# kharchenkolab/dropEst

Hardware: AMD Instinct MI355X
Metric: Mreads/s processed to final count matrix (higher is better)
Workload: dtype u64

## Files before the change

dropest_amd/csrc/context.h:

```cpp
#pragma once

#include <algorithm>
#include <chrono>
#include <condition_variable>
#include <functional>
#include <mutex>
#include <cstring>
#include <map>
#include <memory>
#include <string>
#include <thread>
#include <unordered_map>
#include <unordered_set>
#include <vector>

#include "../../include/dropest_amd.h"
#include "k_cbhash.h"
#include "k_collisions.h"
#include "k_merge.h"
#include "k_umi_directional.h"
#include "whitelist.h"
#include "k_misc.h"
#include "k_radix.h"
#include "k_ssort.h"
#include "k_segreduce.h"
#include "k_mergepath.h"
#include "matrix_decode.h"
#include "util.h"

namespace dropest {

typedef unsigned long long u64;
typedef uint32_t u32;

struct ReadChunk {
	DevBuf<u64> cb, umi;
	DevBuf<u32> gene, aux;
	const u64 *p_cb = nullptr, *p_umi = nullptr;
	const u32 *p_gene = nullptr, *p_aux = nullptr;
	uint64_t n = 0;
};

struct KernelStat { u32 launches = 0; double ms = 0, bytes = 0; };

__global__ __launch_bounds__(256) void store_append_kernel(const u64 *__restrict__ s_cb, const u64 *__restrict__ s_umi, const u32 *__restrict__ s_gene, const u32 *__restrict__ s_aux,
                                                           u64 *__restrict__ d_cb, u64 *__restrict__ d_umi, u32 *__restrict__ d_gene, u32 *__restrict__ d_aux, size_t count) {
	for (size_t i = size_t(blockIdx.x) * 256u + threadIdx.x; i < count; i += size_t(gridDim.x) * 256u) { d_cb[i] = s_cb[i]; d_umi[i] = s_umi[i]; d_gene[i] = s_gene[i]; d_aux[i] = s_aux[i]; }
}

struct ReadStore {
	DevBuf<u64> cb, umi;
	DevBuf<u32> gene, aux;
	size_t n = 0;
	hipStream_t copy = nullptr;
	PinnedBuf<unsigned char> stage[2];
	hipEvent_t done[2] = {nullptr, nullptr};
	int cur = 0;
	~ReadStore() { for (auto e : done) if (e) (void)hipEventDestroy(e); if (copy) (void)hipStreamDestroy(copy); }
	size_t capacity() const { return cb.n; }
	void reserve(size_t want) {
		if (want <= capacity() && cb.p) return;
		size_t cap = std::max<size_t>(want, std::max<size_t>(capacity() * 2, size_t(1) << 20));
		if (n && !copy) HIP_CHECK(hipStreamCreateWithFlags(&copy, hipStreamNonBlocking));
		if (copy) HIP_CHECK(stream_wait(copy));
		DevBuf<u64> ncb, numi; DevBuf<u32> ngene, naux;
		ncb.alloc(cap); numi.alloc(cap); ngene.alloc(cap); naux.alloc(cap);
		ncb.mark_persistent(); numi.mark_persistent(); ngene.mark_persistent(); naux.mark_persistent();
		if (n) {
			HIP_CHECK(hipMemcpyAsync(ncb.p, cb.p, n * 8, hipMemcpyDeviceToDevice, copy));
			HIP_CHECK(hipMemcpyAsync(numi.p, umi.p, n * 8, hipMemcpyDeviceToDevice, copy));
			HIP_CHECK(hipMemcpyAsync(ngene.p, gene.p, n * 4, hipMemcpyDeviceToDevice, copy));
			HIP_CHECK(hipMemcpyAsync(naux.p, aux.p, n * 4, hipMemcpyDeviceToDevice, copy));
			HIP_CHECK(stream_wait(copy));
		}
		cb = std::move(ncb); umi = std::move(numi); gene = std::move(ngene); aux = std::move(naux);
	}
	static bool is_pinned(const void *p) {
		hipPointerAttribute_t a{};
		if (hipPointerGetAttributes(&a, p) != hipSuccess) { (void)hipGetLastError(); return false; }
		return a.type == hipMemoryTypeHost;
	}
	void push(const uint64_t *h_cb, const uint64_t *h_umi, const uint32_t *h_gene, const uint32_t *h_aux, size_t count) {
		if (!count) return;
		reserve(n + count);
		if (!copy) HIP_CHECK(hipStreamCreateWithFlags(&copy, hipStreamNonBlocking));
		if (is_pinned(h_cb) && is_pinned(h_umi) && is_pinned(h_gene) && is_pinned(h_aux)) {
			HIP_CHECK(hipMemcpyAsync(cb.p + n, h_cb, count * 8, hipMemcpyHostToDevice, copy));
			HIP_CHECK(hipMemcpyAsync(umi.p + n, h_umi, count * 8, hipMemcpyHostToDevice, copy));
			HIP_CHECK(hipMemcpyAsync(gene.p + n, h_gene, count * 4, hipMemcpyHostToDevice, copy));
			HIP_CHECK(hipMemcpyAsync(aux.p + n, h_aux, count * 4, hipMemcpyHostToDevice, copy));
			HIP_CHECK(stream_wait(copy));
			n += count;
			return;
		}
		const size_t piece_max = size_t(4) << 20;
		for (size_t at = 0; at < count; at += piece_max) {
			const size_t m = std::min(piece_max, count - at);
			PinnedBuf<unsigned char> &st = stage[cur];
			if (!done[cur]) HIP_CHECK(hipEventCreateWithFlags(&done[cur], hipEventDisableTiming));
			else HIP_CHECK(event_wait(done[cur]));
			st.ensure(m * 24);
			unsigned char *b = st.p;
			std::memcpy(b, h_cb + at, m * 8); std::memcpy(b + m * 8, h_umi + at, m * 8);
			std::memcpy(b + m * 16, h_gene + at, m * 4); std::memcpy(b + m * 20, h_aux + at, m * 4);
			HIP_CHECK(hipMemcpyAsync(cb.p + n, b, m * 8, hipMemcpyHostToDevice, copy));
			HIP_CHECK(hipMemcpyAsync(umi.p + n, b + m * 8, m * 8, hipMemcpyHostToDevice, copy));
			HIP_CHECK(hipMemcpyAsync(gene.p + n, b + m * 16, m * 4, hipMemcpyHostToDevice, copy));
			HIP_CHECK(hipMemcpyAsync(aux.p + n, b + m * 20, m * 4, hipMemcpyHostToDevice, copy));
			HIP_CHECK(hipEventRecord(done[cur], copy));
			cur ^= 1;
			n += m;
		}
	}
	void push_segments(size_t n_seg, const uint64_t *const *h_cb, const uint64_t *const *h_umi, const uint32_t *const *h_gene, const uint32_t *const *h_aux,
	                   const uint64_t *counts) {
		size_t total = 0;
		for (size_t k = 0; k < n_seg; ++k) total += size_t(counts[k]);
		if (!total) return;
		if (total > (size_t(4) << 20)) { for (size_t k = 0; k < n_seg; ++k) push(h_cb[k], h_umi[k], h_gene[k], h_aux[k], size_t(counts[k])); return; }
		reserve(n + total);
		if (!copy) HIP_CHECK(hipStreamCreateWithFlags(&copy, hipStreamNonBlocking));
		PinnedBuf<unsigned char> &st = stage[cur];
		if (!done[cur]) HIP_CHECK(hipEventCreateWithFlags(&done[cur], hipEventDisableTiming));
		else HIP_CHECK(event_wait(done[cur]));
		st.ensure(total * 24);
		unsigned char *b = st.p;
		size_t at = 0;
		for (size_t k = 0; k < n_seg; ++k) {
			const size_t m = size_t(counts[k]);
			if (!m) continue;
			std::memcpy(b + at * 8, h_cb[k], m * 8); std::memcpy(b + total * 8 + at * 8, h_umi[k], m * 8);
			std::memcpy(b + total * 16 + at * 4, h_gene[k], m * 4); std::memcpy(b + total * 20 + at * 4, h_aux[k], m * 4);
			at += m;
		}
		HIP_CHECK(hipMemcpyAsync(cb.p + n, b, total * 8, hipMemcpyHostToDevice, copy));
		HIP_CHECK(hipMemcpyAsync(umi.p + n, b + total * 8, total * 8, hipMemcpyHostToDevice, copy));
		HIP_CHECK(hipMemcpyAsync(gene.p + n, b + total * 16, total * 4, hipMemcpyHostToDevice, copy));
		HIP_CHECK(hipMemcpyAsync(aux.p + n, b + total * 20, total * 4, hipMemcpyHostToDevice, copy));
		HIP_CHECK(hipEventRecord(done[cur], copy));
		cur ^= 1;
		n += total;
	}
	void push_device(const uint64_t *d_cb, const uint64_t *d_umi, const uint32_t *d_gene, const uint32_t *d_aux, size_t count, hipStream_t on) {
		if (!count) return;
		reserve(n + count);
		hipLaunchKernelGGL(store_append_kernel, dim3(unsigned(std::min<size_t>((count + 255) / 256, 4096))), dim3(256), 0, on, reinterpret_cast<const u64 *>(d_cb),
		                   reinterpret_cast<const u64 *>(d_umi), d_gene, d_aux, cb.p + n, umi.p + n, gene.p + n, aux.p + n, count);
		HIP_CHECK(hipGetLastError());
		HIP_CHECK(stream_wait(on));
		n += count;
	}
	void push_peer(const uint64_t *d_cb, const uint64_t *d_umi, const uint32_t *d_gene, const uint32_t *d_aux, size_t count, int dst_device, int src_device, hipStream_t on) {
		if (!count) return;
		reserve(n + count);
		HIP_CHECK(hipMemcpyPeerAsync(cb.p + n, dst_device, d_cb, src_device, count * 8, on));
		HIP_CHECK(hipMemcpyPeerAsync(umi.p + n, dst_device, d_umi, src_device, count * 8, on));
		HIP_CHECK(hipMemcpyPeerAsync(gene.p + n, dst_device, d_gene, src_device, count * 4, on));
		HIP_CHECK(hipMemcpyPeerAsync(aux.p + n, dst_device, d_aux, src_device, count * 4, on));
		HIP_CHECK(stream_wait(on));
		n += count;
	}
	void wait() { if (copy) HIP_CHECK(stream_wait(copy)); }
	void clear() { wait(); n = 0; }
};

inline std::string decode_code(u64 code, const std::vector<std::string> &side) {
	if (code & ESCAPE_BIT) {
		u64 k = code & ~ESCAPE_BIT;
		if (k >= side.size()) throw RangeError("escaped code refers to an unregistered side string");
		return side[k];
	}
	if (code == 0) return std::string();
	int len = (bit_length(code) - 1) / 2;
	std::string s(size_t(len), 'A');
	for (int i = 0; i < len; ++i) s[size_t(i)] = "ACGT"[(code >> (2 * (len - 1 - i))) & 3];
	return s;
}
inline bool encode_code(const std::string &s, u64 &code) {
	if (s.empty() || s.size() > 31) return false;
	u64 c = 1;
// ... 73 lines not shown
		std::unique_lock<std::mutex> one(job_m, std::try_to_lock);
		if (!one.owns_lock()) return false;
		{
			std::lock_guard<std::mutex> lk(m);
			job = fn; active = workers; pending = workers; ++generation; error.clear();
		}
		cv_go.notify_all();
		std::unique_lock<std::mutex> lk(m);
		cv_done.wait(lk, [&] { return pending == 0; });
		if (!error.empty()) throw std::runtime_error(error);
		return true;
	}
};
template <class F>
inline unsigned parallel_ranges(size_t n, F &&fn, size_t min_per_worker = 100000, unsigned max_workers = 8) {
	HostPool &pool = HostPool::get();
	unsigned workers = unsigned(std::min<size_t>(std::min<size_t>(max_workers, pool.size()), std::max<size_t>(1, n / std::max<size_t>(1, min_per_worker))));
	if (workers <= 1) { fn(size_t(0), n, 0u); return 1; }
	if (pool.run(workers, [&](unsigned w) { fn(n * w / workers, n * (w + 1) / workers, w); })) return workers;
	for (unsigned w = 0; w < workers; ++w) fn(n * w / workers, n * (w + 1) / workers, w);
	return workers;
}

struct GlibcRand {
	uint32_t ring[34];
	int pos = 0;
	uint64_t drawn = 0;
	explicit GlibcRand(unsigned seed = 1) { this->seed(seed); }
	void seed(unsigned s) {
		int32_t r[34];
		r[0] = int32_t(s ? s : 1u);
		for (int i = 1; i < 31; ++i) {
			const int64_t hi = r[i - 1] / 127773, lo = r[i - 1] % 127773;
			int64_t w = 16807 * lo - 2836 * hi;
			if (w < 0) w += 2147483647;
			r[i] = int32_t(w);
		}
		for (int i = 0; i < 31; ++i) ring[i] = uint32_t(r[i]);
		for (int i = 31; i < 34; ++i) ring[i] = ring[i - 31];
		pos = 0; drawn = 0;
		for (int i = 0; i < 310; ++i) step();
	}
	uint32_t step() {
		const uint32_t v = ring[(pos + 3) % 34] + ring[(pos + 31) % 34];
		ring[pos] = v;
		pos = (pos + 1) % 34;
		return v;
	}
	int next() { ++drawn; return int(step() >> 1); }
	void skip_to(uint64_t n_drawn) { while (drawn < n_drawn) next(); }
};

struct HostCell {
	u32 id;
	CellRowPod row;
	bool merged = false, excluded = false;
};

}

struct SimplePairs { std::vector<uint64_t> key; std::vector<uint32_t> cnt, ed; std::vector<double> prob;  };

struct dropest_ctx {
	using u64 = dropest::u64;
	using u32 = dropest::u32;

	dropest_cfg cfg;
	std::string barcodes_file, match_levels;
	u32 query_mask = 0;
	u32 min_before = 0, min_after = 0;
	hipStream_t stream = nullptr;

	std::vector<dropest::ReadChunk> chunks;
	dropest::ReadStore store;
	long store_chunk = -1;
	uint64_t n_reads = 0;
	dropest::DevBuf<u64> cat_cb, cat_umi;
	dropest::DevBuf<u32> cat_gene, cat_aux;
	const u64 *d_cb = nullptr, *d_umi = nullptr;
	const u32 *d_gene = nullptr, *d_aux = nullptr;
	std::vector<std::string> side;
	dropest::ReadPack rpack{};
	std::function<void()> unpack_reads;
	void need_columns() {
		if (!rpack.on()) return;
		if (!unpack_reads) throw dropest::InvalidError("internal: packed reads without an unpacker");
		unpack_reads();
		rpack = dropest::ReadPack{};
	}

	bool initialized = false, merged = false;
	dropest::GlibcRand rng;
	void reseed_rng() { rng.seed(cfg.umi_merge_kind == DROPEST_UMI_MERGE_SIMPLE ? 42u : 1u); }

	dropest::DevBuf<dropest::CbSlot> t_slots;
	dropest::DevBuf<u32> slot;
	dropest::DevBuf<u64> hot_key;
	dropest::DevBuf<u32> hot_slot;
	u32 n_hot = 0;
	dropest::CbTable table{};
	uint64_t forced_table_capacity = 0;
	u32 n_cells = 0;
	dropest::DevBuf<u64> cell_cb;
	dropest::DevBuf<u32> cell_first;
	dropest::KeyLayout layout{};
	int umi_clean_bits = 0;
	u32 wanted_bits[3] = {0, 0, 0};
	bool umi_sentinel_stripped = false;
	int umi_dict_mode = 0;
	bool umi_dict_on = false;
	u32 umi_dict_n = 0;
	dropest::DevBuf<u64> umi_dict, umi_ranked;
	std::vector<u64> umi_dict_host;
	const u64 *umi_key_column() const { return umi_dict_on ? umi_ranked.p : d_umi; }
	void build_umi_dict(const std::function<void(dropest::DevBuf<u64> &, u32 &)> *across = nullptr);
	bool umi_dict_wanted(int gene_bits, int cell_bits) const;
	void sort_unique_u64(dropest::DevBuf<u64> &d, u32 &n);
	bool map_umi(u64 api_code, u64 &field) const;
	bool map_umi_or_add(u64 api_code, u64 &field);
	dropest::IngestStats ingest{};
	dropest::GlobalCounters counters{};

	dropest::DevBuf<u64> keys_a, keys_b;
	dropest::DevBuf<u32> vals_a, vals_b;
	bool chr_from_gene = false;
	bool lazy_stats = false;
	dropest::DevBuf<u32> gene_chr;
	dropest::DevBuf<u32> mol_exon, mol_intron, mol_exon2, mol_intron2, cg_exon, cg_intron;

	u32 n_mol = 0;
	dropest::DevBuf<u64> mol_key;
	dropest::DevBuf<u32> mol_reads, mol_mark;
	u32 n_cg = 0;
	dropest::DevBuf<u64> cg_key;
	dropest::DevBuf<u32> cg_mol_begin, cg_n_all, cg_n_req, cg_reads_all, cg_reads_req;
	dropest::DevBuf<u32> cell_cg_count;
	dropest::DevBuf<u32> cell_cg_begin, cell_n_genes, cell_req_genes, cell_req_umis, cell_total_umis, cell_total_reads;
	u32 n_chr_rows = 0;
	dropest::DevBuf<u64> chr_row_key;
	dropest::DevBuf<u32> chr_exon, chr_intron, chr_inter;

	dropest::Whitelist wl;
	dropest::DevBuf<dropest::WlEntry> d_wl[dropest::WL_MAX_PARTS];
	dropest::DevBuf<u64> d_wl_code[dropest::WL_MAX_PARTS];
	dropest::DevBuf<dropest::WlTabRow> d_wl_tab[dropest::WL_MAX_PARTS];
	bool wl_tab_ok = false;
	dropest::DevBuf<u64> mol_key2;
	dropest::DevBuf<u32> mol_reads2, mol_mark2, remap;
	std::unordered_map<u32, u32> reassign;
	std::unordered_map<u64, std::vector<dropest::UmiOverride>> umi_overrides;

	dropest::PinnedBuf<unsigned char> h_stage;
	void fetch(void *dst, const void *d_src, size_t bytes);
	dropest::PinnedBuf<unsigned char> h_up;
	void upload(void *d_dst, const void *src, size_t bytes);

	dropest::DevBuf<u32> tile_counts, tile_prefix, scalars, rs_hist, rs_row_total, rs_digit_base;
	dropest::DevBuf<u32> real_list;
	dropest::DevBuf<dropest::CellRowPod> real_rows_dev;
	dropest::DevBuf<u32> sizes_dev;
	bool real_list_current = false;
	bool real_pristine = false;
	dropest::DevBuf<u64> scalars64;
	struct MatrixResult {
		dropest::DevBuf<u32> d_row, d_val;
		dropest::PinnedBuf<u32> h_row, h_val;
		struct List {
			dropest::DevBuf<u32> d;
			dropest::PinnedBuf<u32> h;
			u32 cap = 0, n = 0;
			void ensure(u32 c, bool to_host) { cap = c; d.ensure(1 + 2 * size_t(c)); if (to_host) h.ensure(1 + 2 * size_t(c)); }
			u32 *d_count() const { return d.p; }
			u32 *d_pos() const { return d.p + 1; }
			u32 *d_val() const { return d.p + 1 + cap; }
			u32 *h_count() const { return h.p; }
			u32 *h_pos() const { return h.p ? h.p + 1 : nullptr; }
			u32 *h_val() const { return h.p ? h.p + 1 + cap : nullptr; }
		};
		dropest::DevBuf<uint16_t> d_row16, d_val16;
		dropest::PinnedBuf<uint16_t> h_row16, h_val16;
		List vals;
		dropest::DevBuf<uint8_t> d_drow8, d_val8;
		dropest::PinnedBuf<uint8_t> h_drow8, h_val8;
		List rows;
		int narrow = 0;
		dropest::DevBuf<u32> d_col_cell, d_col_start, d_col_list;
		std::vector<u32> col_list_host;
		bool wire = false;
		std::shared_ptr<dropest::DecodeJob> job, late_job;
		std::chrono::steady_clock::time_point job_t0;
		MatrixResult *dependent = nullptr;
		std::vector<u32> rider_out, rider_cnt, wire_chunk_end;
		dropest::DevBuf<u32> d_rider_out;
		void settle() {
			if (dependent) { MatrixResult *d = dependent; dependent = nullptr; d->settle(); }
			if (job) { (void)job->wait(); job->quiesce(); job.reset(); }
			if (late_job) { late_job->quiesce(); late_job.reset(); }
		}
		dropest::PinnedBuf<u32> h_flags;
		u32 wire_epoch = 0;
		std::vector<u32> colptr;
		uint64_t nnz = 0, ncols = 0;
	} mat[3];
	dropest::DevBuf<dropest::IngestStats> d_ingest;
	dropest::DevBuf<dropest::GlobalCounters> d_counters;

	std::vector<dropest::HostCell> real;
	std::vector<uint64_t> filtered;
	std::vector<u32> filtered_ridx;
	dropest::PinnedBuf<u64> sort_stage;
	dropest::DevBuf<u64> sort_cols;
	std::vector<u32> sort_idx;
	std::vector<int32_t> filtered_umis;
	std::vector<uint64_t> sort_ids;
	bool filtered_valid = false;
	u32 filtered_threshold = 0;
	int filtered_max_cells = -1;
	struct CbMirror {
		std::vector<u64> key; std::vector<u32> id; u64 mask = 0; int level = 0;
		void clear() { key.clear(); id.clear(); mask = 0; level = 0; }
		void build(size_t n, const std::function<void(size_t, u64 &, u32 &)> &item) {
			size_t cap = 16; while (cap < n * 2 + 2) cap <<= 1;
			key.assign(cap, 0ull); id.assign(cap, 0u); mask = cap - 1;
			for (size_t i = 0; i < n; ++i) {
				u64 k; u32 v; item(i, k, v);
				u64 h = dropest::mix64(k) & mask;
				while (key[h] != 0ull && key[h] != k) h = (h + 1) & mask;
				key[h] = k; id[h] = v;
			}
		}
		long find(u64 k) const {
			if (key.empty()) return -1;
			for (u64 h = dropest::mix64(k) & mask;; h = (h + 1) & mask) { if (key[h] == k) return long(id[h]); if (key[h] == 0ull) return -1; }
		}
	} cb_mirror;
	long real_find(u32 cell_id) const {
		size_t lo = 0, hi = real.size();
		while (lo < hi) { size_t mid = (lo + hi) / 2; if (real[mid].id < cell_id) lo = mid + 1; else hi = mid; }
		return (lo < real.size() && real[lo].id == cell_id) ? long(lo) : -1;
	}
	u32 real_at(u32 cell_id) const {
		long i = real_find(cell_id);
		if (i < 0) throw dropest::RangeError("cell is not a real-candidate cell");
		return u32(i);
	}
	std::string barcode_of(const dropest::HostCell &h) const { return dropest::decode_code(h.row.barcode, side); }
	const std::vector<uint64_t> &filtered_cells();
	std::vector<std::pair<uint64_t, uint64_t>> merge_pairs;
	uint64_t n_real_now = 0;

	bool profiling = false;
	std::string profile_only;
	std::map<std::string, dropest::KernelStat> stats;
	struct Pending { std::string name; hipEvent_t a, b; double bytes; };
	std::vector<Pending> pending;
	std::vector<hipEvent_t> event_pool;

	bool stage_sync = getenv("DROPEST_STAGE_SYNC") != nullptr;
	struct HostStage {
		dropest_ctx *c; const char *name; std::chrono::steady_clock::time_point t0;
		HostStage(dropest_ctx *ctx, const char *n) : c(ctx), name(n) {
			if (c->stage_sync && c->profiling) (void)dropest::stream_wait(c->stream);
			t0 = std::chrono::steady_clock::now();
		}
		~HostStage() {
			if (!c->profiling || !c->profile_only.empty()) return;
			if (c->stage_sync) (void)dropest::stream_wait(c->stream);
			auto &s = c->stats[std::string("host:") + name];
			s.launches++;
			s.ms += std::chrono::duration<double, std::milli>(std::chrono::steady_clock::now() - t0).count();
		}
	};

	~dropest_ctx();
	void init_from_cfg(const dropest_cfg &c);

	template <class F> void timed(const char *name, double bytes, F &&launch);
	void collect_timings();

	void concat_chunks();
	void free_results();
	void release_tables() {
		t_slots.release(); slot.release(); keys_a.release(); keys_b.release(); vals_a.release(); vals_b.release();
		mol_key.release(); mol_reads.release(); mol_mark.release(); mol_key2.release(); mol_reads2.release(); mol_mark2.release();
		mol_exon.release(); mol_intron.release(); mol_exon2.release(); mol_intron2.release();
	}
	void run_set_initialized();
	void run_merge_and_filter();

	void build_cb_table();
	void assign_cell_ids();
	void plan_key_layout();
	void build_keys(bool with_stats = false, bool allow_fused = true);
	bool build_keys_fused(bool with_stats);
	void ss_splitters_from_sample(u32 n_sample, u32 os, u32 Ff, u32 F2, u64 varying_of_sample);
	bool keys_in_l1 = false;
	dropest::DevBuf<u32> ks_flag;
	u32 main_sort_passes = 0, main_sort_kind = 0;
	void scan_counts(const u32 *in, u32 *out, u32 n, u32 *total_out);
	dropest::DevBuf<u32> scan_chunk;
	void radix_sort(u64 *&keys, u32 *&vals, u64 *&keys_alt, u32 *&vals_alt, u32 n, u64 varying_mask, int val_bytes = 4,
	                const char *stat_prefix = nullptr);
	dropest::DevBuf<u64> ss_sample_a, ss_sample_b, ss_fine, ss_coarse;
	dropest::DevBuf<u32> ss_base1, ss_cnt2, ss_bucket_base, ss_bucket_cnt, ss_tmp, ss_n_loc, ss_prefix, ss_chunk, ss_big_list;
	struct RecvChunk { hipEvent_t ev; dropest::CbRanges rg; };
	std::vector<RecvChunk> recv_chunks;
	double hot_coverage = 0;
	dropest::DevBuf<u32> ss_cg_loc, ss_cg_cnt, ss_cg_prefix;
	bool cg_from_sort = false;
	dropest::DevBuf<u32> ss_cursors;
	bool ss_no_reserve = false;
	bool splitter_sort_reduce();
	void reduce_all();
	void reduce_molecules_to_cell_gene();
	void reduce_cell_gene_to_cells();
	void refresh_real_rows();
	void upload_whitelist();
	void search_merge_candidates(const std::vector<u32> &cells, const dropest::MergeUniverse &U, dropest::MergeSearch &S);
	void search_merge_candidates_host(const std::vector<u32> &cells, const dropest::MergeUniverse &U, dropest::MergeSearch &S);
	void build_merge_pairs(const std::vector<u32> &cells, dropest::MergeSearch &S);
	void decide_merge_targets(const dropest::MergeUniverse &U, dropest::MergeSearch &S, const std::vector<u32> &inter,
	                          std::vector<long> &targets, std::vector<u32> &target_ridx);
	std::vector<std::vector<u32>> replay_candidate_orders(const dropest::MergeUniverse &U, dropest::MergeSearch &S,
	                                                      const std::vector<u32> &need_order);
	std::vector<u32> pair_intersections(const std::vector<u32> &pair_base_cell, const std::vector<u32> &pair_cand_cell);
	void pair_intersections(const std::vector<u32> &pair_base_cell, const std::vector<u32> &pair_cand_cell, std::vector<u32> &inter);
	std::vector<double> poisson_expected_intersections(const std::vector<u32> &pair_base_cell, const std::vector<u32> &pair_cand_cell);
	struct PoissonTables { dropest::DevBuf<double> p, mult, np; dropest::DevBuf<u64> adj; u32 n_classes = 0, max_size = 0; bool ready = false; } ptab;
	void poisson_local_umis(u32 &kept, u32 &max_size);
	struct PoissonSource { const u32 *cell_cg_begin, *cell_cg_count; const u64 *cg_key; const u32 *cg_mol_begin; u64 gene_mask; };
	void poisson_tables_from_state();
	void poisson_tables_from_umi_codes(u32 kept, u64 code_mask, u32 max_size);
	void poisson_expected_pairs(const PoissonSource &src, const u32 *d_pb, const u32 *d_pc, u32 NP, const u32 *count_host, double *expected);
	struct ValidationView {
		dropest::DevBuf<u64> mol_key, cg_key;
		dropest::DevBuf<u32> cg_mol_begin, cell_cg_begin, cell_cg_count;
		dropest::DevBuf<uint4> barcodes;
		std::vector<uint64_t> cells;
		std::vector<u32> umis;
		u32 n_mol = 0, n_cg = 0, F = 0;
		int umi_bits = 0, gene_bits = 0;
		u64 gene_none = 0;
		double ms = 0;
	};
	bool is_shard_ctx = false, was_split = false;
	void validation_build_view(ValidationView &V);
	void validation_set_barcodes(ValidationView &V, const std::vector<std::string> &text);
	void validation_finish_view(ValidationView &V);
	struct ValidationPairs {
		dropest::DevBuf<u32> d_pb, d_pc, d_cnt, d_inter; dropest::DevBuf<dropest::PairRange> d_pr;
		std::vector<u32> cnt;
	};
	bool validation_common_genes(const ValidationView &V, const std::vector<u32> &a, const std::vector<u32> &b, ValidationPairs &P);
	u32 validation_evaluate_range(const ValidationView &V, const dropest_validation_opts &opts, ValidationPairs &P, u32 q0, u32 q1, u32 *inter, double *expected);
	static void validation_tail(size_t n, const u32 *inter, double *expected, double *prob);
	void validation_sample(const ValidationView &V, const dropest_validation_opts &opts, dropest_validation_sample &S, std::vector<u32> &a, std::vector<u32> &b);
	void validation_evaluate(const ValidationView &V, const dropest_validation_opts &opts, dropest_validation_sample &S, const std::vector<u32> &a,
	                         const std::vector<u32> &b);
	void run_merge_validation(const dropest_validation_opts *opts, dropest_validation_sample *samples, u32 n_samples);
	void poisson_build_tables(const u32 *d_counts, u32 n_counts, double total, u32 max_size);
	void poisson_expected_from_keys(const u32 *d_off, u32 NP, const u64 *d_keys, u32 NK, double *expected_host);
	void shard_merge_umi_histogram(dropest::DevBuf<u32> &hist, uint64_t &kept, u32 &max_size);
	void shard_merge_set_umi_distribution(const u32 *d_counts, uint64_t n_counts, uint64_t kept_total, u32 max_size);
	void shard_merge_expected(uint64_t n_pairs, const uint32_t *cand_local, const uint64_t *base_begin, const uint64_t *base_end,
	                          const uint64_t *d_base_low, double *expected);
	void shard_merge_decide_poisson(const uint32_t *inter, const double *expected, int64_t *target_g);
	void decide_poisson_targets(const dropest::MergeUniverse &U, dropest::MergeSearch &S, const std::vector<u32> &inter,
	                            const std::vector<double> &expected, std::vector<long> &targets, std::vector<u32> &target_ridx);
	std::vector<long> compute_merge_targets(const std::vector<u32> &cells, const std::vector<u32> &ridx,
	                                        std::vector<u32> *target_ridx = nullptr);
	void compute_merge_targets(const std::vector<u32> &cells, const std::vector<u32> &ridx, std::vector<long> &targets,
	                           std::vector<u32> *target_ridx);
	dropest::DevBuf<u32> cell_real_index;
	struct MergeScratch {
		dropest::MergeSearch S;
		std::vector<u32> pb, inter, tr, cells, ridx, target_ridx, cur, rank, src, tgt32, lists, ids_dense;
		std::vector<long> targets;
		std::vector<int64_t> tgt;
		std::vector<int32_t> reads, umis;
		std::vector<uint8_t> excl;
		dropest::DevBuf<u32> d_pb, d_pc, d_inter, d_src, d_tgt;
		dropest::DevBuf<dropest::PairRange> d_pr;
	} ms;
	void run_cb_merge_real();
	void run_cb_merge_simple();
	void simple_merge_targets(std::vector<u32> &cells, std::vector<u32> &tgt_id, SimplePairs &P);
	struct StrategyTargets { bool valid = false; std::vector<u32> cells, target; SimplePairs P; } strategy_targets;
	const StrategyTargets &need_strategy_targets();
	struct SimpleReplayInput { std::vector<u64> query; std::vector<std::vector<u32>> in_order; };
	void simple_pair_table(const u64 *sorted, u32 n_valid, int cell_bits, const u32 *d_cell_size, const u64 *d_cell_code, SimplePairs &P,
	                       dropest::DevBuf<u64> *d_run_key, dropest::DevBuf<u32> *d_run_cnt, u32 *n_runs = nullptr);
	void simple_pairs_to_host(const u64 *d_run_key, const u32 *d_run_cnt, u32 runs, const u64 *d_cell_code, SimplePairs &P);
	void simple_replay_local(const std::vector<u32> &bases, SimpleReplayInput &R, bool globalize);
	void run_cb_merge_all();
	void merge_all_filtered_targets(std::vector<u32> &target_pos);
	void merge_all_targets(std::vector<u64> code, const std::vector<int32_t> &umis, const std::function<std::string(u32)> &text,
	                       const std::vector<u32> *bases, std::vector<u32> &target_pos);
	std::unordered_set<u32> extra_excluded;
	std::unordered_set<u32> explicit_sources;
	void clear_strategy_pairs() {
		if (explicit_sources.empty()) { merge_pairs.clear(); return; }
		std::vector<std::pair<uint64_t, uint64_t>> keep;
		for (auto const &pr : merge_pairs) if (explicit_sources.count(u32(pr.first))) keep.push_back(pr);
		merge_pairs.swap(keep);
	}
	void mutate_exclude_cell(u32 cell);
	void mutate_merge_cells(u32 src, u32 tgt);
	void mutate_merge_umis(u32 cell, u32 gene, uint64_t n, const uint64_t *src, const uint64_t *tgt);
	void mutate_add_umi_to_cell(u32 cell, u32 gene, uint64_t umi_code, u32 mark, const uint8_t *quality, u32 quality_length);
	u32 n_qsum_rows = 0;
	void emit_matrix_levels(u32 query_mask, bool reads_output);
	struct ShardMerge;
	std::shared_ptr<ShardMerge> shard;
	bool ingested = false, external_merge_done = false;
	void run_ingest();
	void shard_export_rows(const std::vector<u32> &local_cells);
	void shard_merge_begin_free();
	void shard_merge_search(uint64_t n_global, const uint64_t *g_barcode, const uint32_t *g_n_genes, const int32_t *g_total_umis,
	                        uint64_t n_bases, const uint32_t *base_g, const uint32_t *base_local, uint64_t *n_pairs);
	void shard_merge_intersect(uint64_t n_pairs, const uint32_t *cand_local, const uint64_t *base_begin, const uint64_t *base_end,
	                           const uint64_t *d_base_low, uint32_t *inter);
	void shard_merge_decide(const uint32_t *inter, int64_t *target_g);
	void shard_merge_quality_import(uint64_t n_local, const uint32_t *local_rank, const uint32_t *d_import_rank, const uint32_t *d_import_q);
	const u32 *reagg_import_prio = nullptr;
	u32 reagg_import_from = 0, reagg_import_n = 0;
	void shard_merge_finish(uint64_t n_local, const uint32_t *local_id, const uint8_t *excluded, const uint8_t *merged_away,
	                        const int32_t *total_reads, const int32_t *total_umis, uint64_t n_moves, const uint32_t *move_src,
	                        const uint32_t *move_tgt, uint64_t n_import, const uint32_t *d_cell, const uint64_t *d_low,
	                        const uint32_t *const d_cols[4]);
	void reaggregate_after_merge();
	void run_umi_merge_simple();
	std::vector<u32> umi_first_positions(const std::vector<u64> &sorted_codes);
	struct ShardHooks {
		std::function<std::vector<u64>(const std::vector<u64> &)> first_seen_global;
		std::function<std::vector<u64>(const std::vector<u32> &, const std::vector<u32> &, const std::vector<u32> &)> rng_offsets;
		std::function<void(u32 *, size_t)> globalize_umi_first;
	};
	std::shared_ptr<ShardHooks> hooks;
	void emit_columns_device(bool filtered_m, bool reads_output, const std::vector<u32> &col_cell, const std::vector<u32> &col_start, uint64_t nnz, bool wait = true);
	struct GatheredGroups { std::vector<u32> size, off, begin, hr, hm, hfirst; std::vector<u64> hk; };
	void umi_gather_groups(const std::vector<u32> &groups, GatheredGroups &G, const u32 *d_first_table);
	void umi_patch_groups(const std::vector<u32> &p_idx, const std::vector<u32> &p_all, const std::vector<u32> &p_req,
	                      const std::vector<u32> &p_rreq, const std::unordered_map<u32, int> &umis_removed);
// ... 59 lines not shown
```

dropest_amd/csrc/dropest_amd.hip:

```cpp

#include "context.h"
extern "C" void dropest_bgzf_warm_up(void *stream);
#include "k_keyscatter.h"
#include "k_umidict.h"

#include <atomic>
#include <functional>
#include <map>
#include <mutex>

using namespace dropest;

static thread_local std::string g_last_error;

template <class F>
static dropest_status guarded(F &&f) {
	try {
		f();
		return DROPEST_OK;
	} catch (const InvalidError &e) { g_last_error = e.what(); return DROPEST_ERR_INVALID;
	} catch (const RangeError &e) { g_last_error = e.what(); return DROPEST_ERR_RANGE;
	} catch (const UnsupportedError &e) { g_last_error = e.what(); return DROPEST_ERR_UNSUPPORTED;
	} catch (const IoError &e) { g_last_error = e.what(); return DROPEST_ERR_IO;
	} catch (const DeviceError &e) { g_last_error = e.what(); return DROPEST_ERR_DEVICE;
	} catch (const std::bad_alloc &) { g_last_error = "host allocation failed"; return DROPEST_ERR_DEVICE;
	} catch (const std::exception &e) { g_last_error = e.what(); return DROPEST_ERR_INVALID; }
}

static void need_init(dropest_ctx *ctx) {
	if (!ctx) throw InvalidError("null context");
	if (!ctx->initialized) throw InvalidError("You must initialize container");
	HIP_CHECK(hipSetDevice(ctx->cfg.device));
}

static inline u32 div_up(uint64_t a, uint64_t b) { return u32((a + b - 1) / b); }

static void partition_by_owner_on(int device, hipStream_t st, const u64 *d_cb, const u64 *d_umi, const u32 *d_gene, const u32 *d_aux, uint64_t n64,
                                  u32 n_parts, u64 *d_out_cb, u64 *d_out_umi, u32 *d_out_gene, u32 *d_out_aux, u32 *d_out_idx, uint64_t *counts,
                                  void *d_scratch, uint64_t scratch_bytes);

template <class K>
static u32 resident_grid(K kernel, int threads, u32 wanted) {
	int dev = 0, cus = 0, per_cu = 0;
	HIP_CHECK(hipGetDevice(&dev));
	HIP_CHECK(hipDeviceGetAttribute(&cus, hipDeviceAttributeMultiprocessorCount, dev));
	HIP_CHECK(hipOccupancyMaxActiveBlocksPerMultiprocessor(&per_cu, kernel, threads, 0));
	return std::max<u32>(1u, std::min<u32>(wanted, u32(std::max(1, cus) * std::max(1, per_cu))));
}

static u32 query_mask_from_code(const std::string &code) {
	u32 m = 0;
	for (char c : code) {
		switch (c) {
			case 'e': m |= 1u << 2; break;
			case 'i': m |= 1u << 4; break;
			case 'E': m |= 1u << 3; break;
			case 'I': m |= 1u << 5; break;
			case 'B': m |= 1u << 6; break;
			case 'A': m |= 1u << 7; break;
			default: throw InvalidError(std::string("Unexpected gene match levels: ") + c);
		}
	}
	return m;
}

void dropest_ctx::init_from_cfg(const dropest_cfg &c) {
	cfg = c;
	barcodes_file = c.barcodes_file ? c.barcodes_file : "";
	match_levels = c.gene_match_levels ? c.gene_match_levels : "eEBA";
	cfg.barcodes_file = barcodes_file.c_str();
	cfg.gene_match_levels = match_levels.c_str();
	query_mask = query_mask_from_code(match_levels);
	if (c.min_genes_before_merge < 0 || c.min_genes_after_merge < 0) throw InvalidError("negative gene threshold");
	min_before = u32(c.min_genes_before_merge);
	min_after = std::max(u32(c.min_genes_after_merge), min_before);
	if (c.merge_kind != DROPEST_MERGE_NONE && c.merge_kind != DROPEST_MERGE_REAL_BARCODES && c.merge_kind != DROPEST_MERGE_SIMPLE &&
	    c.merge_kind != DROPEST_MERGE_POISSON_REAL && c.merge_kind != DROPEST_MERGE_POISSON_SIMPLE && c.merge_kind != DROPEST_MERGE_ALL)
		throw InvalidError("unknown merge_kind");
	if (c.umi_merge_kind != DROPEST_UMI_MERGE_SIMPLE && c.umi_merge_kind != DROPEST_UMI_MERGE_DIRECTIONAL)
		throw InvalidError("unknown umi_merge_kind");
	if (c.max_umi_merge_edit_distance < 0) throw InvalidError("negative max_umi_merge_edit_distance");
	int ndev = 0;
	if (hipGetDeviceCount(&ndev) != hipSuccess || ndev == 0)
		throw DeviceError("no HIP device visible: the dropEst hot path has no CPU implementation");
	if (c.device < 0 || c.device >= ndev) throw InvalidError("device ordinal out of range");
	HIP_CHECK(hipSetDevice(c.device));
	HIP_CHECK(hipStreamCreateWithFlags(&stream, hipStreamNonBlocking));
	{
		void *scratch = nullptr;
		HIP_CHECK(hipMalloc(&scratch, 256));
		(void)hipMemsetAsync(scratch, 0, 256, stream);
		(void)hipMemsetAsync(scratch, 0, 256, nullptr);
		{
			void *pin = nullptr, *big = nullptr;
			const size_t mb = size_t(1) << 20;
			if (hipHostMalloc(&pin, mb, hipHostMallocDefault) == hipSuccess && hipMalloc(&big, mb) == hipSuccess) {
				(void)hipMemcpyAsync(big, pin, mb, hipMemcpyHostToDevice, nullptr);
				(void)hipMemcpyAsync(pin, big, mb, hipMemcpyDeviceToHost, nullptr);
				(void)hipStreamSynchronize(nullptr);
				for (size_t bytes : {size_t(8) << 10, size_t(48) << 10, size_t(256) << 10, mb}) {
					(void)hipMemcpyAsync(big, pin, bytes, hipMemcpyHostToDevice, stream);
					(void)hipMemcpyAsync(pin, big, bytes, hipMemcpyDeviceToHost, stream);
				}
				(void)hipStreamSynchronize(stream);
			}
			if (big) (void)hipFree(big);
			if (pin) (void)hipHostFree(pin);
		}
		hipLaunchKernelGGL(store_append_kernel, dim3(1), dim3(256), 0, stream, (const u64 *)nullptr, (const u64 *)nullptr, (const u32 *)nullptr, (const u32 *)nullptr,
		                   (u64 *)nullptr, (u64 *)nullptr, (u32 *)nullptr, (u32 *)nullptr, size_t(0));
		(void)hipGetLastError();
		dropest_bgzf_warm_up(stream);
		(void)hipStreamSynchronize(stream);
		(void)hipStreamSynchronize(nullptr);
		(void)hipFree(scratch);
	}
	reseed_rng();
}

dropest_ctx::~dropest_ctx() {
	for (auto &p : pending) { (void)hipEventDestroy(p.a); (void)hipEventDestroy(p.b); }
	for (auto e : event_pool) (void)hipEventDestroy(e);
	for (auto &M : mat) M.settle();
	if (stream2) { (void)stream_wait(stream2); (void)hipStreamDestroy(stream2); }
	if (ev_fork) (void)hipEventDestroy(ev_fork);
	if (ev_raw) (void)hipEventDestroy(ev_raw);
	if (ev_ship) (void)hipEventDestroy(ev_ship);
	if (stream) (void)hipStreamDestroy(stream);
}

template <class F>
void dropest_ctx::timed(const char *name, double bytes, F &&launch) {
	auto selected = [&]() {
		if (profile_only.empty()) return true;
		size_t at = 0;
		while (at <= profile_only.size()) {
			size_t end = profile_only.find('|', at);
			if (end == std::string::npos) end = profile_only.size();
			if (end > at && std::strncmp(name, profile_only.c_str() + at, end - at) == 0) return true;
			at = end + 1;
		}
		return false;
	};
	static const bool sync_trace = getenv("DROPEST_SYNC_TRACE") != nullptr;
	if (sync_trace) {
		fprintf(stderr, "[launch %p] %s\n", static_cast<void *>(this), name);
		launch();
		HIP_CHECK(hipGetLastError());
		HIP_CHECK(hipStreamSynchronize(stream));
		if (stream2) HIP_CHECK(hipStreamSynchronize(stream2));
		fprintf(stderr, "[done   %p] %s\n", static_cast<void *>(this), name);
		return;
	}
	if (!profiling || !selected()) {
		launch(); HIP_CHECK(hipGetLastError()); return;
	}
	auto get = [&]() {
		if (!event_pool.empty()) { hipEvent_t e = event_pool.back(); event_pool.pop_back(); return e; }
		hipEvent_t e; HIP_CHECK(hipEventCreate(&e)); return e;
	};
	hipEvent_t a = get(), b = get();
	HIP_CHECK(hipEventRecord(a, stream));
	launch();
	HIP_CHECK(hipGetLastError());
	HIP_CHECK(hipEventRecord(b, stream));
	pending.push_back(Pending{name, a, b, bytes});
}

void dropest_ctx::fetch(void *dst, const void *d_src, size_t bytes) {
	if (!bytes) return;
	h_stage.ensure(std::max<size_t>(bytes, 4096));
	HIP_CHECK(hipMemcpyAsync(h_stage.p, d_src, bytes, hipMemcpyDeviceToHost, stream));
	HIP_CHECK(stream_wait(stream));
	if (bytes < (size_t(4) << 20)) std::memcpy(dst, h_stage.p, bytes);
	else
		dropest::parallel_ranges(bytes, [&](size_t b, size_t e, unsigned) { std::memcpy(static_cast<char *>(dst) + b, h_stage.p + b, e - b); }, size_t(2) << 20, dropest::HostPool::MAX);
}

void dropest_ctx::upload(void *d_dst, const void *src, size_t bytes) {
	if (!bytes) return;
	if (bytes < (size_t(1) << 20)) { HIP_CHECK(hipMemcpyAsync(d_dst, src, bytes, hipMemcpyHostToDevice, stream)); HIP_CHECK(stream_wait(stream)); return; }
	h_up.ensure(bytes);
	dropest::parallel_ranges(bytes, [&](size_t b, size_t e, unsigned) { std::memcpy(h_up.p + b, static_cast<const char *>(src) + b, e - b); }, size_t(2) << 20, dropest::HostPool::MAX);
	HIP_CHECK(hipMemcpyAsync(d_dst, h_up.p, bytes, hipMemcpyHostToDevice, stream));
	HIP_CHECK(stream_wait(stream));
}

static void tail_mark(const char *what, bool restart = false) {
	static const bool on = getenv("DROPEST_TAIL_TRACE") != nullptr;
	if (!on) return;
	static thread_local std::chrono::steady_clock::time_point t0;
	const auto now = std::chrono::steady_clock::now();
	if (restart) t0 = now;
	fprintf(stderr, "[tail] %9.1f us  %s\n", std::chrono::duration<double, std::micro>(now - t0).count(), what);
}

void dropest_ctx::collect_timings() {
	if (pending.empty()) return;
	HIP_CHECK(stream_wait(stream));
	for (auto &p : pending) {
		float ms = 0;
		HIP_CHECK(hipEventElapsedTime(&ms, p.a, p.b));
		auto &s = stats[p.name];
		s.launches++; s.ms += ms; s.bytes += p.bytes;
		event_pool.push_back(p.a); event_pool.push_back(p.b);
	}
	pending.clear();
}

void dropest_ctx::concat_chunks() {
	if (d_cb) return;
	if (n_reads == 0) return;
	store.wait();
	if (store_chunk >= 0) {
		dropest::ReadChunk &c = chunks[size_t(store_chunk)];
		c.p_cb = store.cb.p; c.p_umi = store.umi.p; c.p_gene = store.gene.p; c.p_aux = store.aux.p; c.n = store.n;
	}
	if (n_reads >= 0xFFFFFFFEull) throw UnsupportedError("more than 2^32-2 reads in one context (shard across GPUs)");
	if (chunks.size() == 1) {
		d_cb = chunks[0].p_cb; d_umi = chunks[0].p_umi; d_gene = chunks[0].p_gene; d_aux = chunks[0].p_aux;
		return;
	}
	cat_cb.alloc(n_reads); cat_umi.alloc(n_reads); cat_gene.alloc(n_reads); cat_aux.alloc(n_reads);
	cat_cb.mark_persistent(); cat_umi.mark_persistent(); cat_gene.mark_persistent(); cat_aux.mark_persistent();
	uint64_t off = 0;
	for (auto &c : chunks) {
		HIP_CHECK(hipMemcpyAsync(cat_cb.p + off, c.p_cb, c.n * 8, hipMemcpyDeviceToDevice, stream));
		HIP_CHECK(hipMemcpyAsync(cat_umi.p + off, c.p_umi, c.n * 8, hipMemcpyDeviceToDevice, stream));
		HIP_CHECK(hipMemcpyAsync(cat_gene.p + off, c.p_gene, c.n * 4, hipMemcpyDeviceToDevice, stream));
		HIP_CHECK(hipMemcpyAsync(cat_aux.p + off, c.p_aux, c.n * 4, hipMemcpyDeviceToDevice, stream));
		off += c.n;
	}
	HIP_CHECK(stream_wait(stream));
	chunks.clear();
	chunks.emplace_back();
	chunks[0].p_cb = cat_cb.p; chunks[0].p_umi = cat_umi.p; chunks[0].p_gene = cat_gene.p; chunks[0].p_aux = cat_aux.p;
	chunks[0].n = n_reads;
	d_cb = cat_cb.p; d_umi = cat_umi.p; d_gene = cat_gene.p; d_aux = cat_aux.p;
}

void dropest_ctx::free_results() {
	HostStage hs(this, "reset");
	invalidate_prefetch();
	initialized = merged = ingested = external_merge_done = false;
	ss_no_reserve = false;
	reseed_rng();
	shard.reset();
	n_cells = n_mol = n_cg = n_chr_rows = 0;
	cb_mirror.clear(); real_pristine = false;
	real.clear(); filtered.clear(); filtered_valid = false; strategy_targets = StrategyTargets(); merge_pairs.clear(); reassign.clear(); umi_overrides.clear(); n_real_now = 0;
	merge_rank.clear(); reagg_prio = nullptr; extra_excluded.clear(); explicit_sources.clear(); mol_sorted_rows = 0xFFFFFFFFu;
	layout = dropest::KeyLayout{}; umi_clean_bits = 0; umi_sentinel_stripped = false; chr_from_gene = false;
	umi_dict_on = false; umi_dict_n = 0; umi_dict_host.clear();
}

static constexpr u32 GENE_CHR_CAP = 1u << 20;

void dropest_ctx::build_cb_table() {
	const u32 n = u32(n_reads);
	uint64_t cap = forced_table_capacity ? forced_table_capacity : cfg.cb_table_capacity;
	const bool chunked = !recv_chunks.empty() && !forced_table_capacity;
	const u32 n_chunks_in = chunked ? u32(recv_chunks.size()) : 1u;
	if (chunked) HIP_CHECK(hipStreamWaitEvent(stream, recv_chunks[0].ev, 0));
	uint64_t n_first = n;
	if (chunked) n_first = recv_chunks[0].rg.total();
	auto over_sample_ranges = [&](auto &&f) {
		if (!chunked) { f(u32(0), n); return; }
		const CbRanges &rg = recv_chunks[0].rg;
		for (u32 q = 0; q < rg.n; ++q) if (rg.cnt[q]) f(rg.off[q], rg.cnt[q]);
	};
	uint64_t sample_min = uint64_t(1) << 22;
	if (const char *e = getenv("DROPEST_CB_SAMPLE_MIN")) sample_min = uint64_t(std::max(1ll, atoll(e)));
	if (cap == 0 && n_reads >= sample_min && !getenv("DROPEST_CB_NO_SAMPLE")) {
		const u32 stride = 64, n_s = u32(div_up(u32(std::min<uint64_t>(n_first, n)), stride)) + (chunked ? 64u : 0u);
		uint64_t cap_s = 1024; while (cap_s < uint64_t(n_s) * 2) cap_s <<= 1;
		t_slots.ensure(cap_s); scalars.ensure(4 + CB_HOT_LEVELS + 4);
		CbTable ts{t_slots.p, cap_s - 1};
		HIP_CHECK(hipMemsetAsync(t_slots.p, 0, cap_s * sizeof(CbSlot), stream));
		HIP_CHECK(hipMemsetAsync(scalars.p, 0, 4, stream));
		timed("cb_sample", double(n_s) * 8, [&] {
			static const u32 count_every = [] { const char *e = getenv("DROPEST_CB_SAMPLE_COUNT_EVERY"); return e && atoi(e) >= 1 ? u32(atoi(e)) : 4u; }();
			over_sample_ranges([&](u32 off, u32 cnt) {
				hipLaunchKernelGGL(cb_sample_distinct_kernel, dim3(std::min<u32>(div_up(div_up(cnt, stride), 256), 2048u)), dim3(256), 0, stream, d_cb + off, cnt, stride, ts, scalars.p, rpack, count_every);
			});
		});
		HIP_CHECK(hipMemsetAsync(scalars.p + 4, 0, 4 * CB_HOT_LEVELS, stream));
		const bool want_hot = !getenv("DROPEST_CB_NO_HOT");
		if (want_hot) timed("cb_hot_count", double(cap_s) * sizeof(CbSlot), [&] { hipLaunchKernelGGL(cb_hot_count_kernel, dim3(1024), dim3(256), 0, stream, ts, scalars.p + 4); });
		u32 head[4 + CB_HOT_LEVELS] = {0};
		fetch(head, scalars.p, sizeof(head));
		const u32 distinct = head[0];
		if (getenv("DROPEST_CB_TRACE")) {
			fprintf(stderr, "[cb] sample of %u reads: %u distinct; barcodes with >= t sample hits:", n_s, distinct);
			for (int l = 0; l < CB_HOT_LEVELS; ++l) fprintf(stderr, " %u:%u", cb_hot_threshold(l), head[4 + l]);
			fprintf(stderr, "\n");
		}
		const uint64_t est = std::min<uint64_t>(n_reads, uint64_t(double(distinct) * stride * (double(n) / double(std::max<uint64_t>(1, n_first)))));
		cap = 1024; while (cap < est + est / 2) cap <<= 1;
		n_hot = 0; hot_coverage = 0;
		if (want_hot && cap < (1ull << 31)) {
			int level = -1;
			for (int l = 0; l < CB_HOT_LEVELS; ++l) if (head[4 + l] <= CB_HOT_MAX) { level = l; break; }
			if (level >= 0 && head[4 + level] >= 16) {
				hot_key.ensure(CB_HOT_MAX); hot_slot.ensure(CB_HOT_MAX);
				HIP_CHECK(hipMemsetAsync(scalars.p + 1, 0, 4, stream));
				timed("cb_hot_collect", double(cap_s) * sizeof(CbSlot), [&] {
					hipLaunchKernelGGL(cb_hot_collect_kernel, dim3(1024), dim3(256), 0, stream, ts, cb_hot_threshold(level), hot_key.p, scalars.p + 1);
				});
				n_hot = head[4 + level];
				double covered = 0;
				for (int l = level; l < CB_HOT_LEVELS; ++l) covered += double(head[4 + l] - (l + 1 < CB_HOT_LEVELS ? head[4 + l + 1] : 0u)) * cb_hot_threshold(l);
				hot_coverage = covered / double(std::max<u32>(1u, n_s));
			}
		}
		if (profiling) stats["count:hot_barcodes"].launches = n_hot;
	} else n_hot = 0;
	if (cap == 0) { cap = 1024; while (cap < n_reads / 2) cap <<= 1; }
	if (cap & (cap - 1)) throw InvalidError("cb_table_capacity must be a power of two");
	slot.ensure(n);
	d_ingest.ensure(1);
	for (int attempt = 0;; ++attempt) {
		if (cap > (1ull << 32)) throw UnsupportedError("barcode table would exceed 2^32 slots");
		t_slots.ensure(cap);
		table.slots = t_slots.p; table.mask = cap - 1;
		HIP_CHECK(hipMemsetAsync(t_slots.p, 0, cap * sizeof(CbSlot), stream));
		IngestStats init{};
		init.umi_clean_min = ~0ull;
		HIP_CHECK(hipMemcpyAsync(d_ingest.p, &init, sizeof(init), hipMemcpyHostToDevice, stream));
		gene_chr.ensure(GENE_CHR_CAP);
		HIP_CHECK(hipMemsetAsync(gene_chr.p, 0xFF, size_t(GENE_CHR_CAP) * 4, stream));
		if (n >= (1u << 20) || lazy_stats) {
			const u32 stride = 2048, n_s = div_up(n, stride);
			timed("gene_chr_seed", double(n_s) * 8, [&] {
				over_sample_ranges([&](u32 off, u32 cnt) {
					hipLaunchKernelGGL(gene_chr_seed_kernel, dim3(std::min<u32>(div_up(div_up(cnt, stride), 256), 64u)), dim3(256), 0, stream, d_gene + off, d_aux + off, cnt, stride, gene_chr.p, GENE_CHR_CAP, d_ingest.p, rpack);
				});
			});
		}
		const bool vec = ((uintptr_t(d_cb) | uintptr_t(d_umi) | uintptr_t(d_gene) | uintptr_t(d_aux)) & 15u) == 0;
		static const u32 grid_v = resident_grid(cb_insert_kernel<256, true>, 256, ~0u), grid_s = resident_grid(cb_insert_kernel<256, false>, 256, ~0u);
		const u32 blocks = std::min<u32>(div_up(n, 256 * 4), vec ? grid_v : grid_s);
		if (lazy_stats)
			timed("ingest_sample_stats", double(div_up(n, 256u)) * 16, [&] {
				const u32 every = std::max<u32>(1u, 256u / n_chunks_in);
				over_sample_ranges([&](u32 off, u32 cnt) {
					hipLaunchKernelGGL(ingest_sample_stats_kernel, dim3(std::min<u32>(div_up(div_up(cnt, every), 256), 1024u)), dim3(256), 0, stream, d_umi + off, d_gene + off, d_aux + off, cnt, every, d_ingest.p, rpack);
				});
			});
		if (n_hot && attempt == 0 && cap < (1ull << 31)) {
			const int want = int(size_t(CB_HOT_LDS) * 16);
			bool granted = true;
			for (const void *k : {reinterpret_cast<const void *>(cb_insert_hot_kernel<true, false>), reinterpret_cast<const void *>(cb_insert_hot_kernel<false, false>),
			                      reinterpret_cast<const void *>(cb_insert_hot_kernel<true>), reinterpret_cast<const void *>(cb_insert_hot_kernel<false>)})
				if (hipFuncSetAttribute(k, hipFuncAttributeMaxDynamicSharedMemorySize, want) != hipSuccess) { (void)hipGetLastError(); granted = false; }
			if (!granted) n_hot = 0;
		}
		if (n_hot && attempt == 0 && cap < (1ull << 31)) {
			hipLaunchKernelGGL(cb_hot_preinsert_kernel, dim3(div_up(n_hot, 256)), dim3(256), 0, stream, hot_key.p, n_hot, table, hot_slot.p, &d_ingest.p->overflow);
			HIP_CHECK(hipGetLastError());
			const size_t lds = size_t(CB_HOT_LDS) * 16;
			int cus = 0;
			HIP_CHECK(hipDeviceGetAttribute(&cus, hipDeviceAttributeMultiprocessorCount, cfg.device));
			const u32 hb = std::min<u32>(div_up(n, 1024 * 4), u32(std::max(1, cus)));
			const CbHot hot{hot_key.p, hot_slot.p, n_hot};
			timed("cb_insert", double(n) * (lazy_stats ? 8 + 4 : 8 + 8 + 4 + 4 + 4), [&] {
				auto go = [&](auto kernel) {
					HIP_CHECK(hipFuncSetAttribute(reinterpret_cast<const void *>(kernel), hipFuncAttributeMaxDynamicSharedMemorySize, int(lds)));
					for (u32 k = 0; k < n_chunks_in; ++k) {
						if (chunked && k) HIP_CHECK(hipStreamWaitEvent(stream, recv_chunks[k].ev, 0));
						hipLaunchKernelGGL(kernel, dim3(hb), dim3(1024), lds, stream, d_cb, d_umi, d_gene, d_aux, chunked ? recv_chunks[k].rg : CbRanges::whole(n), table, hot, slot.p, gene_chr.p, GENE_CHR_CAP, d_ingest.p, rpack);
					}
				};
				if (lazy_stats) { if (vec) go(cb_insert_hot_kernel<true, false>); else go(cb_insert_hot_kernel<false, false>); }
				else if (vec) go(cb_insert_hot_kernel<true>); else go(cb_insert_hot_kernel<false>);
			});
#ifdef DROPEST_CBI_PROBE
			if (lazy_stats && vec && getenv("DROPEST_CBI_PROBE")) {
				keys_a.ensure(n);
				auto again = [&](const char *name, auto kernel) {
					HIP_CHECK(hipFuncSetAttribute(reinterpret_cast<const void *>(kernel), hipFuncAttributeMaxDynamicSharedMemorySize, int(lds)));
					timed(name, double(n) * 12, [&] { hipLaunchKernelGGL(kernel, dim3(hb), dim3(1024), lds, stream, d_cb, d_umi, d_gene, d_aux, CbRanges::whole(n), table, hot, reinterpret_cast<u32 *>(keys_a.p), gene_chr.p, GENE_CHR_CAP, d_ingest.p); });
				};
				again("cbi:again", cb_insert_hot_kernel<true, false, 0>);
				again("cbi:no_probe", cb_insert_hot_kernel<true, false, 1>);
				again("cbi:no_lds", cb_insert_hot_kernel<true, false, 2>);
				again("cbi:no_atomics", cb_insert_hot_kernel<true, false, 4>);
				again("cbi:no_probe_no_lds", cb_insert_hot_kernel<true, false, 3>);
				again("cbi:no_probe_no_atomics", cb_insert_hot_kernel<true, false, 5>);
			}
#endif
		} else {
		n_hot = 0;
		timed("cb_insert", double(n) * (lazy_stats ? 8 + 4 : 8 + 8 + 4 + 4 + 4), [&] {
			auto go = [&](auto kernel) {
				const bool by_chunk = chunked && attempt == 0;
				for (u32 k = 0; k < (by_chunk ? n_chunks_in : 1u); ++k) {
					if (by_chunk && k) HIP_CHECK(hipStreamWaitEvent(stream, recv_chunks[k].ev, 0));
					hipLaunchKernelGGL(kernel, dim3(blocks), dim3(256), 0, stream, d_cb, d_umi, d_gene, d_aux, by_chunk ? recv_chunks[k].rg : CbRanges::whole(n), table, slot.p, gene_chr.p, GENE_CHR_CAP, d_ingest.p, rpack);
				}
			};
			if (lazy_stats) { if (vec) go(cb_insert_kernel<256, true, false>); else go(cb_insert_kernel<256, false, false>); }
			else if (vec) go(cb_insert_kernel<256, true>); else go(cb_insert_kernel<256, false>);
		});
		}
		fetch(&ingest, d_ingest.p, sizeof(ingest));
		if (!ingest.overflow) break;
		if (attempt >= 6) throw DeviceError("barcode table overflow after repeated growth");
		cap <<= 2;
	}
}

void dropest_ctx::assign_cell_ids() {
	const u32 n = u32(n_reads);
	const uint64_t cap = table.mask + 1;
	keys_a.ensure(n); keys_b.ensure(n);
	vals_a.ensure(1); vals_b.ensure(1);
	scalars.ensure(16);
	HIP_CHECK(hipMemsetAsync(scalars.p, 0, 4, stream));
	timed("cb_compact_slots", double(cap) * 16, [&] {
		hipLaunchKernelGGL(cb_compact_slots_kernel, dim3(u32(std::min<uint64_t>((cap + 4095) / 4096, 4096))), dim3(256), 0, stream, table,
		                   keys_a.p, scalars.p);
	});
	u32 total = 0;
	fetch(&total, scalars.p, 4);
	n_cells = total;
	if (uint64_t(n_cells) * 10 > cap * 7)
	{
		forced_table_capacity = cap << 2;
		build_cb_table();
		return assign_cell_ids();
	}
	u64 *k = keys_a.p, *k_alt = keys_b.p;
	u32 *v = vals_a.p, *v_alt = vals_b.p;
	const int ord_bits = std::max(1, bit_length(uint64_t(n ? n - 1 : 0)));
	radix_sort(k, v, k_alt, v_alt, n_cells, ((1ull << ord_bits) - 1ull) << 32, 0, "cell_ids:");
	cell_cb.ensure(n_cells); cell_first.ensure(n_cells);
	timed("cb_assign_ids", double(n_cells) * 40, [&] {
		hipLaunchKernelGGL(cb_assign_sorted_kernel, dim3(div_up(n_cells, 256)), dim3(256), 0, stream, k, n_cells, table, cell_cb.p, cell_first.p);
	});
}

void dropest_ctx::plan_key_layout() {
	KeyLayout L{};
	const bool any_clean = ingest.umi_clean_max != 0;
	int clean_bits = 0;
	umi_sentinel_stripped = false;
	if (any_clean) {
		const int bl_min = bit_length(ingest.umi_clean_min), bl_max = bit_length(ingest.umi_clean_max);
		if (bl_min == bl_max) {
			umi_sentinel_stripped = true;
			clean_bits = bl_max - 1;
			L.umi_strip_mask = clean_bits ? ((1ull << clean_bits) - 1ull) : 0ull;
		} else {
			clean_bits = bl_max;
			L.umi_strip_mask = ~0ull;
		}
	}
	L.gene_bits = bit_length(uint64_t(ingest.gene_max_plus1));
	if ((1ull << L.gene_bits) - 1 < ingest.gene_max_plus1) L.gene_bits++;
	if (L.gene_bits == 0) L.gene_bits = 1;
	L.gene_none = (1ull << L.gene_bits) - 1ull;
	L.cell_bits = std::max(1, bit_length(uint64_t(n_cells ? n_cells - 1 : 0)));
	if (!umi_dict_on && n_reads && !hooks && !rpack.on() && umi_dict_wanted(L.gene_bits, L.cell_bits)) build_umi_dict();
	if (umi_dict_on) {
		umi_sentinel_stripped = false;
		clean_bits = std::max(1, bit_length(uint64_t(umi_dict_n) + 255u));
		L.umi_strip_mask = ~0ull;
	}
	umi_clean_bits = clean_bits;
	L.umi_escape_base = 1ull << clean_bits;
	L.umi_bits = clean_bits;
	if (ingest.umi_escape_max_plus1) L.umi_bits = bit_length(L.umi_escape_base + ingest.umi_escape_max_plus1 - 1);
	wanted_bits[0] = u32(L.cell_bits); wanted_bits[1] = u32(L.gene_bits); wanted_bits[2] = u32(L.umi_bits);
	if (L.gene_bits + L.umi_bits >= 64)
		throw UnsupportedError("gene + UMI fields of the sort key need " + std::to_string(L.gene_bits + L.umi_bits) + " bits and leave no room for the cells; "
		                       "the pass should have keyed the UMIs by their rank in a dictionary (k_umidict.h; sharded runs: shard_run.h global_umi_dictionary)");
	if (L.umi_bits + L.gene_bits + L.cell_bits > 64)
		throw UnsupportedError("sort key needs " + std::to_string(L.umi_bits + L.gene_bits + L.cell_bits) +
		                       " bits (cell " + std::to_string(L.cell_bits) + " + gene " + std::to_string(L.gene_bits) +
		                       " + UMI " + std::to_string(L.umi_bits) + "); one context sorts 64-bit keys -- the cell field shrinks when the stream is split by barcode: dropest_ctx_split");
	chr_from_gene = !ingest.gene_chr_conflict && (L.umi_bits >= 16 || (u64(ingest.chr_max_plus1) <= (1ull << L.umi_bits)));
	if (getenv("DROPEST_FORCE_GENERAL_LAYOUT")) chr_from_gene = false;
	if (chr_from_gene) {
		const bool fits = L.umi_bits + L.gene_bits + L.cell_bits + 3 <= 64 && !getenv("DROPEST_FORCE_BYTE_VALUES");
		L.mark_shift = fits ? 3 : 0;
		L.val_bytes = fits ? 0 : 1;
	} else {
		L.mark_shift = 0; L.val_bytes = 4;
	}
	layout = L;
}

bool dropest_ctx::umi_dict_wanted(int gene_bits, int cell_bits) const {
	int clean_bits = 0;
	if (ingest.umi_clean_max != 0) {
		const int bl_min = bit_length(ingest.umi_clean_min), bl_max = bit_length(ingest.umi_clean_max);
		clean_bits = bl_min == bl_max ? bl_max - 1 : bl_max;
	}
	int plain_bits = clean_bits;
	if (ingest.umi_escape_max_plus1) plain_bits = bit_length((1ull << clean_bits) + ingest.umi_escape_max_plus1 - 1);
	const int mode = getenv("DROPEST_UMI_DICT") ? atoi(getenv("DROPEST_UMI_DICT")) : umi_dict_mode;
	return mode >= 2 || gene_bits + plain_bits >= 64 || (mode == 1 && plain_bits + gene_bits + cell_bits > 64);
}

void dropest_ctx::build_umi_dict(const std::function<void(dropest::DevBuf<u64> &, u32 &)> *across) {
	HostStage hs(this, "umi_dict");
	need_columns();
	const u32 n = u32(n_reads);
	u32 total = 0;
	umi_dict.ensure(1);
	if (n) {
		keys_a.ensure(n); keys_b.ensure(n); vals_a.ensure(1); vals_b.ensure(1);
		u64 *k = keys_a.p, *k_alt = keys_b.p;
		u32 *v = vals_a.p, *v_alt = vals_b.p;
		timed("umi_dict:fill", double(n) * 20, [&] {
			hipLaunchKernelGGL(umi_dict_fill_kernel, dim3(std::min<u32>(div_up(n, 256), 8192u)), dim3(256), 0, stream, d_umi, d_gene, n, k);
		});
		radix_sort(k, v, k_alt, v_alt, n, ~0ull, 0, "umi_dict:");
		const u32 nb = div_up(n, u32(UD_T * UD_PER));
		DevBuf<u32> cnt, base;
		cnt.alloc(nb); base.alloc(nb);
		scalars.ensure(16);
		timed("umi_dict:unique", double(n) * 16, [&] {
			hipLaunchKernelGGL(umi_dict_count_kernel, dim3(nb), dim3(UD_T), 0, stream, k, n, cnt.p);
			scan_counts(cnt.p, base.p, nb, scalars.p);
		});
		fetch(&total, scalars.p, 4);
		umi_dict.ensure(std::max<u32>(total, 1u));
		if (total) hipLaunchKernelGGL(umi_dict_write_kernel, dim3(nb), dim3(UD_T), 0, stream, k, n, base.p, umi_dict.p);
		HIP_CHECK(hipGetLastError());
	}
	if (across) { HIP_CHECK(stream_wait(stream)); (*across)(umi_dict, total); }
	umi_dict_n = total;
	umi_ranked.ensure(std::max<u32>(n, 1u));
	timed("umi_dict:rank", double(n) * 20, [&] {
		if (n) hipLaunchKernelGGL(umi_dict_rank_kernel, dim3(std::min<u32>(div_up(n, 256), 8192u)), dim3(256), 0, stream, d_umi, d_gene, n, umi_dict.p, total, umi_ranked.p);
	});
	HIP_CHECK(hipGetLastError());
	umi_dict_host.resize(total);
	if (total) fetch(umi_dict_host.data(), umi_dict.p, size_t(total) * 8);
	else HIP_CHECK(stream_wait(stream));
	umi_dict_on = true;
	if (profiling) stats["count:umi_dictionary"].launches += 1;
}

void dropest_ctx::sort_unique_u64(dropest::DevBuf<u64> &d, u32 &n) {
	if (n == 0) return;
	keys_a.ensure(n); keys_b.ensure(n); vals_a.ensure(1); vals_b.ensure(1);
	HIP_CHECK(hipMemcpyAsync(keys_a.p, d.p, size_t(n) * 8, hipMemcpyDeviceToDevice, stream));
	u64 *k = keys_a.p, *k_alt = keys_b.p;
	u32 *v = vals_a.p, *v_alt = vals_b.p;
	radix_sort(k, v, k_alt, v_alt, n, ~0ull, 0, "umi_dict:all:");
	const u32 nb = div_up(n, u32(UD_T * UD_PER));
	DevBuf<u32> cnt, base;
	cnt.alloc(nb); base.alloc(nb);
	scalars.ensure(16);
	hipLaunchKernelGGL(umi_dict_count_kernel, dim3(nb), dim3(UD_T), 0, stream, k, n, cnt.p);
	scan_counts(cnt.p, base.p, nb, scalars.p);
	u32 total = 0;
	fetch(&total, scalars.p, 4);
	d.ensure(std::max<u32>(total, 1u));
	if (total) hipLaunchKernelGGL(umi_dict_write_kernel, dim3(nb), dim3(UD_T), 0, stream, k, n, base.p, d.p);
	HIP_CHECK(hipGetLastError());
	HIP_CHECK(stream_wait(stream));
	n = total;
}

dropest_ctx::u64 dropest_ctx::unmap_umi(u64 ucode) const {
	if (ucode >= layout.umi_escape_base && ingest.umi_escape_max_plus1) return ESCAPE_BIT | (ucode - layout.umi_escape_base);
	if (umi_dict_on) {
		if (ucode >= umi_dict_host.size()) throw InvalidError("internal: UMI rank beyond the dictionary");
		return umi_dict_host[size_t(ucode)];
	}
	if (umi_sentinel_stripped) return (1ull << umi_clean_bits) | ucode;
	return ucode;
}

bool dropest_ctx::map_umi(u64 api_code, u64 &field) const {
	const u64 umask = layout.umi_bits ? ((1ull << layout.umi_bits) - 1ull) : 0ull;
	if (api_code & ESCAPE_BIT) {
		const u64 id = api_code & ~ESCAPE_BIT;
		if (id >= ingest.umi_escape_max_plus1) return false;
		field = layout.umi_escape_base + id;
		return true;
	}
	if (umi_dict_on) {
		const auto sorted_end = umi_dict_host.begin() + umi_dict_n;
		auto it = std::lower_bound(umi_dict_host.begin(), sorted_end, api_code);
		if (it == sorted_end || *it != api_code) it = std::find(sorted_end, umi_dict_host.end(), api_code);
		if (it == umi_dict_host.end()) return false;
		field = u64(it - umi_dict_host.begin());
		return true;
	}
	if (umi_sentinel_stripped && bit_length(api_code) - 1 != umi_clean_bits) return false;
	field = api_code & layout.umi_strip_mask;
	return !(field > umask || (ingest.umi_escape_max_plus1 && field >= layout.umi_escape_base));
}

bool dropest_ctx::map_umi_or_add(u64 api_code, u64 &field) {
	if (map_umi(api_code, field)) return true;
	if (!umi_dict_on || (api_code & ESCAPE_BIT) || u64(umi_dict_host.size()) >= layout.umi_escape_base) return false;
	field = u64(umi_dict_host.size());
	umi_dict_host.push_back(api_code);
	return true;
}

static int sort_mode_override() {
	const char *e = getenv("DROPEST_SORT");
	if (!e) return 0;
	return !strcmp(e, "lsd") ? 1 : (!strcmp(e, "splitter") ? 2 : 0);
}

struct SsPlan { bool applicable = false, reserve = false; int tb = 0, fb1 = 0, fb2 = 0; uint64_t cap1 = 0, cap2 = 0, span = 0, os = 64; };
static SsPlan ss_plan(uint64_t n_reads, bool chr_from_gene, int val_bytes) {
	SsPlan P;
	const int mode = sort_mode_override();
	const char *e_min = getenv("DROPEST_SSORT_MIN");
	const uint64_t min_reads = e_min ? uint64_t(atoll(e_min)) : (uint64_t(1) << 22);
	if (mode == 1 || !chr_from_gene || val_bytes > 1) return P;
	if (mode != 2 && n_reads < min_reads) return P;
	if (n_reads < 512 || n_reads >= 0xFFFFFFFEull) return P;
	int tb = 8;
	while (tb < 20 && (n_reads >> tb) > 1600) ++tb;
	if (const char *e = getenv("DROPEST_SSORT_TB")) tb = std::min(20, std::max(8, atoi(e)));
	if ((n_reads >> tb) > 4096) return P;
	P.applicable = true; P.tb = tb; P.fb1 = tb / 2; P.fb2 = tb - P.fb1;
	const uint64_t F1 = 1ull << P.fb1, F2 = 1ull << tb, mean1 = (n_reads + F1 - 1) / F1, mean2 = (n_reads + F2 - 1) / F2;
	P.cap1 = (mean1 + mean1 / 16 + 2 * SS_TILE + 15) & ~15ull;
	P.cap2 = (mean2 + mean2 * 3 / 4 + 64 + 15) & ~15ull;
	if (mean2 <= 1024 && n_reads >= (1ull << 28) && !getenv("DROPEST_SSORT_OS")) {
		P.os = 32;
		P.cap2 = (mean2 * 5 / 2 + 64 + 15) & ~15ull;
	}
	if (const char *e = getenv("DROPEST_SS_CAP2_PERCENT")) P.cap2 = (mean2 * uint64_t(std::max(100, atoi(e))) / 100 + 15) & ~15ull;
	P.span = std::max(F1 * P.cap1, F2 * P.cap2);
	P.reserve = !getenv("DROPEST_SS_NO_RESERVE") && P.span < 0xFFFFFFF0ull;
	if (!P.reserve) P.span = n_reads;
	return P;
}

void dropest_ctx::ss_splitters_from_sample(u32 n_sample, u32 os, u32 Ff, u32 F2, u64 varying_of_sample) {
	u64 *k = ss_sample_a.p, *k_alt = ss_sample_b.p;
	u32 *v = nullptr, *v_alt = nullptr;
	radix_sort(k, v, k_alt, v_alt, n_sample, varying_of_sample, 0, "ss_sample:");
	hipLaunchKernelGGL(ss_pick_splitters_kernel, dim3(div_up(F2, 256)), dim3(256), 0, stream, k, os, Ff, F2, ss_fine.p, ss_coarse.p);
	HIP_CHECK(hipGetLastError());
}

bool dropest_ctx::build_keys_fused(bool with_stats) {
	const bool off = getenv("DROPEST_NO_FUSED_KEYS") != nullptr;
	if (off || ss_no_reserve || !chr_from_gene || layout.val_bytes > 1) return false;
	const char *e_cov = getenv("DROPEST_FUSED_KEYS_MIN_COVERAGE");
	const double min_cov = e_cov ? atof(e_cov) : 0.4;
	if (hot_coverage < min_cov) return false;
	const SsPlan plan = ss_plan(n_reads, chr_from_gene, layout.val_bytes);
	if (!plan.applicable || !plan.reserve) return false;
	const u32 n = u32(n_reads);
	const bool vec = ((uintptr_t(umi_key_column()) | uintptr_t(d_gene) | uintptr_t(d_aux)) & 15u) == 0;
	if (!vec) return false;
	const int fb1 = plan.fb1, fb2 = plan.fb2, ms = layout.mark_shift, VB = layout.val_bytes;
	const u32 F1 = 1u << fb1, Ff = 1u << fb2, F2 = F1 * Ff;
	if (F1 > KS_MAXF) return false;
	uint64_t os_max = plan.os;
	if (const char *e = getenv("DROPEST_SSORT_OS")) os_max = uint64_t(std::max(1, atoi(e)));
	const u32 os = u32(std::max<uint64_t>(1, std::min<uint64_t>(os_max, uint64_t(n) / (uint64_t(F2) * 2))));
	const u32 n_sample = F2 * os;
	const u32 lds_genes = with_stats && !getenv("DROPEST_NO_LDS_GENE_TABLE") ? std::min<u32>((ingest.gene_max_plus1 + 3u) & ~3u, BK_LDS_GENES_MAX) : 0u;
	const size_t lds = ks_dynamic_lds(lds_genes);
	const size_t span = size_t(plan.span);
	const size_t val_words = (span * size_t(VB) + 3) / 4 + 1;
	keys_a.ensure(span); keys_b.ensure(span); vals_a.ensure(val_words); vals_b.ensure(val_words);
	const CbHot hot{hot_key.p, hot_slot.p, n_hot};
	ss_sample_a.ensure(n_sample); ss_sample_b.ensure(n_sample); ss_fine.ensure(F2); ss_coarse.ensure(F1);
	timed("ss_sample", double(n_sample) * (20.0 / 16 * 8 + 8), [&] {
		if (rpack.on()) hipLaunchKernelGGL(ss_sample_reads_kernel<true>, dim3(div_up(n_sample, 256)), dim3(256), 0, stream, umi_key_column(), d_gene, d_aux, slot.p, n, table, layout, hot, rpack, n_sample, ss_sample_a.p);
		else hipLaunchKernelGGL(ss_sample_reads_kernel<false>, dim3(div_up(n_sample, 256)), dim3(256), 0, stream, umi_key_column(), d_gene, d_aux, slot.p, n, table, layout, hot, rpack, n_sample, ss_sample_a.p);
	});
	const int key_bits = layout.cell_bits + layout.gene_bits + layout.umi_bits;
	ss_splitters_from_sample(n_sample, os, Ff, F2, key_bits >= 64 ? ~0ull : ((1ull << key_bits) - 1ull));
	const u32 cap1 = u32(plan.cap1), CS1 = 32;
	ss_cursors.ensure(size_t(F1) * CS1 + F2); ks_flag.ensure(1);
	HIP_CHECK(hipMemsetAsync(ss_cursors.p, 0, (size_t(F1) * CS1 + F2) * 4, stream));
	HIP_CHECK(hipMemsetAsync(ks_flag.p, 0, 4, stream));
	d_counters.ensure(1);
	GlobalCounters init{};
	init.key_and = ~0ull;
	HIP_CHECK(hipMemcpyAsync(d_counters.p, &init, sizeof(init), hipMemcpyHostToDevice, stream));
	if (with_stats) {
		IngestStats zero{};
		zero.umi_clean_min = ~0ull;
		zero.gene_chr_conflict = ingest.gene_chr_conflict;
		HIP_CHECK(hipMemcpyAsync(d_ingest.p, &zero, sizeof(zero), hipMemcpyHostToDevice, stream));
	}
	int cus = 0, dev = 0;
	HIP_CHECK(hipGetDevice(&dev));
	HIP_CHECK(hipDeviceGetAttribute(&cus, hipDeviceAttributeMultiprocessorCount, dev));
	const SsReserve r1{ss_cursors.p, CS1, cap1, 0u, ks_flag.p, 0u};
	bool launched = true;
	timed("build_keys+L1", double(n) * (8 + 4 + 4 + 4 + 4 + 8 + VB), [&] {
		auto go = [&](auto kernel) {
			if (hipFuncSetAttribute(reinterpret_cast<const void *>(kernel), hipFuncAttributeMaxDynamicSharedMemorySize, int(lds)) != hipSuccess) { (void)hipGetLastError(); launched = false; return; }
			const u32 blocks = std::max<u32>(1u, std::min<u32>(div_up(n, u32(KS_TILE)), u32(std::max(1, cus))));
			hipLaunchKernelGGL(kernel, dim3(blocks), dim3(KS_T), lds, stream, umi_key_column(), d_gene, d_aux, slot.p, n, table, layout, d_counters.p, hot, gene_chr.p, GENE_CHR_CAP, d_ingest.p,
			                   lds_genes, rpack, keys_b.p, reinterpret_cast<uint8_t *>(vals_b.p), ms, fb1, ss_coarse.p, r1);
		};
		auto pick = [&](auto vb) {
			constexpr int V = decltype(vb)::value;
			const int mode = with_stats ? (lds_genes ? 2 : 1) : 0;
			if (rpack.on()) { if (mode == 2) go(build_keys_scatter_kernel<V, 2, true>); else if (mode == 1) go(build_keys_scatter_kernel<V, 1, true>); else go(build_keys_scatter_kernel<V, 0, true>); }
			else { if (mode == 2) go(build_keys_scatter_kernel<V, 2, false>); else if (mode == 1) go(build_keys_scatter_kernel<V, 1, false>); else go(build_keys_scatter_kernel<V, 0, false>); }
		};
		if (VB == 0) pick(std::integral_constant<int, 0>{}); else pick(std::integral_constant<int, 1>{});
	});
	if (!launched) return false;
	fetch(&counters, d_counters.p, sizeof(counters));
	if (with_stats) {
		IngestStats exact{};
		fetch(&exact, d_ingest.p, sizeof(exact));
		exact.cb_escape_count = ingest.cb_escape_count;
		exact.overflow = 0;
		ingest = exact;
	}
	keys_in_l1 = true;
	return true;
}

void dropest_ctx::build_keys(bool with_stats, bool allow_fused) {
	keys_in_l1 = false;
	if (allow_fused && build_keys_fused(with_stats)) return;
	const u32 n = u32(n_reads);
	const size_t span = std::max<size_t>(n, ss_no_reserve ? 0 : size_t(ss_plan(n_reads, chr_from_gene, layout.val_bytes).span));
	const size_t val_words = (span * size_t(layout.val_bytes) + 3) / 4 + 1;
	keys_a.ensure(span); keys_b.ensure(span); vals_a.ensure(val_words); vals_b.ensure(val_words);
	d_counters.ensure(1);
	GlobalCounters init{};
	init.key_and = ~0ull;
	HIP_CHECK(hipMemcpyAsync(d_counters.p, &init, sizeof(init), hipMemcpyHostToDevice, stream));
	if (with_stats) {
		IngestStats zero{};
		zero.umi_clean_min = ~0ull;
		zero.gene_chr_conflict = ingest.gene_chr_conflict;
		HIP_CHECK(hipMemcpyAsync(d_ingest.p, &zero, sizeof(zero), hipMemcpyHostToDevice, stream));
	}
	const bool vec = ((uintptr_t(umi_key_column()) | uintptr_t(d_gene) | uintptr_t(d_aux)) & 15u) == 0;
	timed("build_keys", double(n) * (8 + 4 + 4 + 4 + 4 + 8 + layout.val_bytes), [&] {
		void *v = vals_a.p;
		const CbHot hot{hot_key.p, hot_slot.p, n_hot};
		int cus = 0, dev = 0;
		HIP_CHECK(hipGetDevice(&dev));
		HIP_CHECK(hipDeviceGetAttribute(&cus, hipDeviceAttributeMultiprocessorCount, dev));
		const u32 lds_genes = with_stats && !getenv("DROPEST_NO_LDS_GENE_TABLE") ? std::min<u32>((ingest.gene_max_plus1 + 3u) & ~3u, BK_LDS_GENES_MAX) : 0u;
		auto go = [&](auto kernel, u32 lds = 0u) {
			int per_cu = 0;
			HIP_CHECK(hipOccupancyMaxActiveBlocksPerMultiprocessor(&per_cu, kernel, 256, lds));
			const u32 blocks = std::max<u32>(1u, std::min<u32>(div_up(n, 256 * 4), u32(std::max(1, cus) * std::max(1, std::min(per_cu, 4)))));
			hipLaunchKernelGGL(kernel, dim3(blocks), dim3(256), lds, stream, umi_key_column(), d_gene, d_aux, slot.p, n, table, layout, keys_a.p, v, d_counters.p, hot,
			                   gene_chr.p, GENE_CHR_CAP, d_ingest.p, lds, rpack);
		};
		if (rpack.on() && !vec) throw InvalidError("internal: packed exchange records that are not 16-byte aligned");
		auto pick = [&](auto vb) {
			constexpr int VB = decltype(vb)::value;
			if (rpack.on()) {
				if (with_stats && lds_genes) { if (n_hot) go(build_keys_kernel<256, VB, true, true, true, true, true>, lds_genes); else go(build_keys_kernel<256, VB, true, false, true, true, true>, lds_genes); }
				else if (with_stats) { if (n_hot) go(build_keys_kernel<256, VB, true, true, true, false, true>); else go(build_keys_kernel<256, VB, true, false, true, false, true>); }
				else { if (n_hot) go(build_keys_kernel<256, VB, true, true, false, false, true>); else go(build_keys_kernel<256, VB, true, false, false, false, true>); }
			} else if (with_stats && lds_genes && vec) {
				if (n_hot) go(build_keys_kernel<256, VB, true, true, true, true>, lds_genes); else go(build_keys_kernel<256, VB, true, false, true, true>, lds_genes);
			} else if (with_stats) {
				if (n_hot) { if (vec) go(build_keys_kernel<256, VB, true, true, true>); else go(build_keys_kernel<256, VB, false, true, true>); }
				else { if (vec) go(build_keys_kernel<256, VB, true, false, true>); else go(build_keys_kernel<256, VB, false, false, true>); }
			} else {
				if (n_hot) { if (vec) go(build_keys_kernel<256, VB, true, true>); else go(build_keys_kernel<256, VB, false, true>); }
				else { if (vec) go(build_keys_kernel<256, VB, true>); else go(build_keys_kernel<256, VB, false>); }
			}
		};
		if (layout.val_bytes == 0) pick(std::integral_constant<int, 0>{});
		else if (layout.val_bytes == 1) pick(std::integral_constant<int, 1>{});
		else pick(std::integral_constant<int, 4>{});
	});
	fetch(&counters, d_counters.p, sizeof(counters));
	if (with_stats) {
		IngestStats exact{};
		fetch(&exact, d_ingest.p, sizeof(exact));
		exact.cb_escape_count = ingest.cb_escape_count;
		exact.overflow = 0;
		ingest = exact;
	}
}

static constexpr int RS_T = 512, RS_I = 16, RS_TILE_REC = RS_T * RS_I;
template <int T, int I, bool PF, int VB, int RB = 8>
static void rs_launch_shape(dim3 grid, hipStream_t st, const u64 *k, const void *v, u64 *ok, void *ov, u32 n, int shift, u32 tpb,
                            const u32 *hist, const u32 *base) {
	static_assert(RS_TILE_REC % (T * I) == 0, "shape must tile the histogram ranges");
	hipLaunchKernelGGL((rs_scatter_kernel_t<T, I, PF, VB, RB>), grid, dim3(T), 0, st, k, v, ok, ov, n, shift, tpb * u32(RS_TILE_REC / (T * I)), hist, base);
}
static int rs_shape_override() {
	static const int shape = [] { const char *e = getenv("DROPEST_RS_SHAPE"); return e ? atoi(e) : -1; }();
	return shape;
}
template <int VB>
static void rs_launch_vb(int shape, dim3 grid, hipStream_t st, const u64 *k, const void *v, u64 *ok, void *ov, u32 n, int shift, u32 tpb,
                         const u32 *hist, const u32 *base) {
	switch (shape) {
		case 1: return rs_launch_shape<512, 8, true, VB>(grid, st, k, v, ok, ov, n, shift, tpb, hist, base);
		case 2: return rs_launch_shape<512, 8, false, VB>(grid, st, k, v, ok, ov, n, shift, tpb, hist, base);
		case 3: return rs_launch_shape<256, 8, false, VB>(grid, st, k, v, ok, ov, n, shift, tpb, hist, base);
		case 4: return rs_launch_shape<512, 4, false, VB>(grid, st, k, v, ok, ov, n, shift, tpb, hist, base);
		case 5: return rs_launch_shape<1024, 4, false, VB>(grid, st, k, v, ok, ov, n, shift, tpb, hist, base);
		case 6: return rs_launch_shape<256, 16, false, VB>(grid, st, k, v, ok, ov, n, shift, tpb, hist, base);
		case 7: return rs_launch_shape<1024, 8, false, VB>(grid, st, k, v, ok, ov, n, shift, tpb, hist, base);
		default: return rs_launch_shape<512, 16, true, VB>(grid, st, k, v, ok, ov, n, shift, tpb, hist, base);
	}
}
static void rs_launch(int val_bytes, int bits, dim3 grid, hipStream_t st, const u64 *k, const void *v, u64 *ok, void *ov, u32 n, int shift, u32 tpb,
                      const u32 *hist, const u32 *base) {
	if (bits == 9) {
		if (val_bytes == 0) return rs_launch_shape<512, 8, false, 0, 9>(grid, st, k, v, ok, ov, n, shift, tpb, hist, base);
		if (val_bytes == 1) return rs_launch_shape<512, 8, false, 1, 9>(grid, st, k, v, ok, ov, n, shift, tpb, hist, base);
		return rs_launch_shape<512, 16, true, 4, 9>(grid, st, k, v, ok, ov, n, shift, tpb, hist, base);
	}
	const int o = rs_shape_override();
	if (val_bytes == 0) rs_launch_vb<0>(o >= 0 ? o : 2, grid, st, k, v, ok, ov, n, shift, tpb, hist, base);
	else if (val_bytes == 1) rs_launch_vb<1>(o >= 0 ? o : 2, grid, st, k, v, ok, ov, n, shift, tpb, hist, base);
	else rs_launch_vb<4>(o >= 0 ? o : 0, grid, st, k, v, ok, ov, n, shift, tpb, hist, base);
}

struct RadixPass { int shift, bits; };
static constexpr u32 RS_RADIX_MAX = 512;
static std::vector<RadixPass> plan_radix_passes(u64 varying_mask) {
	std::vector<RadixPass> plain, wide;
	if (!varying_mask) return plain;
	const int lo = __builtin_ctzll(varying_mask), hi = 64 - __builtin_clzll(varying_mask), width = hi - lo;
	for (int shift = lo; shift < 64; shift += 8)
		if ((varying_mask >> shift) & 0xFFull) plain.push_back({shift, 8});
	static const bool allow_wide = getenv("DROPEST_RS_NO_WIDE") == nullptr;
	const int passes = (width + 8) / 9, n9 = width - 8 * passes;
	static const int max_wide = [] { const char *e = getenv("DROPEST_RS_WIDE_MAX"); return e ? atoi(e) : 64; }();
	if (!allow_wide || n9 < 1 || n9 > max_wide || size_t(passes) >= plain.size()) return plain;
	int shift = lo;
	for (int i = 0; i < passes; ++i) { const int bits = i >= passes - n9 ? 9 : 8; wide.push_back({shift, bits}); shift += bits; }
	return wide;
}

void dropest_ctx::scan_counts(const u32 *in, u32 *out, u32 n, u32 *total_out) {
	if (n <= 16384 || n > 1024u * 1024u) {
		hipLaunchKernelGGL(scan_small_kernel, dim3(1), dim3(1024), 0, stream, in, out, n, total_out);
		return;
	}
	const u32 n_chunks = div_up(n, 1024);
	scan_chunk.ensure(1024);
	hipLaunchKernelGGL(ss_chunk_sums_kernel<1024>, dim3(n_chunks), dim3(1024), 0, stream, in, n, scan_chunk.p);
	hipLaunchKernelGGL(ss_prefix_kernel<1024>, dim3(n_chunks), dim3(1024), 0, stream, in, n, scan_chunk.p, n_chunks, out, total_out);
}

void dropest_ctx::radix_sort(u64 *&keys, u32 *&vals, u64 *&keys_alt, u32 *&vals_alt, u32 n, u64 varying_mask, int val_bytes,
                             const char *stat_prefix) {
	if (n == 0) return;
	const u32 n_tiles = div_up(n, RS_TILE_REC);
	u32 nblocks = std::min<u32>(n_tiles, 1024);
	const u32 tpb = div_up(n_tiles, nblocks);
	nblocks = div_up(n_tiles, tpb);
	rs_hist.ensure(size_t(RS_RADIX_MAX) * nblocks); rs_row_total.ensure(RS_RADIX_MAX); rs_digit_base.ensure(RS_RADIX_MAX);
	const std::string scatter_s = std::string(stat_prefix ? stat_prefix : "") +
	                              (val_bytes == 4 ? "rs_scatter" : (val_bytes == 1 ? "rs_scatter:key+1B" : "rs_scatter:keys"));
	const std::string hist_s = std::string(stat_prefix ? stat_prefix : "") + "rs_hist", scan_s = std::string(stat_prefix ? stat_prefix : "") + "rs_scan";
	const char *scatter_name = scatter_s.c_str();
	for (const RadixPass &ps : plan_radix_passes(varying_mask)) {
		const int shift = ps.shift;
		const u32 radix = 1u << ps.bits;
		timed(hist_s.c_str(), double(n) * 8, [&] {
			if (ps.bits == 9) hipLaunchKernelGGL(rs_hist_kernel<9>, dim3(nblocks), dim3(RS_THREADS), 0, stream, keys, n, shift, tpb, u32(RS_TILE_REC), rs_hist.p);
			else hipLaunchKernelGGL(rs_hist_kernel<8>, dim3(nblocks), dim3(RS_THREADS), 0, stream, keys, n, shift, tpb, u32(RS_TILE_REC), rs_hist.p);
		});
		timed(scan_s.c_str(), double(radix) * nblocks * 8, [&] {
			hipLaunchKernelGGL(rs_scan_rows_kernel, dim3(radix), dim3(256), 0, stream, rs_hist.p, nblocks, rs_row_total.p);
			if (ps.bits == 9) hipLaunchKernelGGL(rs_scan_totals_kernel<512>, dim3(1), dim3(512), 0, stream, rs_row_total.p, rs_digit_base.p);
			else hipLaunchKernelGGL(rs_scan_totals_kernel<256>, dim3(1), dim3(256), 0, stream, rs_row_total.p, rs_digit_base.p);
		});
		timed(scatter_name, double(n) * 2 * (8 + val_bytes), [&] {
			rs_launch(val_bytes, ps.bits, dim3(nblocks), stream, keys, vals, keys_alt, vals_alt, n, shift, tpb, rs_hist.p, rs_digit_base.p);
		});
		std::swap(keys, keys_alt);
		std::swap(vals, vals_alt);
	}
}

static std::mutex g_lds_order_mu;
static std::map<int, bool> g_lds_order_known;
static void lds_atomics_mark_unordered(int device) {
	std::lock_guard<std::mutex> lk(g_lds_order_mu);
	g_lds_order_known[device] = false;
	fprintf(stderr, "[dropest_amd] device %d: a bucket came out of its LDS sort unsorted behind the one-atomic ranking; the finishing sort ranks with ballots from now on (slower, same results)\n", device);
}
static bool lds_atomics_lane_ordered(int device, hipStream_t stream) {
	std::mutex &mu = g_lds_order_mu;
	std::map<int, bool> &known = g_lds_order_known;
	std::lock_guard<std::mutex> lk(mu);
	auto it = known.find(device);
	if (it != known.end()) return it->second;
	if (getenv("DROPEST_SS_BALLOT_RANK")) return known[device] = false;
	const u32 rounds = 256;
	std::vector<u32> h(size_t(rounds) * 64), got(size_t(rounds) * 64);
	u32 x = 2463534242u;
	for (u32 r = 0; r < rounds; ++r) {
		const u32 nd = 1u + r % 64u;
		for (u32 l = 0; l < 64; ++l) { x ^= x << 13; x ^= x >> 17; x ^= x << 5; h[size_t(r) * 64 + l] = (x >> 8) % nd; }
	}
	DevBuf<u32> d_in, d_out;
	d_in.alloc(h.size()); d_out.alloc(h.size());
	HIP_CHECK(hipMemcpyAsync(d_in.p, h.data(), h.size() * 4, hipMemcpyHostToDevice, stream));
	hipLaunchKernelGGL(ss_lds_order_probe_kernel, dim3(1), dim3(64), 0, stream, d_in.p, rounds, d_out.p);
	HIP_CHECK(hipGetLastError());
	HIP_CHECK(hipMemcpyAsync(got.data(), d_out.p, got.size() * 4, hipMemcpyDeviceToHost, stream));
	HIP_CHECK(stream_wait(stream));
	bool ordered = true;
	for (u32 r = 0; r < rounds && ordered; ++r) {
		u32 seen[64] = {0};
		for (u32 l = 0; l < 64; ++l) { const u32 d = h[size_t(r) * 64 + l]; if (got[size_t(r) * 64 + l] != seen[d]) ordered = false; ++seen[d]; }
	}
	if (!ordered) fprintf(stderr, "[dropest_amd] device %d: LDS atomics of one instruction are not applied in lane order here; the finishing sort of the splitter sort ranks with ballots (slower, same results)\n", device);
	return known[device] = ordered;
}

bool dropest_ctx::splitter_sort_reduce() {
	const u32 n = u32(n_reads);
	const SsPlan plan = ss_plan(n_reads, chr_from_gene, layout.val_bytes);
	if (!plan.applicable) return false;
	const int tb = plan.tb, fb1 = plan.fb1, fb2 = plan.fb2;
	const bool wide = fb2 > 9;
	const u32 F1 = 1u << fb1, Ff = 1u << fb2, F2 = F1 * Ff;
	const int ms = layout.mark_shift, VB = layout.val_bytes;
	(void)tb;
	uint64_t os_max = plan.os;
	if (const char *e = getenv("DROPEST_SSORT_OS")) os_max = uint64_t(std::max(1, atoi(e)));
	const u32 os = u32(std::max<uint64_t>(1, std::min<uint64_t>(os_max, uint64_t(n) / (uint64_t(F2) * 2))));
	const u32 n_sample = F2 * os;
	const u64 order_mask = ~((1ull << ms) - 1ull);
	const u64 varying = (counters.key_or ^ counters.key_and) & order_mask;
	const bool reserve = plan.reserve && !ss_no_reserve && keys_a.n >= plan.span && keys_b.n >= plan.span &&
	                     (!VB || (vals_a.bytes() >= plan.span && vals_b.bytes() >= plan.span));
	const size_t span = reserve ? size_t(plan.span) : size_t(n);

	HostStage hs(this, "splitter_sort");
	u64 *keys = keys_a.p, *keys_alt = keys_b.p;
	uint8_t *vals = reinterpret_cast<uint8_t *>(vals_a.p), *vals_alt = reinterpret_cast<uint8_t *>(vals_b.p);

	const bool in_l1 = keys_in_l1 && reserve;
	if (keys_in_l1 && !reserve) throw InvalidError("internal: keys partitioned by the key pass, but the sort does not place by reservation");
	const bool rebase = VB == 1 && ms == 0 && reserve && !in_l1 && !getenv("DROPEST_SS_NO_REBASE");
	const int VB2 = rebase ? 0 : VB, ms2 = rebase ? 3 : ms;
	const u64 rebase_mask = rebase ? ~((1ull << layout.umi_bits) - 1ull) : 0ull;
	if (!in_l1) {
		ss_sample_a.ensure(n_sample); ss_sample_b.ensure(n_sample); ss_fine.ensure(F2); ss_coarse.ensure(F1);
		timed("ss_sample", double(n_sample) * 16, [&] {
			hipLaunchKernelGGL(ss_sample_kernel, dim3(div_up(n_sample, 256)), dim3(256), 0, stream, keys, n, ms, n_sample, ss_sample_a.p);
		});
		ss_splitters_from_sample(n_sample, os, Ff, F2, varying >> ms);
	}

	const u32 n_tiles = div_up(n, SS_TILE);
	u32 nblocks = std::min<u32>(n_tiles, 1024);
	const u32 tpb = div_up(n_tiles, nblocks);
	nblocks = div_up(n_tiles, tpb);
	const u32 parts = std::max<u32>(1, std::min<u32>(16, 2048 / F1));
	ss_bucket_base.ensure(F2); ss_bucket_cnt.ensure(F2); scalars.ensure(16);
	HIP_CHECK(hipMemsetAsync(scalars.p, 0, 16, stream));
	u32 max_cnt = 0;
	static const u32 SMALL_MAX = [] { const char *e = getenv("DROPEST_SS_SMALL_MAX"); return e && atoi(e) >= 256 && atoi(e) <= 2048 ? u32(atoi(e)) : 2048u; }();
	const bool atomic_rank = lds_atomics_lane_ordered(cfg.device, stream);
	ss_tmp.ensure(span * 2 + 2); ss_n_loc.ensure(F2); ss_prefix.ensure(F2); ss_chunk.ensure(1024);
	SsLocalArgs a{};
	a.keys = keys; a.vals = vals; a.bucket_base = ss_bucket_base.p; a.bucket_cnt = ss_bucket_cnt.p; a.n_buckets = F2; a.ms = ms2;
	if (rebase) { a.rebase_coarse = ss_coarse.p; a.rebase_mask = rebase_mask; a.rebase_div = Ff; }
	a.t_key = keys_alt; a.t_reads = ss_tmp.p; a.t_agg = ss_tmp.p + span; a.n_loc = ss_n_loc.p;
	if (const char *e = getenv("DROPEST_SS_DEBUG")) a.debug = u32(atoi(e));
	a.order_flag = scalars.p + 2;
	a.atomic_below = u32(ms2 + layout.umi_bits);
	if (const char *e = getenv("DROPEST_SS_ATOMIC_BELOW")) a.atomic_below = u32(atoi(e));
	a.cap = SMALL_MAX; a.skip_above = SMALL_MAX;
	const bool fused_cg_off = getenv("DROPEST_SS_NO_FUSED_CG") != nullptr;
	const bool fuse_cg = !fused_cg_off;
	cg_from_sort = false;
	if (fuse_cg) {
		ss_cg_loc.ensure(F2); ss_cg_cnt.ensure(F2); ss_cg_prefix.ensure(F2);
		HIP_CHECK(hipMemsetAsync(ss_cg_loc.p, 0, size_t(F2) * 4, stream));
		a.cg_loc = ss_cg_loc.p; a.cg_shift = ms2 + layout.umi_bits;
	}
	auto launch_small = [&] {
		static const int wave_mode = [] { const char *e = getenv("DROPEST_SS_LOCAL_WAVE"); return e ? atoi(e) : 0; }();
		if ((wave_mode == 64 || wave_mode == 128) && atomic_rank) {
			const size_t lds1 = ss_local_lds_bytes(a.cap, wave_mode);
			timed(VB2 ? "ss_local:key+1B" : "ss_local:keys", double(n) * (8 + VB2), [&] {
				if (wave_mode == 64) { if (VB2) hipLaunchKernelGGL((ss_local_wave_kernel<64, 1, true>), dim3(F2), dim3(64), lds1, stream, a); else hipLaunchKernelGGL((ss_local_wave_kernel<64, 0, true>), dim3(F2), dim3(64), lds1, stream, a); }
				else { if (VB2) hipLaunchKernelGGL((ss_local_wave_kernel<128, 1, true>), dim3(F2), dim3(128), lds1, stream, a); else hipLaunchKernelGGL((ss_local_wave_kernel<128, 0, true>), dim3(F2), dim3(128), lds1, stream, a); }
			});
			return;
		}
		const size_t lds = ss_local_lds_bytes(a.cap, 256);
		timed(VB2 ? "ss_local:key+1B" : "ss_local:keys", double(n) * (8 + VB2), [&] {
			if (atomic_rank) { if (VB2) hipLaunchKernelGGL((ss_local_kernel<1, true>), dim3(F2), dim3(256), lds, stream, a); else hipLaunchKernelGGL((ss_local_kernel<0, true>), dim3(F2), dim3(256), lds, stream, a); }
			else if (VB2) hipLaunchKernelGGL(ss_local_kernel<1>, dim3(F2), dim3(256), lds, stream, a);
			else hipLaunchKernelGGL(ss_local_kernel<0>, dim3(F2), dim3(256), lds, stream, a);
		});
	};
	if (reserve) {
		const u32 cap1 = u32(plan.cap1), cap2 = u32(plan.cap2), CS1 = 32;
		ss_cursors.ensure(size_t(F1) * CS1 + F2);
		if (!in_l1) HIP_CHECK(hipMemsetAsync(ss_cursors.p, 0, (size_t(F1) * CS1 + F2) * 4, stream));
		else HIP_CHECK(hipMemcpyAsync(scalars.p + 3, ks_flag.p, 4, hipMemcpyDeviceToDevice, stream));
		u32 *cur1 = ss_cursors.p, *cur2 = ss_cursors.p + size_t(F1) * CS1;
		const u32 probe = [] { const char *e = getenv("DROPEST_SS_PROBE"); return e ? u32(atoi(e)) : 0u; }();
		const bool no256 = getenv("DROPEST_SS_NO_F256") != nullptr;
		const u32 rebase_bits = [] { const char *e = getenv("DROPEST_SS_REBASE_BITS"); return e ? u32(std::min(61, std::max(1, atoi(e)))) : 61u; }();
		const SsReserve r1{cur1, CS1, cap1, 0u, scalars.p + 3, probe, rebase_bits}, r2{cur2, 1u, cap2, 0u, scalars.p + 3, probe, 61u};
		if (!in_l1) timed(VB ? "ss_scatter:L1:key+1B" : "ss_scatter:L1:keys", double(n) * (8 + VB + 8 + VB2), [&] {
			auto go = [&](auto kernel) { hipLaunchKernelGGL(kernel, dim3(nblocks), dim3(SS_T), 0, stream, keys, vals, keys_alt, vals_alt, n, ms, fb1, ss_coarse.p, tpb, r1, rebase_mask); };
			if (rebase) { if (wide) go(ss_scatter_res_l1_kernel<1, 1024, true>); else if (fb1 <= 8 && !no256) go(ss_scatter_res_l1_kernel<1, 256, true>); else go(ss_scatter_res_l1_kernel<1, 512, true>); }
			else if (wide) { if (VB) go(ss_scatter_res_l1_kernel<1, 1024>); else go(ss_scatter_res_l1_kernel<0, 1024>); }
			else if (fb1 <= 8 && !no256) { if (VB) go(ss_scatter_res_l1_kernel<1, 256>); else go(ss_scatter_res_l1_kernel<0, 256>); }
			else { if (VB) go(ss_scatter_res_l1_kernel<1, 512>); else go(ss_scatter_res_l1_kernel<0, 512>); }
		});
		timed(VB2 ? "ss_scatter:L2:key+1B" : "ss_scatter:L2:keys", double(n) * 2 * (8 + VB2), [&] {
			auto go = [&](auto kernel) { hipLaunchKernelGGL(kernel, dim3(F1 * parts), dim3(SS_T), 0, stream, keys_alt, vals_alt, keys, vals, ms2, fb2, ss_fine.p, cur1, CS1, cap1, parts, r2,
			                                                 rebase ? ss_coarse.p : static_cast<const u64 *>(nullptr), rebase_mask); };
			if (wide) { if (VB2) go(ss_scatter_res_l2_kernel<1, 1024>); else go(ss_scatter_res_l2_kernel<0, 1024>); }
			else if (fb2 <= 8 && !no256) { if (VB2) go(ss_scatter_res_l2_kernel<1, 256>); else go(ss_scatter_res_l2_kernel<0, 256>); }
			else { if (VB2) go(ss_scatter_res_l2_kernel<1, 512>); else go(ss_scatter_res_l2_kernel<0, 512>); }
		});
		timed("ss_scan", double(F2) * 12, [&] {
			hipLaunchKernelGGL(ss_res_buckets_kernel, dim3(div_up(F2, 256)), dim3(256), 0, stream, cur2, F2, cap2, ss_bucket_base.p, ss_bucket_cnt.p, scalars.p);
		});
		launch_small();
		u32 head[4] = {0, 0, 0, 0};
		fetch(head, scalars.p, 16);
		max_cnt = head[0];
		if (head[3]) {
			stats["count:ss_reserve_overflow"].launches += 1;
			ss_no_reserve = true;
			build_keys(false);
			return splitter_sort_reduce();
		}
		if (max_cnt > SS_LOCAL_MAX) { build_keys(false, false); return false; }
	} else {
	rs_hist.ensure(size_t(F1) * nblocks); rs_row_total.ensure(1024); ss_base1.ensure(F1 + 1);
	timed("ss_hist:L1", double(n) * 8, [&] {
		if (wide) hipLaunchKernelGGL(ss_hist_l1_kernel<1024>, dim3(nblocks), dim3(SS_T), 0, stream, keys, n, ms, fb1, ss_coarse.p, tpb, rs_hist.p);
		else hipLaunchKernelGGL(ss_hist_l1_kernel<512>, dim3(nblocks), dim3(SS_T), 0, stream, keys, n, ms, fb1, ss_coarse.p, tpb, rs_hist.p);
	});
	timed("ss_scan", double(F1) * nblocks * 8, [&] {
		hipLaunchKernelGGL(rs_scan_rows_kernel, dim3(F1), dim3(256), 0, stream, rs_hist.p, nblocks, rs_row_total.p);
		if (wide) hipLaunchKernelGGL(ss_scan_totals_kernel<1024>, dim3(1), dim3(1024), 0, stream, rs_row_total.p, F1, n, ss_base1.p);
		else hipLaunchKernelGGL(ss_scan_totals_kernel<512>, dim3(1), dim3(512), 0, stream, rs_row_total.p, F1, n, ss_base1.p);
	});
	timed(VB ? "ss_scatter:L1:key+1B" : "ss_scatter:L1:keys", double(n) * 2 * (8 + VB), [&] {
		auto go = [&](auto kernel) { hipLaunchKernelGGL(kernel, dim3(nblocks), dim3(SS_T), 0, stream, keys, vals, keys_alt, vals_alt, n, ms, fb1, ss_coarse.p, tpb, rs_hist.p, ss_base1.p); };
		if (wide) { if (VB) go(ss_scatter_l1_kernel<1, 1024>); else go(ss_scatter_l1_kernel<0, 1024>); }
		else { if (VB) go(ss_scatter_l1_kernel<1, 512>); else go(ss_scatter_l1_kernel<0, 512>); }
	});

	ss_cnt2.ensure(size_t(F2) * parts);
	timed("ss_hist:L2", double(n) * 8, [&] {
		if (wide) hipLaunchKernelGGL(ss_hist_l2_kernel<1024>, dim3(F1 * parts), dim3(SS_T), 0, stream, keys_alt, ms, fb2, ss_fine.p, ss_base1.p, parts, ss_cnt2.p);
		else hipLaunchKernelGGL(ss_hist_l2_kernel<512>, dim3(F1 * parts), dim3(SS_T), 0, stream, keys_alt, ms, fb2, ss_fine.p, ss_base1.p, parts, ss_cnt2.p);
	});
	timed("ss_scan", double(F2) * parts * 8, [&] {
		if (wide) hipLaunchKernelGGL(ss_scan_seg_kernel<1024>, dim3(F1), dim3(1024), 0, stream, ss_cnt2.p, Ff, parts, ss_base1.p, ss_bucket_base.p, ss_bucket_cnt.p, scalars.p);
		else hipLaunchKernelGGL(ss_scan_seg_kernel<512>, dim3(F1), dim3(512), 0, stream, ss_cnt2.p, Ff, parts, ss_base1.p, ss_bucket_base.p, ss_bucket_cnt.p, scalars.p);
	});
	fetch(&max_cnt, scalars.p, 4);
	if (max_cnt > SS_LOCAL_MAX) return false;
	timed(VB ? "ss_scatter:L2:key+1B" : "ss_scatter:L2:keys", double(n) * 2 * (8 + VB), [&] {
		auto go = [&](auto kernel) { hipLaunchKernelGGL(kernel, dim3(F1 * parts), dim3(SS_T), 0, stream, keys_alt, vals_alt, keys, vals, ms, fb2, ss_fine.p, ss_base1.p, parts, ss_cnt2.p); };
		if (wide) { if (VB) go(ss_scatter_l2_kernel<1, 1024>); else go(ss_scatter_l2_kernel<0, 1024>); }
		else { if (VB) go(ss_scatter_l2_kernel<1, 512>); else go(ss_scatter_l2_kernel<0, 512>); }
	});
	}

	if (!reserve) launch_small();
	if (max_cnt > SMALL_MAX) {
		std::vector<u32> cnts(F2), medium, big;
		fetch(cnts.data(), ss_bucket_cnt.p, size_t(F2) * 4);
		for (u32 b = 0; b < F2; ++b) if (cnts[b] > SMALL_MAX) (cnts[b] <= 4096 ? medium : big).push_back(b);
		ss_big_list.ensure(medium.size() + big.size());
		if (!medium.empty()) HIP_CHECK(hipMemcpyAsync(ss_big_list.p, medium.data(), medium.size() * 4, hipMemcpyHostToDevice, stream));
		if (!big.empty()) HIP_CHECK(hipMemcpyAsync(ss_big_list.p + medium.size(), big.data(), big.size() * 4, hipMemcpyHostToDevice, stream));
		auto launch = [&](auto kernel, u32 threads, u32 cap, const u32 *list, size_t count) {
			SsLocalArgs g = a;
			g.big_list = list; g.cap = cap; g.skip_above = cap;
			const size_t lds = ss_local_lds_bytes(cap, int(threads));
			HIP_CHECK(hipFuncSetAttribute(reinterpret_cast<const void *>(kernel), hipFuncAttributeMaxDynamicSharedMemorySize, int(lds)));
			hipLaunchKernelGGL(kernel, dim3(u32(count)), dim3(threads), lds, stream, g);
		};
		timed("ss_local:big", 0, [&] {
			if (atomic_rank) {
				if (!medium.empty()) { if (VB2) launch(ss_local_big_kernel<256, 1, true>, 256, 4096, ss_big_list.p, medium.size()); else launch(ss_local_big_kernel<256, 0, true>, 256, 4096, ss_big_list.p, medium.size()); }
				if (!big.empty()) { if (VB2) launch(ss_local_big_kernel<512, 1, true>, 512, SS_LOCAL_MAX, ss_big_list.p + medium.size(), big.size()); else launch(ss_local_big_kernel<512, 0, true>, 512, SS_LOCAL_MAX, ss_big_list.p + medium.size(), big.size()); }
			} else {
				if (!medium.empty()) { if (VB2) launch(ss_local_big_kernel<256, 1>, 256, 4096, ss_big_list.p, medium.size()); else launch(ss_local_big_kernel<256, 0>, 256, 4096, ss_big_list.p, medium.size()); }
				if (!big.empty()) { if (VB2) launch(ss_local_big_kernel<512, 1>, 512, SS_LOCAL_MAX, ss_big_list.p + medium.size(), big.size()); else launch(ss_local_big_kernel<512, 0>, 512, SS_LOCAL_MAX, ss_big_list.p + medium.size(), big.size()); }
			}
		});
		HIP_CHECK(stream_wait(stream));
	}
	const u32 n_chunks = div_up(F2, 1024);
	timed("ss_scan", double(F2) * 12, [&] {
		hipLaunchKernelGGL(ss_chunk_sums_kernel<1024>, dim3(n_chunks), dim3(1024), 0, stream, ss_n_loc.p, F2, ss_chunk.p);
		hipLaunchKernelGGL(ss_prefix_kernel<1024>, dim3(n_chunks), dim3(1024), 0, stream, ss_n_loc.p, F2, ss_chunk.p, n_chunks, ss_prefix.p, scalars.p + 1);
		if (fuse_cg) {
			hipLaunchKernelGGL(ss_cg_counts_kernel, dim3(div_up(F2, 256)), dim3(256), 0, stream, ss_bucket_base.p, ss_n_loc.p, keys_alt, layout.umi_bits, F2, ss_cg_loc.p, ss_cg_cnt.p);
			hipLaunchKernelGGL(ss_chunk_sums_kernel<1024>, dim3(n_chunks), dim3(1024), 0, stream, ss_cg_cnt.p, F2, ss_chunk.p);
			hipLaunchKernelGGL(ss_prefix_kernel<1024>, dim3(n_chunks), dim3(1024), 0, stream, ss_cg_cnt.p, F2, ss_chunk.p, n_chunks, ss_cg_prefix.p, scalars.p + 4);
		}
	});
	u32 total_flag[4] = {0, 0, 0, 0};
	fetch(total_flag, scalars.p + 1, 16);
	if (total_flag[1]) {
		if (atomic_rank) lds_atomics_mark_unordered(cfg.device);
		stats["count:ss_order_violation"].launches += 1;
		build_keys(false, false);
		return false;
	}
	const u32 total = total_flag[0];
	n_mol = total;
	for (auto it = pending.rbegin(); it != pending.rend(); ++it)
		if (it->name.compare(0, 10, "ss_local:k") == 0) { it->bytes += double(n_mol) * 16; break; }
	mol_key.ensure(size_t(n_mol) + 1);
	for (DevBuf<u32> *b : {&mol_reads, &mol_mark, &mol_exon, &mol_intron}) b->ensure(size_t(n_mol) + 1);
	SsCompactArgs c{};
	c.bucket_base = ss_bucket_base.p; c.n_loc = ss_n_loc.p; c.prefix = ss_prefix.p; c.n_buckets = F2;
	c.t_key = keys_alt; c.t_reads = ss_tmp.p; c.t_agg = ss_tmp.p + span;
	c.mol_key = mol_key.p; c.mol_reads = mol_reads.p; c.mol_mark = mol_mark.p; c.mol_exon = mol_exon.p; c.mol_intron = mol_intron.p;
	if (fuse_cg) {
		n_cg = total_flag[3];
		cg_key.ensure(size_t(n_cg) + 1); cg_mol_begin.ensure(size_t(n_cg) + 1);
		for (DevBuf<u32> *b : {&cg_n_all, &cg_n_req, &cg_reads_all, &cg_reads_req, &cg_exon, &cg_intron}) b->ensure(size_t(n_cg) + 1);
		SsCompactCgArgs g{};
		g.bucket_base = ss_bucket_base.p; g.n_loc = ss_n_loc.p; g.prefix = ss_prefix.p; g.cg_loc = ss_cg_loc.p; g.cg_cnt = ss_cg_cnt.p; g.cg_prefix = ss_cg_prefix.p;
		g.n_buckets = F2; g.t_key = keys_alt; g.t_reads = ss_tmp.p; g.t_agg = ss_tmp.p + span;
		g.mol_key = mol_key.p; g.mol_reads = mol_reads.p; g.mol_mark = mol_mark.p; g.mol_exon = mol_exon.p; g.mol_intron = mol_intron.p;
		g.cg_key = cg_key.p; g.cg_mol_begin = cg_mol_begin.p;
		g.out[0] = cg_n_all.p; g.out[1] = cg_n_req.p; g.out[2] = cg_reads_all.p; g.out[3] = cg_reads_req.p; g.out[4] = cg_exon.p; g.out[5] = cg_intron.p;
		g.umi_bits = layout.umi_bits; g.query_mask = query_mask; g.n_cg = n_cg;
		if (const char *e = getenv("DROPEST_CG_DBG")) g.dbg = u32(atoi(e));
		timed("ss_compact:cell_gene", double(n_mol) * (16 + 24) + double(n_cg) * 36, [&] {
			hipLaunchKernelGGL(ss_cg_zero_borders_kernel, dim3(div_up(F2, 256)), dim3(256), 0, stream, g);
			hipLaunchKernelGGL(ss_compact_cg_kernel<false>, dim3(div_up(F2, 4)), dim3(256), 0, stream, g);
		});
		HIP_CHECK(hipMemcpyAsync(cg_mol_begin.p + n_cg, &n_mol, 4, hipMemcpyHostToDevice, stream));
		cg_from_sort = true;
	} else
	timed("ss_compact", double(n_mol) * (16 + 24), [&] {
		hipLaunchKernelGGL(ss_compact_kernel, dim3(div_up(F2, 4)), dim3(256), 0, stream, c);
	});
	for (DevBuf<u32> *b : {&mol_reads, &mol_mark, &mol_exon, &mol_intron}) HIP_CHECK(hipMemsetAsync(b->p + n_mol, 0, 4, stream));
	main_sort_passes = 3; main_sort_kind = 1;
	return true;
}

template <class P>
static u32 seg_reduce_grid(u32 tiles) {
	static const u32 resident = [] {
		int dev = 0, cus = 0, per_cu = 0;
		HIP_CHECK(hipGetDevice(&dev));
		HIP_CHECK(hipDeviceGetAttribute(&cus, hipDeviceAttributeMultiprocessorCount, dev));
		HIP_CHECK(hipOccupancyMaxActiveBlocksPerMultiprocessor(&per_cu, seg_reduce_kernel<P>, SR_THREADS, 0));
		return u32(std::max(1, cus) * std::max(1, per_cu));
	}();
	return std::max<u32>(1u, std::min(tiles, resident));
}

template <class P, class Prep>
static u32 run_segmented_reduce(dropest_ctx &c, const char *tag, P &policy, u32 n, double bytes_per_row, Prep &&prepare,
                                double out_bytes_per_run = 0) {
	if (n == 0) {
		prepare(0);
		if constexpr (!P::DIRECT) for (int ch = 0; ch < P::NV; ++ch) if (policy.out[ch]) HIP_CHECK(hipMemsetAsync(policy.out[ch], 0, 4, c.stream));
		return 0;
	}
	const u32 tiles = div_up(n, SR_THREADS * P::ITEMS);
	c.tile_counts.ensure(tiles); c.tile_prefix.ensure(tiles); c.scalars.ensure(16);
	const std::string n_count = std::string("seg_count:") + tag, n_reduce = std::string("seg_reduce:") + tag;
	c.timed(n_count.c_str(), double(n) * 8, [&] {
		hipLaunchKernelGGL(seg_count_kernel<P>, dim3(tiles), dim3(SR_THREADS), 0, c.stream, policy, n, c.tile_counts.p);
	});
	c.timed("scan_small", double(tiles) * 8, [&] {
		c.scan_counts(c.tile_counts.p, c.tile_prefix.p, tiles, c.scalars.p);
	});
	u32 total = 0;
	c.fetch(&total, c.scalars.p, 4);
	prepare(total);
	if constexpr (!P::DIRECT) {
		hipLaunchKernelGGL(seg_zero_borders_kernel<P>, dim3(div_up(tiles, 256)), dim3(256), 0, c.stream, policy, c.tile_prefix.p, tiles, total);
	}
	c.timed(n_reduce.c_str(), double(n) * bytes_per_row + double(total) * out_bytes_per_run, [&] {
		hipLaunchKernelGGL(seg_reduce_kernel<P>, dim3(seg_reduce_grid<P>(tiles)), dim3(SR_THREADS), 0, c.stream, policy, n, c.tile_prefix.p);
	});
	return total;
}

static void zero_async(dropest_ctx &c, void *p, size_t bytes) { HIP_CHECK(hipMemsetAsync(p, 0, bytes, c.stream)); }
struct ZeroArrays { uint32_t *p[8]; uint32_t n_arrays; };
__global__ __launch_bounds__(256) void zero_arrays_kernel(ZeroArrays a, size_t words) {
	const size_t quads = words / 4;
	for (uint32_t k = 0; k < a.n_arrays; ++k) {
		uint4 *q = reinterpret_cast<uint4 *>(a.p[k]);
		for (size_t i = size_t(blockIdx.x) * 256 + threadIdx.x; i < quads; i += size_t(gridDim.x) * 256) q[i] = make_uint4(0, 0, 0, 0);
		if (blockIdx.x == 0 && threadIdx.x < words - quads * 4) a.p[k][quads * 4 + threadIdx.x] = 0;
	}
}

void dropest_ctx::reduce_all() {
	const u32 n = u32(n_reads);
	u64 *keys = keys_a.p, *keys_alt = keys_b.p;
	u32 *vals = vals_a.p, *vals_alt = vals_b.p;
	const u64 order_mask = ~((1ull << layout.mark_shift) - 1ull);
	const u64 varying = (counters.key_or ^ counters.key_and) & order_mask;
	if (splitter_sort_reduce()) {
		n_chr_rows = 0;
		if (!cg_from_sort) reduce_molecules_to_cell_gene();
		reduce_cell_gene_to_cells();
		HIP_CHECK(stream_wait(stream));
		return;
	}
	main_sort_passes = u32(plan_radix_passes(varying).size()); main_sort_kind = 0;
	radix_sort(keys, vals, keys_alt, vals_alt, n, varying, layout.val_bytes);

	if (chr_from_gene) {
		auto run = [&](auto &p) {
			p.keys = keys;
			n_mol = run_segmented_reduce(*this, "molecules", p, n, 8 + layout.val_bytes, [&](u32 total) {
				mol_key.ensure(total + 1);
				for (DevBuf<u32> *b : {&mol_reads, &mol_mark, &mol_exon, &mol_intron}) b->ensure(total + 1);
				p.mol_key = mol_key.p; p.out[0] = mol_reads.p; p.out[1] = mol_mark.p; p.out[2] = mol_exon.p; p.out[3] = mol_intron.p;
			}, 24);
		};
		if (layout.val_bytes == 0) { ReadsToMoleculesX<0> p{}; run(p); }
		else { ReadsToMoleculesX<1> p{}; p.marks = reinterpret_cast<const uint8_t *>(vals); run(p); }
		n_chr_rows = 0;
	} else {
		{
			ReadsToMolecules p{};
			p.keys = keys; p.vals = vals;
			n_mol = run_segmented_reduce(*this, "molecules", p, n, 12, [&](u32 total) {
				mol_key.ensure(total + 1); mol_reads.ensure(total + 1); mol_mark.ensure(total + 1);
				p.mol_key = mol_key.p; p.out[0] = mol_reads.p; p.out[1] = mol_mark.p;
			}, 16);
		}
		{
			ReadsToChrRows p{};
			p.keys = keys; p.vals = vals;
			p.cell_shift = layout.gene_bits + layout.umi_bits; p.umi_bits = layout.umi_bits; p.gene_mask = layout.gene_none;
			n_chr_rows = run_segmented_reduce(*this, "chr_rows", p, n, 12 + 2, [&](u32 total) {
				chr_row_key.ensure(total + 1); chr_exon.ensure(total + 1); chr_intron.ensure(total + 1); chr_inter.ensure(total + 1);
				p.row_key = chr_row_key.p; p.out[0] = chr_exon.p; p.out[1] = chr_intron.p; p.out[2] = chr_inter.p;
			});
		}
	}
	reduce_molecules_to_cell_gene();
	reduce_cell_gene_to_cells();
	HIP_CHECK(stream_wait(stream));
}

void dropest_ctx::reduce_molecules_to_cell_gene() {
	auto prepare_common = [&](u32 total) {
		cg_key.ensure(total + 1); cg_mol_begin.ensure(total + 1);
		for (DevBuf<u32> *b : {&cg_n_all, &cg_n_req, &cg_reads_all, &cg_reads_req}) b->ensure(total + 1);
	};
	if (chr_from_gene) {
		MoleculesToCellGeneX p{};
		p.mol_key = mol_key.p; p.mol_reads = mol_reads.p; p.mol_mark = mol_mark.p; p.mol_exon = mol_exon.p; p.mol_intron = mol_intron.p;
		p.umi_bits = layout.umi_bits; p.query_mask = query_mask;
		n_cg = run_segmented_reduce(*this, "cell_gene", p, n_mol, 24, [&](u32 total) {
			prepare_common(total);
			for (DevBuf<u32> *b : {&cg_exon, &cg_intron}) b->ensure(total + 1);
			p.cg_key = cg_key.p; p.cg_mol_begin = cg_mol_begin.p;
			p.out[0] = cg_n_all.p; p.out[1] = cg_n_req.p; p.out[2] = cg_reads_all.p; p.out[3] = cg_reads_req.p;
			p.out[4] = cg_exon.p; p.out[5] = cg_intron.p;
		}, 36);
	} else {
		MoleculesToCellGene p{};
		p.mol_key = mol_key.p; p.mol_reads = mol_reads.p; p.mol_mark = mol_mark.p;
		p.umi_bits = layout.umi_bits; p.query_mask = query_mask;
		n_cg = run_segmented_reduce(*this, "cell_gene", p, n_mol, 16, [&](u32 total) {
			prepare_common(total);
			p.cg_key = cg_key.p; p.cg_mol_begin = cg_mol_begin.p;
			p.out[0] = cg_n_all.p; p.out[1] = cg_n_req.p; p.out[2] = cg_reads_all.p; p.out[3] = cg_reads_req.p;
		}, 28);
	}
	HIP_CHECK(hipMemcpyAsync(cg_mol_begin.p + n_cg, &n_mol, 4, hipMemcpyHostToDevice, stream));
}

void dropest_ctx::reduce_cell_gene_to_cells() {
	CellGeneToCells p{};
	p.cg_key = cg_key.p; p.n_all = cg_n_all.p; p.n_req = cg_n_req.p; p.reads_all = cg_reads_all.p;
	p.gene_bits = layout.gene_bits; p.gene_mask = layout.gene_none;
	const size_t nc = size_t(n_cells) + 1;
	cell_cg_begin.ensure(nc); cell_cg_count.ensure(nc); cell_n_genes.ensure(nc); cell_req_genes.ensure(nc);
	cell_req_umis.ensure(nc); cell_total_umis.ensure(nc); cell_total_reads.ensure(nc);
	{
		ZeroArrays z{};
		for (DevBuf<u32> *b : {&cell_cg_begin, &cell_cg_count, &cell_n_genes, &cell_req_genes, &cell_req_umis, &cell_total_umis, &cell_total_reads})
			z.p[z.n_arrays++] = b->p;
		hipLaunchKernelGGL(zero_arrays_kernel, dim3(u32(std::min<size_t>(div_up(u32(std::min<size_t>(nc / 4 + 1, 0xFFFFFFFFull)), 256u), 2048u))), dim3(256), 0, stream, z, nc);
		HIP_CHECK(hipGetLastError());
	}
	p.cell_cg_begin = cell_cg_begin.p;
	p.out[0] = cell_n_genes.p; p.out[1] = cell_req_genes.p; p.out[2] = cell_req_umis.p;
	p.out[3] = cell_total_umis.p; p.out[4] = cell_total_reads.p; p.out[5] = cell_cg_count.p;
	if (n_cg == 0) return;
	const u32 tiles = div_up(n_cg, SR_THREADS * CellGeneToCells::ITEMS);
	timed("seg_reduce:cells", double(n_cg) * (24 + 4), [&] {
		hipLaunchKernelGGL(seg_reduce_kernel<CellGeneToCells>, dim3(seg_reduce_grid<CellGeneToCells>(tiles)), dim3(SR_THREADS), 0, stream, p, n_cg,
		                   static_cast<const u32 *>(nullptr));
	});
}

void dropest_ctx::fetch_real_cells(bool at_init) {
	invalidate_prefetch();
	real.clear(); real_list_current = false;
	if (n_cells == 0) return;
	DevBuf<u32> &list = real_list; list.ensure(n_cells);
	scalars.ensure(16);
	const u32 tiles = div_up(n_cells, RC_TILE);
	tile_counts.ensure(tiles); tile_prefix.ensure(tiles);
	timed("flag_real", double(n_cells) * 8, [&] {
		hipLaunchKernelGGL(count_real_kernel, dim3(tiles), dim3(RC_THREADS), 0, stream, cell_n_genes.p, n_cells, min_before, tile_counts.p);
		scan_counts(tile_counts.p, tile_prefix.p, tiles, scalars.p);
		hipLaunchKernelGGL(write_real_kernel, dim3(tiles), dim3(RC_THREADS), 0, stream, cell_n_genes.p, n_cells, min_before,
		                   tile_prefix.p, list.p);
	});
	tail_mark("fetch_real_cells: flag kernels enqueued", true);
	u32 count = 0;
	fetch(&count, scalars.p, 4);
	tail_mark("count fetched");
	if (count == 0) return;
	DevBuf<CellRowPod> &rows = real_rows_dev; rows.ensure(count);
	CellArrays a{cell_cb.p, cell_first.p, cell_n_genes.p, cell_req_genes.p, cell_req_umis.p, cell_total_umis.p, cell_total_reads.p};
	timed("gather_cell_rows", double(count) * 72, [&] {
		hipLaunchKernelGGL(gather_cell_rows_kernel, dim3(div_up(count, 256)), dim3(256), 0, stream, a, list.p, 0u, count, rows.p);
	});
	const size_t row_bytes = size_t(count) * sizeof(CellRowPod), id_off = (row_bytes + 15) & ~size_t(15);
	h_stage.ensure(id_off + size_t(count) * 4);
	HIP_CHECK(hipMemcpyAsync(h_stage.p, rows.p, row_bytes, hipMemcpyDeviceToHost, stream));
	HIP_CHECK(hipMemcpyAsync(h_stage.p + id_off, list.p, size_t(count) * 4, hipMemcpyDeviceToHost, stream));
	HIP_CHECK(stream_wait(stream));
	tail_mark("rows on the host");
	const CellRowPod *host_rows = reinterpret_cast<const CellRowPod *>(h_stage.p);
	const u32 *ids = reinterpret_cast<const u32 *>(h_stage.p + id_off);
	if (at_init && auto_pf_form >= 0 && n_reads && merge_phase_changes_nothing() && (auto_pf_form != 1 || narrow_possible()))
		prefetch_raw_matrix(auto_pf_reads, auto_pf_form, host_rows, ids, count);
	tail_mark("prefetch enqueued");
	real.resize(count);
	parallel_ranges(count, [&](size_t b, size_t e, unsigned) {
		for (size_t i = b; i < e; ++i) {
			HostCell &h = real[i];
			h.id = ids[i];
			h.row = host_rows[i];
			h.merged = h.excluded = false;
		}
	});
	real_list_current = true;
	real_pristine = true;
	tail_mark("host mirror filled");
}

void dropest_ctx::request_filtered(u32 genes_threshold, int max_cells) {
	filtered_threshold = genes_threshold; filtered_max_cells = max_cells; filtered_valid = false;
	strategy_targets = StrategyTargets();
	n_real_now = 0;
	constexpr unsigned W = dropest::HostPool::MAX;
	uint64_t part[W + 1] = {0};
	const unsigned workers = parallel_ranges(real.size(), [&](size_t b, size_t e, unsigned w) {
		uint64_t c = 0;
		for (size_t i = b; i < e; ++i) { const HostCell &h = real[i]; c += (!h.merged && !h.excluded && h.row.n_genes >= min_before); }
		part[w] = c;
	}, 100000, W);
	for (unsigned w = 0; w < workers; ++w) n_real_now += part[w];
}

const std::vector<uint64_t> &dropest_ctx::filtered_cells() {
	if (!filtered_valid) { HostStage hs(this, "sort_filtered"); sort_filtered(filtered_threshold, filtered_max_cells); }
	return filtered;
}

void dropest_ctx::sort_filtered(u32 genes_threshold, int max_cells) {
	auto passes = [&](const HostCell &h) {
		return !(h.merged || h.excluded || h.row.n_genes < min_before) && h.row.requested_genes >= genes_threshold;
	};
	size_t device_min = 100000;
	if (const char *e = getenv("DROPEST_DEVICE_SORT_MIN")) device_min = size_t(std::max(1, atoi(e)));

	const size_t R = real.size();
	if (R >= device_min && R < 0x50000000ull && real_pristine && real_list_current && genes_threshold == 0 && !getenv("DROPEST_SORTF_HOST")) {
		HostStage st(this, "sort_filtered:device_only");
		const u32 m = u32(R);
		sort_cols.ensure(size_t(m) * 3); scalars64.ensure(8);
		keys_a.ensure(m); keys_b.ensure(m); vals_a.ensure(m); vals_b.ensure(m);
		u64 init[8] = {0, ~0ull, 0, ~0ull, 0, ~0ull, 64, 0};
		HIP_CHECK(hipMemcpyAsync(scalars64.p, init, sizeof(init), hipMemcpyHostToDevice, stream));
		u64 *d_code = sort_cols.p, *d_umis = sort_cols.p + m, *d_sizes = sort_cols.p + 2 * size_t(m);
		hipLaunchKernelGGL(sortf_columns_kernel, dim3(std::min<u32>(div_up(m, 256), 2048u)), dim3(256), 0, stream, real_rows_dev.p, m, d_code, d_umis, d_sizes, scalars64.p);
		HIP_CHECK(hipGetLastError());
		u64 st8[8];
		fetch(st8, scalars64.p, sizeof(st8));
		if (st8[6] == st8[7] && !(st8[0] & ESCAPE_BIT)) {
			u64 *k = keys_a.p, *k_alt = keys_b.p;
			u32 *v = vals_a.p, *v_alt = vals_b.p;
			hipLaunchKernelGGL(iota_kernel, dim3(div_up(m, 256)), dim3(256), 0, stream, v, m);
			HIP_CHECK(hipMemcpyAsync(k, d_code, size_t(m) * 8, hipMemcpyDeviceToDevice, stream));
			radix_sort(k, v, k_alt, v_alt, m, st8[0] ^ st8[1]);
			const std::pair<const u64 *, u64> more[2] = {{d_umis, st8[2] ^ st8[3]}, {d_sizes, st8[4] ^ st8[5]}};
			for (auto const &nx : more) {
				hipLaunchKernelGGL(gather_u64_kernel, dim3(div_up(m, 256)), dim3(256), 0, stream, nx.first, v, m, k);
				HIP_CHECK(hipGetLastError());
				radix_sort(k, v, k_alt, v_alt, m, nx.second);
			}
			sort_stage.ensure((size_t(m) * 3 + 1) / 2 + 1);
			u32 *out = reinterpret_cast<u32 *>(sort_stage.p);
			hipLaunchKernelGGL(sortf_out_kernel, dim3(std::min<u32>(div_up(m, 256), 2048u)), dim3(256), 0, stream, v, real_rows_dev.p, real_list.p, m, out);
			HIP_CHECK(hipGetLastError());
			HIP_CHECK(stream_wait(stream));
			size_t start = 0;
			if (max_cells > 0 && size_t(max_cells) < size_t(m)) start = size_t(m) - size_t(max_cells);
			filtered.resize(m - start); filtered_ridx.resize(m - start); filtered_umis.resize(m - start);
			parallel_ranges(m - start, [&](size_t b, size_t e, unsigned) {
				for (size_t i = b; i < e; ++i) { filtered[i] = out[start + i]; filtered_ridx[i] = out[size_t(m) + start + i]; filtered_umis[i] = int32_t(out[2 * size_t(m) + start + i]); }
			});
			filtered_valid = true;
			return;
		}
	}
	if (R >= device_min) {
		constexpr unsigned W = dropest::HostPool::MAX;
		auto st1 = std::make_unique<HostStage>(this, "sort_filtered:scan");
		size_t count[W] = {0};
		u64 any[W] = {0}; int bl[W]; bool uniform[W];
		for (unsigned w = 0; w < W; ++w) { bl[w] = -1; uniform[w] = true; }
		const unsigned workers = parallel_ranges(R, [&](size_t b, size_t e, unsigned w) {
			size_t c = 0; u64 a = 0; int l0 = -1; bool uni = true;
			for (size_t i = b; i < e; ++i) {
				const HostCell &h = real[i];
				if (!passes(h)) continue;
				++c;
				a |= h.row.barcode;
				const int l = bit_length(h.row.barcode);
				if (l0 < 0) l0 = l; else if (l != l0) uni = false;
			}
			count[w] = c; any[w] = a; bl[w] = l0; uniform[w] = uni;
		}, 100000, W);
		size_t m64 = 0; u64 any_all = 0; int bl_all = -1; bool device_sort = true;
		size_t offset[W + 1];
		for (unsigned w = 0; w < workers; ++w) {
			offset[w] = m64; m64 += count[w]; any_all |= any[w];
			if (count[w]) { if (bl_all < 0) bl_all = bl[w]; device_sort &= uniform[w] && bl[w] == bl_all; }
		}
		if (m64 >= device_min && m64 < 0x50000000ull && device_sort && !(any_all & ESCAPE_BIT)) {
			const u32 m = u32(m64);
			st1.reset();
			auto st2 = std::make_unique<HostStage>(this, "sort_filtered:fill");
			sort_stage.ensure(size_t(m) * 3);
			sort_cols.ensure(size_t(m) * 3);
			sort_idx.resize(m); sort_ids.resize(m);
			keys_a.ensure(m); keys_b.ensure(m); vals_a.ensure(m); vals_b.ensure(m);
			u64 *h_code = sort_stage.p, *h_umis = sort_stage.p + m, *h_sizes = sort_stage.p + 2 * size_t(m);
			u64 o[W][3], a[W][3];
			parallel_ranges(R, [&](size_t b, size_t e, unsigned w) {
				u64 lo[3] = {0, 0, 0}, la[3] = {~0ull, ~0ull, ~0ull};
				size_t at = offset[w];
				for (size_t i = b; i < e; ++i) {
					const HostCell &h = real[i];
					if (!passes(h)) continue;
					const u64 sizes = (u64(h.row.requested_genes) << 32) | h.row.requested_umis;
					const u64 umis = u64(size_t(h.row.total_umis));
					h_code[at] = h.row.barcode; h_umis[at] = umis; h_sizes[at] = sizes; sort_idx[at] = u32(i); sort_ids[at] = h.id;
					lo[0] |= h.row.barcode; la[0] &= h.row.barcode; lo[1] |= umis; la[1] &= umis; lo[2] |= sizes; la[2] &= sizes;
					++at;
				}
				for (int c = 0; c < 3; ++c) { o[w][c] = lo[c]; a[w][c] = la[c]; }
			}, 100000, W);
			u64 vary[3];
			for (int c = 0; c < 3; ++c) {
				u64 oo = 0, aa = ~0ull;
				for (unsigned w = 0; w < workers; ++w) if (count[w]) { oo |= o[w][c]; aa &= a[w][c]; }
				vary[c] = oo ^ aa;
			}
			st2.reset();
			auto st3 = std::make_unique<HostStage>(this, "sort_filtered:device");
			{ HostStage sx(this, "sort_filtered:device:h2d");
			hipLaunchKernelGGL(load_u64_from_host_kernel, dim3(std::min<u32>(div_up(m * 3u, 256), 4096u)), dim3(256), 0, stream, sort_stage.p, m * 3u, sort_cols.p);
			HIP_CHECK(hipGetLastError()); }
			auto sx2 = std::make_unique<HostStage>(this, "sort_filtered:device:sorts");
			const u64 *d_code = sort_cols.p, *d_umis = sort_cols.p + m, *d_sizes = sort_cols.p + 2 * size_t(m);
			u64 *k = keys_a.p, *k_alt = keys_b.p;
			u32 *v = vals_a.p, *v_alt = vals_b.p;
			hipLaunchKernelGGL(iota_kernel, dim3(div_up(m, 256)), dim3(256), 0, stream, v, m);
			HIP_CHECK(hipMemcpyAsync(k, d_code, size_t(m) * 8, hipMemcpyDeviceToDevice, stream));
			radix_sort(k, v, k_alt, v_alt, m, vary[0]);
			const std::pair<const u64 *, u64> more[2] = {{d_umis, vary[1]}, {d_sizes, vary[2]}};
			for (auto const &nx : more) {
				hipLaunchKernelGGL(gather_u64_kernel, dim3(div_up(m, 256)), dim3(256), 0, stream, nx.first, v, m, k);
				HIP_CHECK(hipGetLastError());
				radix_sort(k, v, k_alt, v_alt, m, nx.second);
			}
			sx2.reset();
			u32 *perm = reinterpret_cast<u32 *>(sort_stage.p);
			HostStage sx3(this, "sort_filtered:device:d2h");
			hipLaunchKernelGGL(store_u32_to_host_kernel, dim3(std::min<u32>(div_up(m, 256), 2048u)), dim3(256), 0, stream, v, m, perm);
			HIP_CHECK(hipGetLastError());
			HIP_CHECK(stream_wait(stream));
			st3.reset();
			HostStage st4(this, "sort_filtered:gather");
			size_t start = 0;
			if (max_cells > 0 && size_t(max_cells) < size_t(m)) start = size_t(m) - size_t(max_cells);
			filtered.resize(m - start); filtered_ridx.resize(m - start); filtered_umis.resize(m - start);
			parallel_ranges(m - start, [&](size_t b, size_t e, unsigned) {
				for (size_t i = b; i < e; ++i) { const u32 at = perm[start + i]; filtered[i] = sort_ids[at]; filtered_ridx[i] = sort_idx[at]; filtered_umis[i] = int32_t(h_umis[at]); }
			});
			filtered_valid = true;
			return;
		}
	}

	struct Key { u64 sizes; u64 umis; u64 code; u32 idx; };
	std::vector<Key> keys;
	auto key_of = [&](u32 i) {
		const HostCell &h = real[i];
		return Key{(u64(h.row.requested_genes) << 32) | h.row.requested_umis,
		           u64(size_t(h.row.total_umis)),
		           h.row.barcode, i};
	};
	if (R >= 200000) {
		constexpr unsigned W = dropest::HostPool::MAX;
		size_t count[W] = {0}, offset[W + 1] = {0};
		const unsigned workers = parallel_ranges(R, [&](size_t b, size_t e, unsigned w) {
			size_t c = 0;
			for (size_t i = b; i < e; ++i) c += passes(real[i]) ? 1 : 0;
			count[w] = c;
		}, 100000, W);
		for (unsigned w = 0; w < workers; ++w) offset[w + 1] = offset[w] + count[w];
		keys.resize(offset[workers]);
		parallel_ranges(R, [&](size_t b, size_t e, unsigned w) {
			size_t at = offset[w];
			for (size_t i = b; i < e; ++i) if (passes(real[i])) keys[at++] = key_of(u32(i));
		}, 100000, W);
	} else {
		keys.reserve(8192);
		for (u32 i = 0; i < real.size(); ++i) if (passes(real[i])) keys.push_back(key_of(i));
	}
	auto less = [&](const Key &a, const Key &b) {
		if (a.sizes != b.sizes) return a.sizes < b.sizes;
		if (a.umis != b.umis) return a.umis < b.umis;
		const bool plain = !((a.code | b.code) & ESCAPE_BIT) && bit_length(a.code) == bit_length(b.code);
		if (plain) return a.code < b.code;
		return barcode_of(real[a.idx]) < barcode_of(real[b.idx]);
	};
	if (keys.size() > 64) {
		u64 o = 0, a = ~0ull;
		for (const Key &k : keys) { o |= k.sizes; a &= k.sizes; }
		const u64 vary = o ^ a;
		std::vector<Key> other(keys.size());
		for (int shift = 0; shift < 64; shift += 8) {
			if (!((vary >> shift) & 0xFFull)) continue;
			size_t cnt[257] = {0};
			for (const Key &k : keys) ++cnt[((k.sizes >> shift) & 0xFFull) + 1];
			for (int d = 0; d < 256; ++d) cnt[d + 1] += cnt[d];
			for (const Key &k : keys) other[cnt[(k.sizes >> shift) & 0xFFull]++] = k;
			keys.swap(other);
		}
		for (size_t i = 0; i < keys.size();) {
			size_t j = i + 1;
			while (j < keys.size() && keys[j].sizes == keys[i].sizes) ++j;
			if (j - i > 1) std::sort(keys.begin() + long(i), keys.begin() + long(j), less);
			i = j;
		}
	} else
		std::sort(keys.begin(), keys.end(), less);
	filtered.clear(); filtered_ridx.clear();
	size_t start = 0;
	if (max_cells > 0 && size_t(max_cells) < keys.size()) start = keys.size() - size_t(max_cells);
	filtered_umis.clear();
	for (size_t i = start; i < keys.size(); ++i) { filtered.push_back(real[keys[i].idx].id); filtered_ridx.push_back(keys[i].idx); filtered_umis.push_back(int32_t(keys[i].umis)); }
	filtered_valid = true;
}

#include "quality.h"
#include "merge_host.h"
#include "merge_shard.h"
#include "umi_merge_host.h"
#include "umi_directional_host.h"
#include "poisson_merge.h"
#include "simple_merge.h"
#include "merge_all.h"
#include "mutate_host.h"
#include "matrix_emit.h"
#include "validation.h"

void dropest_ctx::run_ingest() {
	if (initialized) throw InvalidError("Container is already initialized");
	if (ingested) return;
	HostStage hs_all(this, "ingest");
	concat_chunks();
	ingest = IngestStats{};
	ingest.umi_clean_min = ~0ull;
	forced_table_capacity = 0;
	if (n_reads > 0) {
		{ HostStage hs(this, "cb_table"); build_cb_table(); }
		{ HostStage hs(this, "cell_ids"); assign_cell_ids(); }
	}
	ingested = true;
}

void dropest_ctx::run_set_initialized() {
	if (initialized) throw InvalidError("Container is already initialized");
	{
		uint64_t sample_min = uint64_t(1) << 22;
		if (const char *e = getenv("DROPEST_CB_SAMPLE_MIN")) sample_min = uint64_t(std::max(1ll, atoll(e)));
		lazy_stats = !ingested && n_reads >= sample_min && !getenv("DROPEST_EXACT_INGEST_STATS");
	}
	run_ingest();
	HostStage hs_all(this, "set_initialized");
	if (n_reads > 0) {
		{
			HostStage hs(this, "keys");
			plan_key_layout();
			if (lazy_stats) {
				const KeyLayout planned = layout;
				const bool planned_chr = chr_from_gene, planned_strip = umi_sentinel_stripped;
				const int planned_clean = umi_clean_bits;
				build_keys(true);
				lazy_stats = false;
				plan_key_layout();
				const bool same = planned.umi_bits == layout.umi_bits && planned.gene_bits == layout.gene_bits && planned.cell_bits == layout.cell_bits &&
				                  planned.mark_shift == layout.mark_shift && planned.val_bytes == layout.val_bytes &&
				                  planned.umi_strip_mask == layout.umi_strip_mask && planned.umi_escape_base == layout.umi_escape_base &&
				                  planned.gene_none == layout.gene_none;
				if (!same || planned_chr != chr_from_gene || planned_strip != umi_sentinel_stripped || planned_clean != umi_clean_bits) {
					if (profiling) stats["count:key_plan_redone"].launches += 1;
					build_keys(false);
				}
			} else build_keys();
		}
		{ HostStage hs(this, "sort+reduce"); reduce_all(); }
		accumulate_umi_qualities();
		{ HostStage hs(this, "real_cells"); fetch_real_cells(true); }
	} else {
		plan_key_layout();
	}
	request_filtered(0, -1);
	initialized = true;
	was_split = false;
	if (auto_pf_form >= 0 && n_reads && merge_phase_changes_nothing() && (auto_pf_form != 1 || narrow_possible())) prefetch_raw_matrix(auto_pf_reads, auto_pf_form);
	collect_timings();
}

bool dropest_ctx::merge_phase_changes_nothing() const {
	return cfg.merge_kind == DROPEST_MERGE_NONE && cfg.umi_merge_kind != DROPEST_UMI_MERGE_DIRECTIONAL && ingest.umi_escape_max_plus1 == 0 && !hooks &&
	       !external_merge_done;
}

void dropest_ctx::run_merge_and_filter() {
	if (!initialized) throw InvalidError("You must initialize container");
	if (merged) throw InvalidError("merge_and_filter was already run");
	if (!merge_phase_changes_nothing()) invalidate_prefetch();
	HostStage hs(this, "merge_and_filter");
	tail_mark("merge_and_filter entered");
	if (cfg.merge_kind == DROPEST_MERGE_REAL_BARCODES && n_cells && !external_merge_done) run_cb_merge_real();
	if (cfg.merge_kind == DROPEST_MERGE_POISSON_REAL && n_cells && !external_merge_done) run_cb_merge_real();
	if ((cfg.merge_kind == DROPEST_MERGE_SIMPLE || cfg.merge_kind == DROPEST_MERGE_POISSON_SIMPLE) && n_cells && !external_merge_done) run_cb_merge_simple();
	if (cfg.merge_kind == DROPEST_MERGE_ALL && n_cells && !external_merge_done) run_cb_merge_all();
	if (cfg.umi_merge_kind == DROPEST_UMI_MERGE_DIRECTIONAL) run_umi_merge_directional(); else run_umi_merge_simple();
	request_filtered(min_after, cfg.max_cells);
	merged = true;
	if (auto_pf_form >= 0 && n_reads && !raw_pf.valid && (auto_pf_form != 1 || narrow_possible())) prefetch_raw_matrix(auto_pf_reads, auto_pf_form);
	collect_timings();
}

template <class F>
static void for_each_molecule(dropest_ctx *ctx, const std::vector<u64> &k, const std::vector<u32> &r, const std::vector<u32> &m, F &&emit,
                              u32 first_row = 0) {
	const KeyLayout &L = ctx->layout;
	const u64 umask = L.umi_bits ? ((1ull << L.umi_bits) - 1ull) : 0ull;
	u64 done_group = ~0ull;
	for (size_t i = 0; i < k.size(); ++i) {
		const u64 cg = k[i] >> L.umi_bits;
		const u64 g = cg & L.gene_none;
		if (g == L.gene_none) continue;
		const u32 c = u32(cg >> L.gene_bits);
		if (!ctx->umi_overrides.empty()) {
			auto it = ctx->umi_overrides.find(cg);
			if (it != ctx->umi_overrides.end()) {
				if (done_group != cg) { for (const UmiOverride &o : it->second) emit(c, u32(g), o.umi, o.reads, o.mark, o.src_row); done_group = cg; }
				continue;
			}
		}
		emit(c, u32(g), ctx->unmap_umi(k[i] & umask), r[i], uint8_t(m[i]), first_row + u32(i));
	}
}

extern "C" {

const char *dropest_last_error(void) { return g_last_error.c_str(); }

void dropest_cfg_defaults(dropest_cfg *cfg) {
	std::memset(cfg, 0, sizeof(*cfg));
	cfg->device = 0;
	cfg->merge_kind = DROPEST_MERGE_NONE;
	cfg->barcodes_kind = DROPEST_BARCODES_INDROP;
	cfg->barcodes_file = nullptr;
	cfg->min_genes_before_merge = 10;
	cfg->min_genes_after_merge = 10;
	cfg->min_merge_fraction = 0.2;
	cfg->max_cb_merge_edit_distance = 2;
	cfg->umi_merge_kind = DROPEST_UMI_MERGE_SIMPLE;
	cfg->umi_merge_multiplier = 2.0;
	cfg->max_merge_prob = 1e-4;
	cfg->max_real_merge_prob = 1e-7;
	cfg->max_umi_merge_edit_distance = 1;
	cfg->gene_match_levels = "eEBA";
	cfg->max_cells = -1;
	cfg->cb_table_capacity = 0;
}

dropest_status dropest_ctx_create(const dropest_cfg *cfg, dropest_ctx **out) {
	if (!cfg || !out) { g_last_error = "null argument"; return DROPEST_ERR_INVALID; }
	*out = nullptr;
	return guarded([&] {
		std::unique_ptr<dropest_ctx> c(new dropest_ctx());
		c->init_from_cfg(*cfg);
		*out = c.release();
	});
}

void dropest_ctx_destroy(dropest_ctx *ctx) {
	if (!ctx) return;
	(void)hipSetDevice(ctx->cfg.device);
	delete ctx;
}

dropest_status dropest_set_side_strings(dropest_ctx *ctx, const char *const *strings, uint64_t n) {
	return guarded([&] {
		if (!ctx) throw InvalidError("null context");
		if (n < ctx->side.size()) throw InvalidError("the side-string table may only grow");
		for (uint64_t i = ctx->side.size(); i < n; ++i) ctx->side.emplace_back(strings[i]);
	});
}

static void push_common(dropest_ctx *ctx, uint64_t n) {
	if (!ctx) throw InvalidError("null context");
	if (ctx->initialized) throw InvalidError("Container is already initialized");
	if (ctx->d_cb) throw InvalidError("reads were already frozen by a previous set_initialized");
	if (ctx->n_reads + n >= 0xFFFFFFFEull) throw UnsupportedError("more than 2^32-2 reads in one context (shard across GPUs)");
	HIP_CHECK(hipSetDevice(ctx->cfg.device));
}

dropest_status dropest_push_reads(dropest_ctx *ctx, const uint64_t *cb, const uint64_t *umi, const uint32_t *gene,
                                  const uint32_t *aux, uint64_t n) {
	return guarded([&] {
		push_common(ctx, n);
		if (n == 0) return;
		if (!cb || !umi || !gene || !aux) throw InvalidError("null read array");
		if (ctx->store_chunk >= 0 && size_t(ctx->store_chunk) + 1 != ctx->chunks.size()) {
			ReadChunk c;
			c.cb.alloc(n); c.umi.alloc(n); c.gene.alloc(n); c.aux.alloc(n);
			c.cb.mark_persistent(); c.umi.mark_persistent(); c.gene.mark_persistent(); c.aux.mark_persistent();
			HIP_CHECK(hipMemcpyAsync(c.cb.p, cb, n * 8, hipMemcpyHostToDevice, ctx->stream));
			HIP_CHECK(hipMemcpyAsync(c.umi.p, umi, n * 8, hipMemcpyHostToDevice, ctx->stream));
			HIP_CHECK(hipMemcpyAsync(c.gene.p, gene, n * 4, hipMemcpyHostToDevice, ctx->stream));
			HIP_CHECK(hipMemcpyAsync(c.aux.p, aux, n * 4, hipMemcpyHostToDevice, ctx->stream));
			HIP_CHECK(stream_wait(ctx->stream));
			c.p_cb = c.cb.p; c.p_umi = c.umi.p; c.p_gene = c.gene.p; c.p_aux = c.aux.p; c.n = n;
			ctx->chunks.push_back(std::move(c));
			ctx->n_reads += n;
			return;
		}
		if (ctx->store_chunk < 0) { ctx->store_chunk = long(ctx->chunks.size()); ctx->chunks.emplace_back(); }
		ctx->store.push(cb, umi, gene, aux, n);
		ctx->chunks[size_t(ctx->store_chunk)].n = ctx->store.n;
		ctx->n_reads += n;
	});
}

dropest_status dropest_push_reads_gather(dropest_ctx *ctx, uint64_t n_segments, const uint64_t *const *cb, const uint64_t *const *umi,
                                         const uint32_t *const *gene, const uint32_t *const *aux, const uint64_t *counts) {
	return guarded([&] {
		if (n_segments && (!cb || !umi || !gene || !aux || !counts)) throw InvalidError("null segment array");
		uint64_t n = 0;
		for (uint64_t k = 0; k < n_segments; ++k) { n += counts[k]; if (counts[k] && (!cb[k] || !umi[k] || !gene[k] || !aux[k])) throw InvalidError("null read array"); }
		push_common(ctx, n);
		if (n == 0) return;
		if (ctx->store_chunk >= 0 && size_t(ctx->store_chunk) + 1 != ctx->chunks.size()) throw InvalidError("dropest_push_reads_gather after an adopted device chunk: push the segments one by one");
		if (ctx->store_chunk < 0) { ctx->store_chunk = long(ctx->chunks.size()); ctx->chunks.emplace_back(); }
		ctx->store.push_segments(size_t(n_segments), cb, umi, gene, aux, counts);
		ctx->chunks[size_t(ctx->store_chunk)].n = ctx->store.n;
		ctx->n_reads += n;
	});
}

// ... 876 lines not shown
dropest_status dropest_count_matrix_device(dropest_ctx *ctx, int filtered, int reads_output, uint64_t *ncols, uint64_t *nnz,
                                           const uint32_t **colptr, const uint32_t **d_rowidx, const uint32_t **d_values) {
	return guarded([&] {
		need_init(ctx);
		ctx->emit_matrix(filtered != 0, reads_output != 0, false);
		const dropest_ctx::MatrixResult &M = ctx->mat[filtered ? 0 : 1];
		*ncols = M.ncols; *nnz = M.nnz;
		*colptr = M.colptr.data(); *d_rowidx = M.d_row.p; *d_values = M.d_val.p;
	});
}

dropest_status dropest_cell_first_reads_device(dropest_ctx *ctx, uint64_t *n_cells, const uint32_t **d_first) {
	return guarded([&] { need_init(ctx); *n_cells = ctx->n_cells; *d_first = ctx->cell_first.p; });
}

static void assemble_columns_launch(int device, int slot, uint64_t n_cols, const uint64_t *src_start, const uint64_t *dst_start,
                                    const uint64_t *len, const uint32_t *d_src_rows, const uint32_t *d_src_vals,
                                    uint32_t *d_dst_rows, uint32_t *d_dst_vals) {
	HIP_CHECK(hipSetDevice(device));
	if (n_cols == 0) return;
	static DevBuf<u64> desc_cache[64][2];
	static PinnedBuf<u64> desc_host[64][2];
	if (device < 0 || device >= 64) throw InvalidError("device index out of range");
	if (slot < 0 || slot > 1) throw InvalidError("descriptor slot must be 0 or 1");
	DevBuf<u64> &d_desc = desc_cache[device][slot];
	PinnedBuf<u64> &desc = desc_host[device][slot];
	d_desc.ensure(n_cols * 3 + n_cols / 2); desc.ensure(n_cols * 3);
	for (uint64_t c = 0; c < n_cols; ++c) { desc.p[3 * c] = src_start[c]; desc.p[3 * c + 1] = dst_start[c]; desc.p[3 * c + 2] = len[c]; }
	HIP_CHECK(hipMemcpyAsync(d_desc.p, desc.p, n_cols * 3 * 8, hipMemcpyHostToDevice, nullptr));
	hipLaunchKernelGGL(assemble_columns_kernel, dim3(u32(n_cols)), dim3(256), 0, nullptr, d_desc.p, d_src_rows, d_src_vals,
	                   d_dst_rows, d_dst_vals);
	HIP_CHECK(hipGetLastError());
}

dropest_status dropest_assemble_columns(int device, uint64_t n_cols, const uint64_t *src_start, const uint64_t *dst_start,
                                        const uint64_t *len, const uint32_t *d_src_rows, const uint32_t *d_src_vals,
                                        uint32_t *d_dst_rows, uint32_t *d_dst_vals) {
	return guarded([&] {
		assemble_columns_launch(device, 0, n_cols, src_start, dst_start, len, d_src_rows, d_src_vals, d_dst_rows, d_dst_vals);
		HIP_CHECK(hipDeviceSynchronize());
	});
}

dropest_status dropest_assemble_columns_async(int device, int slot, uint64_t n_cols, const uint64_t *src_start, const uint64_t *dst_start,
                                              const uint64_t *len, const uint32_t *d_src_rows, const uint32_t *d_src_vals,
                                              uint32_t *d_dst_rows, uint32_t *d_dst_vals) {
	return guarded([&] {
		assemble_columns_launch(device, slot, n_cols, src_start, dst_start, len, d_src_rows, d_src_vals, d_dst_rows, d_dst_vals);
	});
}

dropest_status dropest_host_register(int device, void *host, uint64_t bytes, void **d_ptr) {
	return guarded([&] {
		if (!host || !d_ptr) throw InvalidError("null argument");
		HIP_CHECK(hipSetDevice(device));
		HIP_CHECK(hipHostRegister(host, bytes, hipHostRegisterMapped | hipHostRegisterPortable));
		HIP_CHECK(hipHostGetDevicePointer(d_ptr, host, 0));
	});
}

dropest_status dropest_host_unregister(int device, void *host) {
	return guarded([&] {
		HIP_CHECK(hipSetDevice(device));
		HIP_CHECK(hipHostUnregister(host));
	});
}

dropest_status dropest_kernel_stats(dropest_ctx *ctx, uint32_t *n, dropest_kernel_stat *out) {
	return guarded([&] {
		if (!ctx) throw InvalidError("null context");
		ctx->collect_timings();
		u32 i = 0;
		for (auto &kv : ctx->stats) {
			if (out) { out[i].name = kv.first.c_str(); out[i].launches = kv.second.launches; out[i].ms = kv.second.ms; out[i].bytes = kv.second.bytes; }
			++i;
		}
		*n = i;
	});
}

dropest_status dropest_set_profiling(dropest_ctx *ctx, int enabled) {
	return guarded([&] {
		if (!ctx) throw InvalidError("null context");
		ctx->collect_timings();
		ctx->profiling = enabled != 0;
		if (enabled) ctx->stats.clear();
	});
}

dropest_status dropest_radix_plan(uint64_t varying_mask, uint32_t *n_passes, int32_t *shifts, int32_t *bits) {
	return guarded([&] {
		if (!n_passes) throw InvalidError("null argument");
		const std::vector<RadixPass> plan = plan_radix_passes(varying_mask);
		*n_passes = u32(plan.size());
		for (size_t i = 0; i < plan.size(); ++i) { if (shifts) shifts[i] = plan[i].shift; if (bits) bits[i] = plan[i].bits; }
	});
}

dropest_status dropest_table_sizes(dropest_ctx *ctx, uint64_t out[4]) {
	return guarded([&] { need_init(ctx); out[0] = ctx->n_reads; out[1] = ctx->n_cells; out[2] = ctx->n_mol; out[3] = ctx->n_cg; });
}

dropest_status dropest_rand_sequence(uint32_t seed, uint64_t n, int32_t *out) {
	return guarded([&] {
		if (n && !out) throw InvalidError("null argument");
		GlibcRand r(seed);
		for (uint64_t i = 0; i < n; ++i) out[i] = r.next();
	});
}

dropest_status dropest_debug_poison_scratch(uint64_t seed, uint64_t *n_blocks) {
	return guarded([&] {
		HIP_CHECK(hipDeviceSynchronize());
		const size_t d = DevRegistry::get().poison_all(seed), h = PinnedRegistry::get().poison_all(seed);
		if (n_blocks) *n_blocks = d + h;
	});
}

dropest_status dropest_debug_alloc_ordinal(uint64_t *next_ordinal) {
	return guarded([&] { auto &r = DevRegistry::get(); std::lock_guard<std::mutex> lk(r.mu); *next_ordinal = r.next; });
}

dropest_status dropest_debug_alloc_site(uint64_t ordinal, char *out, uint64_t out_bytes) {
	return guarded([&] {
		auto &r = DevRegistry::get();
		std::lock_guard<std::mutex> lk(r.mu);
		std::string text = "unknown (set DROPEST_ALLOC_TRACE=1)";
		for (auto const &s : r.sites) if (s.ordinal == ordinal) text = std::string(s.file) + ":" + std::to_string(s.line) + " " + std::to_string(s.bytes) + " B" + (s.recycled ? " recycled" : " fresh");
		if (out && out_bytes) { std::snprintf(out, size_t(out_bytes), "%s", text.c_str()); }
	});
}

dropest_status dropest_debug_refresh(void) {
	return guarded([&] { dropest::DevDebug::refresh(); });
}

dropest_status dropest_debug_trim_pool(void) {
	return guarded([&] { DevRegistry::get().trim_pool(); });
}

dropest_status dropest_set_profiling_filter(dropest_ctx *ctx, const char *name_prefix) {
	return guarded([&] {
		if (!ctx) throw InvalidError("null context");
		ctx->collect_timings();
		ctx->profile_only = name_prefix ? name_prefix : "";
	});
}

void *dropest_stream(dropest_ctx *ctx) { return ctx ? ctx->stream : nullptr; }

}

#include "shard_run.h"
```

dropest_amd/csrc/k_ssort.h:

```cpp
#pragma once

#include "util.h"

namespace dropest {

constexpr int SS_T = 512, SS_I = 8, SS_TILE = SS_T * SS_I;
constexpr int SS_MAX_F = 512;
constexpr uint32_t SS_LOCAL_MAX = 8192;

__global__ __launch_bounds__(256) void ss_sample_kernel(const unsigned long long *__restrict__ keys, uint32_t n, int ms,
                                                        uint32_t n_sample, unsigned long long *__restrict__ out) {
	const uint32_t j = blockIdx.x * 256 + threadIdx.x;
	if (j >= n_sample) return;
	const uint32_t pos = uint32_t((uint64_t(j) * n + n / 2) / n_sample);
	out[j] = keys[pos < n ? pos : n - 1] >> ms;
}

__global__ __launch_bounds__(256) void ss_pick_splitters_kernel(const unsigned long long *__restrict__ sorted_sample, uint32_t os, uint32_t F, uint32_t F2,
                                                                unsigned long long *__restrict__ fine, unsigned long long *__restrict__ coarse) {
	const uint32_t j = blockIdx.x * 256 + threadIdx.x;
	if (j >= F2) return;
	const unsigned long long v = j + 1 < F2 ? sorted_sample[size_t(j + 1) * os] : ~0ull;
	fine[j] = v;
	if ((j + 1) % F == 0) coarse[(j + 1) / F - 1] = v;
// ... 207 lines not shown
	uint32_t *overflow;
	uint32_t dbg;
	uint32_t rebase_bits;
};
template <int VB, int MAXF, bool REBASE = false>
__device__ inline void ss_scatter_res_range(const unsigned long long *__restrict__ keys, const uint8_t *__restrict__ vals,
                                            unsigned long long *__restrict__ okeys, uint8_t *__restrict__ ovals, uint32_t begin, uint32_t end,
                                            int ms, int fb, const unsigned long long *sp, const SsReserve rs, uint32_t *cnt, uint32_t *tstart,
                                            uint32_t *gdelta, uint32_t *scratch, unsigned long long *sk, uint16_t *sd, uint8_t *sv,
                                            unsigned long long rebase_mask = 0) {
	static_assert(!REBASE || VB == 1, "rebased keys carry the mark byte in their low bits");
	constexpr int PER = (MAXF + SS_T - 1) / SS_T;
	const uint32_t F = 1u << fb, tid = threadIdx.x;
	unsigned long long key[SS_I];
	uint8_t val[VB ? SS_I : 1];
	auto load_tile = [&](uint32_t t0) {
		const uint32_t in_tile = end - t0 < uint32_t(SS_TILE) ? end - t0 : uint32_t(SS_TILE);
#pragma unroll
		for (int i = 0; i < SS_I; ++i) {
			const uint32_t p = i * SS_T + tid;
			key[i] = p < in_tile ? keys[t0 + p] : 0ull;
			if (VB) val[i] = p < in_tile ? vals[t0 + p] : uint8_t(0);
		}
	};
	if (begin < end) load_tile(begin);
	for (uint32_t t0 = begin; t0 < end; t0 += SS_TILE) {
		const uint32_t in_tile = end - t0 < uint32_t(SS_TILE) ? end - t0 : uint32_t(SS_TILE);
		for (uint32_t j = tid; j < F; j += SS_T) cnt[j] = 0;
		lds_barrier();
		uint32_t pos[SS_I], rk[SS_I];
#pragma unroll
		for (int i = 0; i < SS_I; ++i) pos[i] = 0;
		for (int b = fb - 1; b >= 0; --b) {
			const uint32_t step = 1u << b;
#pragma unroll
			for (int i = 0; i < SS_I; ++i) if (sp[pos[i] + step - 1] <= (key[i] >> ms)) pos[i] += step;
		}
		if (rs.dbg & 1u) {
			uint32_t pos2[SS_I];
#pragma unroll
			for (int i = 0; i < SS_I; ++i) pos2[i] = 0;
			for (int b = fb - 1; b >= 0; --b) {
				const uint32_t step = 1u << b;
#pragma unroll
				for (int i = 0; i < SS_I; ++i) if (sp[pos2[i] + step - 1] <= ((key[i] ^ (rs.dbg >> 8)) >> ms)) pos2[i] += step;
			}
#pragma unroll
			for (int i = 0; i < SS_I; ++i) pos[i] = (pos[i] + pos2[i]) >> 1;
		}
#pragma unroll
		for (int i = 0; i < SS_I; ++i) rk[i] = (i * SS_T + tid) < in_tile ? atomicAdd(&cnt[pos[i]], 1u) : 0u;
		lds_barrier();
		uint32_t c[PER], got[PER], mine = 0;
#pragma unroll
		for (int k = 0; k < PER; ++k) {
			const uint32_t e = tid * PER + k;
			c[k] = e < F ? cnt[e] : 0u; mine += c[k];
			got[k] = c[k] ? atomicAdd(&rs.cursor[size_t(rs.first + e) * rs.cstride], c[k]) : 0u;
		}
		uint32_t total;
		uint32_t ex = block_excl_scan_u32<SS_T, true>(mine, scratch, total);
#pragma unroll
		for (int k = 0; k < PER; ++k) {
			const uint32_t e = tid * PER + k;
			if (e < F) tstart[e] = ex;
			ex += c[k];
		}
		lds_barrier();
#pragma unroll
		for (int i = 0; i < SS_I; ++i)
			if ((i * SS_T + tid) < in_tile) {
				const uint32_t q = tstart[pos[i]] + rk[i];
				sk[q] = key[i]; sd[q] = uint16_t(pos[i]);
				if (VB) sv[q] = val[i];
			}
		if (!(rs.dbg & 2u) && t0 + SS_TILE < end) load_tile(t0 + SS_TILE);
#pragma unroll
		for (int k = 0; k < PER; ++k) {
			const uint32_t e = tid * PER + k;
			if (e < F) {
				gdelta[e] = (rs.first + e) * rs.cap + got[k] - tstart[e];
				if (got[k] + c[k] > rs.cap) atomicOr(rs.overflow, 1u);
			}
		}
		lds_barrier();
		for (uint32_t q = tid; q < in_tile; q += SS_T) {
			const uint32_t d = sd[q], g = gdelta[d] + q;
			if (g < (rs.first + d + 1u) * rs.cap) {
				if constexpr (REBASE) {
					const unsigned long long diff = sk[q] - (d ? (sp[d - 1u] & rebase_mask) : 0ull);
					if (diff >> rs.rebase_bits) atomicOr(rs.overflow, 1u);
					okeys[g] = (diff << 3) | (unsigned long long)(sv[q] & 7u);
				} else {
					okeys[g] = sk[q];
					if (VB) ovals[g] = sv[q];
				}
			}
		}
		if ((rs.dbg & 2u) && t0 + SS_TILE < end) load_tile(t0 + SS_TILE);
		lds_barrier();
	}
}

#define SS_SCATTER_RES_LDS(VB, MAXF)                                                                        \
	__shared__ unsigned long long sp[MAXF];                                                                 \
	__shared__ uint32_t cnt[MAXF], tstart[MAXF], gdelta[MAXF], scratch[SS_T / 64 + 1];                      \
	__shared__ unsigned long long sk[SS_TILE];                                                              \
	__shared__ uint16_t sd[SS_TILE];                                                                        \
	__shared__ uint8_t sv[VB ? SS_TILE : 1];

template <int VB, int MAXF, bool REBASE = false>
__global__ __launch_bounds__(SS_T) void ss_scatter_res_l1_kernel(const unsigned long long *__restrict__ keys, const uint8_t *__restrict__ vals,
                                                                 unsigned long long *__restrict__ okeys, uint8_t *__restrict__ ovals, uint32_t n,
                                                                 int ms, int fb, const unsigned long long *__restrict__ coarse,
                                                                 uint32_t tiles_per_block, SsReserve rs, unsigned long long rebase_mask) {
	SS_SCATTER_RES_LDS(VB, MAXF)
	const uint32_t F = 1u << fb;
	for (uint32_t j = threadIdx.x; j < F; j += SS_T) sp[j] = j + 1 < F ? coarse[j] : ~0ull;
	__syncthreads();
	const uint64_t b64 = uint64_t(blockIdx.x) * tiles_per_block * SS_TILE;
	uint64_t e64 = b64 + uint64_t(tiles_per_block) * SS_TILE;
	if (e64 > n) e64 = n;
	if (b64 < n) ss_scatter_res_range<VB, MAXF, REBASE>(keys, vals, okeys, ovals, uint32_t(b64), uint32_t(e64), ms, fb, sp, rs, cnt, tstart, gdelta, scratch, sk, sd, sv, rebase_mask);
}
template <int VB, int MAXF>
__global__ __launch_bounds__(SS_T) void ss_scatter_res_l2_kernel(const unsigned long long *__restrict__ keys, const uint8_t *__restrict__ vals,
                                                                 unsigned long long *__restrict__ okeys, uint8_t *__restrict__ ovals, int ms, int fb,
                                                                 const unsigned long long *__restrict__ fine, const uint32_t *__restrict__ cur1,
                                                                 uint32_t cstride1, uint32_t cap1, uint32_t parts, SsReserve rs,
                                                                 const unsigned long long *__restrict__ rebase_coarse, unsigned long long rebase_mask) {
	SS_SCATTER_RES_LDS(VB, MAXF)
	const uint32_t F = 1u << fb, s = blockIdx.x / parts, p = blockIdx.x % parts;
	const unsigned long long lo = (rebase_coarse && s) ? (rebase_coarse[s - 1] & rebase_mask) : 0ull;
	for (uint32_t j = threadIdx.x; j < F; j += SS_T) {
		const unsigned long long f = j + 1 < F ? fine[size_t(s) * F + j] : ~0ull;
		sp[j] = j + 1 < F ? (f > lo ? f - lo : 0ull) : ~0ull;
	}
	__syncthreads();
	const uint32_t fill = cur1[size_t(s) * cstride1], sb = s * cap1, se = sb + (fill < cap1 ? fill : cap1);
	const uint32_t tiles = (se - sb + SS_TILE - 1) / SS_TILE, tpp = (tiles + parts - 1) / parts;
	const uint64_t b = uint64_t(sb) + uint64_t(p) * tpp * SS_TILE, e = b + uint64_t(tpp) * SS_TILE;
	const uint32_t begin = b < se ? uint32_t(b) : se, end = e < se ? uint32_t(e) : se;
	SsReserve mine = rs;
	mine.first = s * F;
	if (begin < end) ss_scatter_res_range<VB, MAXF>(keys, vals, okeys, ovals, begin, end, ms, fb, sp, mine, cnt, tstart, gdelta, scratch, sk, sd, sv);
}
__global__ __launch_bounds__(256) void ss_res_buckets_kernel(const uint32_t *__restrict__ cur2, uint32_t n_buckets, uint32_t cap,
                                                             uint32_t *__restrict__ bucket_base, uint32_t *__restrict__ bucket_cnt, uint32_t *__restrict__ max_cnt) {
	const uint32_t b = blockIdx.x * 256 + threadIdx.x;
	uint32_t c = 0;
	if (b < n_buckets) { c = cur2[b] < cap ? cur2[b] : cap; bucket_base[b] = b * cap; bucket_cnt[b] = c; }
	const unsigned long long m = wave_reduce_max_u64(c);
	if (lane_id() == 0 && m) atomicMax(max_cnt, uint32_t(m));
}

struct SsLocalArgs {
	const unsigned long long *keys;
	const uint8_t *vals;
	const uint32_t *bucket_base, *bucket_cnt;
	const uint32_t *big_list;
	uint32_t n_buckets;
	int ms;
	uint32_t cap;
	uint32_t skip_above;
	uint32_t debug;
	uint32_t atomic_below;
	uint32_t *order_flag;
	unsigned long long *t_key;
	uint32_t *t_reads, *t_agg, *n_loc;
	uint32_t *cg_loc;
	int cg_shift;
	const unsigned long long *rebase_coarse;
	unsigned long long rebase_mask;
	uint32_t rebase_div;
};

template <int THREADS, int ITEMS, int VB, bool ATOMIC_RANK = false>
__device__ inline void ss_local_run(const SsLocalArgs &a, uint32_t bucket, uint32_t base, uint32_t cnt, unsigned char *smem) {
	constexpr uint32_t WAVES = THREADS / 64;
	const uint32_t tid = threadIdx.x, w = tid >> 6, lane = tid & 63u;
	unsigned long long *sk = reinterpret_cast<unsigned long long *>(smem);
	uint32_t *agg = reinterpret_cast<uint32_t *>(smem);
	uint32_t *headpos = agg + a.cap;
	uint32_t *wcnt = reinterpret_cast<uint32_t *>(smem + size_t(a.cap) * 8);
	uint32_t *tstart = wcnt + WAVES * 256;
	uint32_t *scratch = tstart + 256;
	uint32_t *wtot = scratch + (THREADS / 64 + 1);
	uint32_t *misc = wtot + WAVES;
	unsigned long long *red = reinterpret_cast<unsigned long long *>(misc + 4 + ((WAVES + 1) & 1u));
	uint8_t *sv = reinterpret_cast<uint8_t *>(red + 2 * WAVES);
	const int ms = a.ms;
	const uint32_t coarse_b = a.rebase_coarse ? bucket / a.rebase_div : 0u;
	const unsigned long long kbase = coarse_b ? (a.rebase_coarse[coarse_b - 1u] & a.rebase_mask) : 0ull;

	const uint32_t lane_off = w * (64 * ITEMS) + lane;
	unsigned long long key[ITEMS];
	uint8_t val[VB ? ITEMS : 1];
	unsigned long long k_or = 0, k_and = ~0ull;
#pragma unroll
	for (int i = 0; i < ITEMS; ++i) {
		const uint32_t p = lane_off + i * 64;
		const bool valid = p < cnt;
		key[i] = valid ? a.keys[base + p] : 0ull;
		if (VB) val[i] = valid ? a.vals[base + p] : uint8_t(0);
	}
#pragma unroll
	for (int i = 0; i < ITEMS; ++i) {
		const uint32_t p = lane_off + i * 64;
		if (p < cnt) { k_or |= key[i]; k_and &= key[i]; sk[p] = key[i]; if (VB) sv[p] = val[i]; }
	}
	k_or = wave_reduce_or_u64(k_or); k_and = wave_reduce_and_u64(k_and);
	if (lane == 0) { red[2 * w] = k_or; red[2 * w + 1] = k_and; }
	lds_barrier();
	k_or = 0; k_and = ~0ull;
#pragma unroll
	for (uint32_t k = 0; k < WAVES; ++k) { k_or |= red[2 * k]; k_and &= red[2 * k + 1]; }
	const unsigned long long vary = (k_or ^ k_and) & ~((1ull << ms) - 1ull);

	for (int shift = vary ? __builtin_ctzll(vary) : 64; shift < 64 && (vary >> shift) != 0; shift += 8) {
		if (((vary >> shift) & 0xFFull) == 0 || (a.debug & 2u)) continue;
		for (uint32_t j = tid; j < WAVES * 256; j += THREADS) wcnt[j] = 0;
		lds_barrier();
		uint32_t lrank[ITEMS];
		const bool by_atomic = ATOMIC_RANK && uint32_t(shift) < a.atomic_below;
		const uint32_t vbits = uint32_t(vary >> shift) & 0xFFu;
#pragma unroll
		for (int i = 0; i < ITEMS; ++i) {
			const bool valid = (lane_off + i * 64) < cnt;
			const uint32_t d = uint32_t(key[i] >> shift) & 0xFFu;
			if (by_atomic) { lrank[i] = valid ? atomicAdd(&wcnt[w * 256 + d], 1u) : 0u; continue; }
			uint32_t diff_lo = 0, diff_hi = 0;
			for (uint32_t left = vbits; left; left &= left - 1u) {
				const int b = __builtin_ctz(left);
				const int32_t mine = int32_t(d << (31 - b)) >> 31;
				const unsigned long long bal = __ballot(mine != 0);
				diff_lo |= uint32_t(bal) ^ uint32_t(mine);
				diff_hi |= uint32_t(bal >> 32) ^ uint32_t(mine);
			}
			unsigned long long m = ~(((unsigned long long)diff_hi << 32) | diff_lo);
			m &= __ballot(valid);
			const uint32_t before = __builtin_amdgcn_mbcnt_hi(uint32_t(m >> 32), __builtin_amdgcn_mbcnt_lo(uint32_t(m), 0u));
			const uint32_t old = wcnt[w * 256 + d];
			__builtin_amdgcn_wave_barrier();
			if (valid && before == 0) wcnt[w * 256 + d] = old + __popcll(m);
			__builtin_amdgcn_wave_barrier();
			lrank[i] = old + before;
		}
		lds_barrier();
		if constexpr (THREADS >= 256) {
			uint32_t run = 0;
			if (tid < 256) {
#pragma unroll
				for (uint32_t k = 0; k < WAVES; ++k) { const uint32_t c = wcnt[k * 256 + tid]; wcnt[k * 256 + tid] = run; run += c; }
			}
			uint32_t total;
			const uint32_t ex = block_excl_scan_u32<THREADS, true>(tid < 256 ? run : 0u, scratch, total);
			if (tid < 256) tstart[tid] = ex;
		} else {
			constexpr uint32_t PER = 256 / THREADS;
			uint32_t tot[PER], sum = 0;
#pragma unroll
			for (uint32_t j = 0; j < PER; ++j) {
				const uint32_t d = tid * PER + j;
				uint32_t run = 0;
#pragma unroll
				for (uint32_t k = 0; k < WAVES; ++k) { const uint32_t c = wcnt[k * 256 + d]; wcnt[k * 256 + d] = run; run += c; }
				tot[j] = run; sum += run;
			}
			uint32_t total;
			uint32_t ex = block_excl_scan_u32<THREADS, true>(sum, scratch, total);
#pragma unroll
			for (uint32_t j = 0; j < PER; ++j) { tstart[tid * PER + j] = ex; ex += tot[j]; }
		}
		lds_barrier();
#pragma unroll
		for (int i = 0; i < ITEMS; ++i)
			if ((lane_off + i * 64) < cnt) {
				const uint32_t d = uint32_t(key[i] >> shift) & 0xFFu;
				const uint32_t q = tstart[d] + wcnt[w * 256 + d] + lrank[i];
				sk[q] = key[i];
				if (VB) sv[q] = val[i];
			}
		lds_barrier();
#pragma unroll
		for (int i = 0; i < ITEMS; ++i) {
			const uint32_t p = lane_off + i * 64;
			if (p < cnt) { key[i] = sk[p]; if (VB) val[i] = sv[p]; }
		}
	}

	uint32_t run = 0, pre[ITEMS], head_bits = 0, cg_heads = 0;
	bool out_of_order = false;
#pragma unroll
	for (int i = 0; i < ITEMS; ++i) {
		const uint32_t p = lane_off + i * 64;
		const bool valid = p < cnt;
		const unsigned long long prev = (valid && p) ? sk[p - 1] : 0ull;
		out_of_order |= valid && p && (prev >> ms) > (key[i] >> ms);
		const bool head = valid && (p == 0 || (prev >> ms) != (key[i] >> ms));
		const unsigned long long bal = __ballot(head);
		pre[i] = run + __builtin_amdgcn_mbcnt_hi(uint32_t(bal >> 32), __builtin_amdgcn_mbcnt_lo(uint32_t(bal), 0u));
		run += uint32_t(__popcll(bal));
		if (head) head_bits |= 1u << i;
		if (a.cg_loc) cg_heads += uint32_t(__popcll(__ballot(valid && p && (prev >> a.cg_shift) != (key[i] >> a.cg_shift))));
	}
	if (lane == 0) wtot[w] = run;
// ... 308 lines not shown
```

Baseline: 11000.

## Read device scalars through a pinned mailbox and build bucket lists on device

Adds a pinned-memory mailbox ring: a tiny kernel copies device scalars into host-visible memory and sets an epoch flag, and the host spin-waits on that flag instead of issuing a memcpy plus stream synchronize. The bucket-size classification for the sample sort moves to a device kernel, which removes the full bucket-count download, the host loop and a blocking drain. Slot compaction is also queued before the ingest readback so two readbacks collapse into one. The cost is extra small kernel launches, host CPU spinning, and more complex ordering logic that can fail if the ring or flags get out of step.

```diff
diff --git a/dropest_amd/csrc/context.h b/dropest_amd/csrc/context.h
--- a/dropest_amd/csrc/context.h
+++ b/dropest_amd/csrc/context.h
@@ -26,6 +26,7 @@
 #include "k_segreduce.h"
 #include "k_mergepath.h"
 #include "matrix_decode.h"
+#include "mailbox.h"
 #include "util.h"
 
 namespace dropest {
@@ -405,6 +406,13 @@
 
 	dropest::PinnedBuf<unsigned char> h_stage;
 	void fetch(void *dst, const void *d_src, size_t bytes);
+	dropest::Mailbox mailbox;
+	int mailbox_spin = -1;
+	static bool mailbox_off() { return getenv("DROPEST_NO_MAILBOX") != nullptr; }
+	dropest::MailboxTicket post_scalars(const void *d_a, size_t bytes_a, const void *d_b = nullptr, size_t bytes_b = 0, bool clear = false);
+	void take_scalars(const dropest::MailboxTicket &t, void *dst_a, void *dst_b = nullptr);
+	void drain();
+	u32 n_host_waits = 0, n_host_wait_copies = 0;
 	dropest::PinnedBuf<unsigned char> h_up;
 	void upload(void *d_dst, const void *src, size_t bytes);
 
@@ -542,6 +550,9 @@
 	void run_merge_and_filter();
 
 	void build_cb_table();
+	void queue_compact_slots();
+	bool slots_compacted = false;
+	u32 compacted_cells = 0;
 	void assign_cell_ids();
 	void plan_key_layout();
 	void build_keys(bool with_stats = false, bool allow_fused = true);
diff --git a/dropest_amd/csrc/dropest_amd.hip b/dropest_amd/csrc/dropest_amd.hip
--- a/dropest_amd/csrc/dropest_amd.hip
+++ b/dropest_amd/csrc/dropest_amd.hip
@@ -170,11 +170,40 @@
 void dropest_ctx::fetch(void *dst, const void *d_src, size_t bytes) {
 	if (!bytes) return;
 	h_stage.ensure(std::max<size_t>(bytes, 4096));
+	++n_host_waits; ++n_host_wait_copies;
 	HIP_CHECK(hipMemcpyAsync(h_stage.p, d_src, bytes, hipMemcpyDeviceToHost, stream));
 	HIP_CHECK(stream_wait(stream));
 	if (bytes < (size_t(4) << 20)) std::memcpy(dst, h_stage.p, bytes);
 	else
 		dropest::parallel_ranges(bytes, [&](size_t b, size_t e, unsigned) { std::memcpy(static_cast<char *>(dst) + b, h_stage.p + b, e - b); }, size_t(2) << 20, dropest::HostPool::MAX);
+}
+
+void dropest_ctx::drain() {
+	++n_host_waits;
+	HIP_CHECK(stream_wait(stream));
+}
+
+dropest::MailboxTicket dropest_ctx::post_scalars(const void *d_a, size_t bytes_a, const void *d_b, size_t bytes_b, bool clear) {
+	if (mailbox_off()) {
+		dropest::MailboxTicket t;
+		t.src[0] = d_a; t.src[1] = d_b; t.bytes[0] = u32(bytes_a); t.bytes[1] = d_b ? u32(bytes_b) : 0u; t.clear = clear; t.stream = stream;
+		return t;
+	}
+	return mailbox.post(stream, d_a, bytes_a, d_b, bytes_b, clear);
+}
+
+void dropest_ctx::take_scalars(const dropest::MailboxTicket &t, void *dst_a, void *dst_b) {
+	if (t.src[0]) {
+		fetch(dst_a, t.src[0], t.bytes[0]);
+		if (t.src[1]) fetch(dst_b, t.src[1], t.bytes[1]);
+		if (t.clear) {
+			HIP_CHECK(hipMemsetAsync(const_cast<void *>(t.src[0]), 0, t.bytes[0], stream));
+			if (t.src[1]) HIP_CHECK(hipMemsetAsync(const_cast<void *>(t.src[1]), 0, t.bytes[1], stream));
+		}
+		return;
+	}
+	++n_host_waits;
+	mailbox.take(t, dst_a, dst_b, mailbox_spin < 0 ? dropest::spin_wait_enabled() : mailbox_spin != 0);
 }
 
 void dropest_ctx::upload(void *d_dst, const void *src, size_t bytes) {
@@ -243,7 +272,7 @@
 	HostStage hs(this, "reset");
 	invalidate_prefetch();
 	initialized = merged = ingested = external_merge_done = false;
-	ss_no_reserve = false;
+	ss_no_reserve = false; slots_compacted = false;
 	reseed_rng();
 	shard.reset();
 	n_cells = n_mol = n_cg = n_chr_rows = 0;
@@ -288,7 +317,7 @@
 		const bool want_hot = !getenv("DROPEST_CB_NO_HOT");
 		if (want_hot) timed("cb_hot_count", double(cap_s) * sizeof(CbSlot), [&] { hipLaunchKernelGGL(cb_hot_count_kernel, dim3(1024), dim3(256), 0, stream, ts, scalars.p + 4); });
 		u32 head[4 + CB_HOT_LEVELS] = {0};
-		fetch(head, scalars.p, sizeof(head));
+		take_scalars(post_scalars(scalars.p, sizeof(head)), head);
 		const u32 distinct = head[0];
 		if (getenv("DROPEST_CB_TRACE")) {
 			fprintf(stderr, "[cb] sample of %u reads: %u distinct; barcodes with >= t sample hits:", n_s, distinct);
@@ -403,14 +432,20 @@
 			else if (vec) go(cb_insert_kernel<256, true>); else go(cb_insert_kernel<256, false>);
 		});
 		}
-		fetch(&ingest, d_ingest.p, sizeof(ingest));
+		slots_compacted = false;
+		if (mailbox_off()) fetch(&ingest, d_ingest.p, sizeof(ingest));
+		else {
+			queue_compact_slots();
+			take_scalars(post_scalars(d_ingest.p, sizeof(ingest), scalars.p, 4), &ingest, &compacted_cells);
+			slots_compacted = !ingest.overflow;
+		}
 		if (!ingest.overflow) break;
 		if (attempt >= 6) throw DeviceError("barcode table overflow after repeated growth");
 		cap <<= 2;
 	}
 }
 
-void dropest_ctx::assign_cell_ids() {
+void dropest_ctx::queue_compact_slots() {
 	const u32 n = u32(n_reads);
 	const uint64_t cap = table.mask + 1;
 	keys_a.ensure(n); keys_b.ensure(n);
@@ -421,8 +456,15 @@
 		hipLaunchKernelGGL(cb_compact_slots_kernel, dim3(u32(std::min<uint64_t>((cap + 4095) / 4096, 4096))), dim3(256), 0, stream, table,
 		                   keys_a.p, scalars.p);
 	});
+}
+
+void dropest_ctx::assign_cell_ids() {
+	const u32 n = u32(n_reads);
+	const uint64_t cap = table.mask + 1;
 	u32 total = 0;
-	fetch(&total, scalars.p, 4);
+	if (slots_compacted) total = compacted_cells;
+	else { queue_compact_slots(); fetch(&total, scalars.p, 4); }
+	slots_compacted = false;
 	n_cells = total;
 	if (uint64_t(n_cells) * 10 > cap * 7)
 	{
@@ -713,14 +755,13 @@
 		if (VB == 0) pick(std::integral_constant<int, 0>{}); else pick(std::integral_constant<int, 1>{});
 	});
 	if (!launched) return false;
-	fetch(&counters, d_counters.p, sizeof(counters));
 	if (with_stats) {
 		IngestStats exact{};
-		fetch(&exact, d_ingest.p, sizeof(exact));
+		take_scalars(post_scalars(d_counters.p, sizeof(counters), d_ingest.p, sizeof(exact)), &counters, &exact);
 		exact.cb_escape_count = ingest.cb_escape_count;
 		exact.overflow = 0;
 		ingest = exact;
-	}
+	} else take_scalars(post_scalars(d_counters.p, sizeof(counters)), &counters);
 	keys_in_l1 = true;
 	return true;
 }
@@ -778,14 +819,13 @@
 		else if (layout.val_bytes == 1) pick(std::integral_constant<int, 1>{});
 		else pick(std::integral_constant<int, 4>{});
 	});
-	fetch(&counters, d_counters.p, sizeof(counters));
 	if (with_stats) {
 		IngestStats exact{};
-		fetch(&exact, d_ingest.p, sizeof(exact));
+		take_scalars(post_scalars(d_counters.p, sizeof(counters), d_ingest.p, sizeof(exact)), &counters, &exact);
 		exact.cb_escape_count = ingest.cb_escape_count;
 		exact.overflow = 0;
 		ingest = exact;
-	}
+	} else take_scalars(post_scalars(d_counters.p, sizeof(counters)), &counters);
 }
 
 static constexpr int RS_T = 512, RS_I = 16, RS_TILE_REC = RS_T * RS_I;
@@ -965,9 +1005,15 @@
 	nblocks = div_up(n_tiles, tpb);
 	const u32 parts = std::max<u32>(1, std::min<u32>(16, 2048 / F1));
 	ss_bucket_base.ensure(F2); ss_bucket_cnt.ensure(F2); scalars.ensure(16);
-	HIP_CHECK(hipMemsetAsync(scalars.p, 0, 16, stream));
+	HIP_CHECK(hipMemsetAsync(scalars.p, 0, 28, stream));
 	u32 max_cnt = 0;
-	static const u32 SMALL_MAX = [] { const char *e = getenv("DROPEST_SS_SMALL_MAX"); return e && atoi(e) >= 256 && atoi(e) <= 2048 ? u32(atoi(e)) : 2048u; }();
+	const u32 SMALL_MAX = [] { const char *e = getenv("DROPEST_SS_SMALL_MAX"); return e && atoi(e) >= 256 && atoi(e) <= 2048 ? u32(atoi(e)) : 2048u; }();
+	const bool device_lists = !mailbox_off();
+	u32 n_medium = 0, n_big = 0;
+	auto list_buckets = [&] {
+		ss_big_list.ensure(F2);
+		hipLaunchKernelGGL(ss_list_buckets_kernel, dim3(div_up(F2, 256)), dim3(256), 0, stream, ss_bucket_cnt.p, F2, SMALL_MAX, ss_big_list.p, scalars.p + 5);
+	};
 	const bool atomic_rank = lds_atomics_lane_ordered(cfg.device, stream);
 	ss_tmp.ensure(span * 2 + 2); ss_n_loc.ensure(F2); ss_prefix.ensure(F2); ss_chunk.ensure(1024);
 	SsLocalArgs a{};
@@ -1031,10 +1077,16 @@
 		timed("ss_scan", double(F2) * 12, [&] {
 			hipLaunchKernelGGL(ss_res_buckets_kernel, dim3(div_up(F2, 256)), dim3(256), 0, stream, cur2, F2, cap2, ss_bucket_base.p, ss_bucket_cnt.p, scalars.p);
 		});
+		u32 head[7] = {0, 0, 0, 0, 0, 0, 0};
+		dropest::MailboxTicket head_ticket;
+		if (device_lists) {
+			timed("ss_scan", double(F2) * 4, list_buckets);
+			head_ticket = post_scalars(scalars.p, sizeof(head));
+		}
 		launch_small();
-		u32 head[4] = {0, 0, 0, 0};
-		fetch(head, scalars.p, 16);
-		max_cnt = head[0];
+		if (device_lists) take_scalars(head_ticket, head);
+		else fetch(head, scalars.p, 16);
+		max_cnt = head[0]; n_medium = head[5]; n_big = head[6];
 		if (head[3]) {
 			stats["count:ss_reserve_overflow"].launches += 1;
 			ss_no_reserve = true;
@@ -1068,7 +1120,12 @@
 		if (wide) hipLaunchKernelGGL(ss_scan_seg_kernel<1024>, dim3(F1), dim3(1024), 0, stream, ss_cnt2.p, Ff, parts, ss_base1.p, ss_bucket_base.p, ss_bucket_cnt.p, scalars.p);
 		else hipLaunchKernelGGL(ss_scan_seg_kernel<512>, dim3(F1), dim3(512), 0, stream, ss_cnt2.p, Ff, parts, ss_base1.p, ss_bucket_base.p, ss_bucket_cnt.p, scalars.p);
 	});
-	fetch(&max_cnt, scalars.p, 4);
+	if (device_lists) {
+		u32 head[7] = {0, 0, 0, 0, 0, 0, 0};
+		timed("ss_scan", double(F2) * 4, list_buckets);
+		take_scalars(post_scalars(scalars.p, sizeof(head)), head);
+		max_cnt = head[0]; n_medium = head[5]; n_big = head[6];
+	} else fetch(&max_cnt, scalars.p, 4);
 	if (max_cnt > SS_LOCAL_MAX) return false;
 	timed(VB ? "ss_scatter:L2:key+1B" : "ss_scatter:L2:keys", double(n) * 2 * (8 + VB), [&] {
 		auto go = [&](auto kernel) { hipLaunchKernelGGL(kernel, dim3(F1 * parts), dim3(SS_T), 0, stream, keys_alt, vals_alt, keys, vals, ms, fb2, ss_fine.p, ss_base1.p, parts, ss_cnt2.p); };
@@ -1079,12 +1136,21 @@
 
 	if (!reserve) launch_small();
 	if (max_cnt > SMALL_MAX) {
-		std::vector<u32> cnts(F2), medium, big;
-		fetch(cnts.data(), ss_bucket_cnt.p, size_t(F2) * 4);
-		for (u32 b = 0; b < F2; ++b) if (cnts[b] > SMALL_MAX) (cnts[b] <= 4096 ? medium : big).push_back(b);
-		ss_big_list.ensure(medium.size() + big.size());
-		if (!medium.empty()) HIP_CHECK(hipMemcpyAsync(ss_big_list.p, medium.data(), medium.size() * 4, hipMemcpyHostToDevice, stream));
-		if (!big.empty()) HIP_CHECK(hipMemcpyAsync(ss_big_list.p + medium.size(), big.data(), big.size() * 4, hipMemcpyHostToDevice, stream));
+		std::vector<u32> cnts, medium, big;
+		const u32 *d_medium = ss_big_list.p, *d_big = nullptr;
+		if (device_lists) {
+			if (uint64_t(n_medium) + n_big == 0 || uint64_t(n_medium) + n_big > F2) throw DeviceError("internal: the device's list of large buckets does not match the largest bucket");
+			d_big = ss_big_list.p + (F2 - n_big);
+		} else {
+			cnts.resize(F2);
+			fetch(cnts.data(), ss_bucket_cnt.p, size_t(F2) * 4);
+			for (u32 b = 0; b < F2; ++b) if (cnts[b] > SMALL_MAX) (cnts[b] <= 4096 ? medium : big).push_back(b);
+			ss_big_list.ensure(medium.size() + big.size());
+			if (!medium.empty()) HIP_CHECK(hipMemcpyAsync(ss_big_list.p, medium.data(), medium.size() * 4, hipMemcpyHostToDevice, stream));
+			if (!big.empty()) HIP_CHECK(hipMemcpyAsync(ss_big_list.p + medium.size(), big.data(), big.size() * 4, hipMemcpyHostToDevice, stream));
+			n_medium = u32(medium.size()); n_big = u32(big.size());
+			d_medium = ss_big_list.p; d_big = ss_big_list.p + medium.size();
+		}
 		auto launch = [&](auto kernel, u32 threads, u32 cap, const u32 *list, size_t count) {
 			SsLocalArgs g = a;
 			g.big_list = list; g.cap = cap; g.skip_above = cap;
@@ -1094,14 +1160,14 @@
 		};
 		timed("ss_local:big", 0, [&] {
 			if (atomic_rank) {
-				if (!medium.empty()) { if (VB2) launch(ss_local_big_kernel<256, 1, true>, 256, 4096, ss_big_list.p, medium.size()); else launch(ss_local_big_kernel<256, 0, true>, 256, 4096, ss_big_list.p, medium.size()); }
-				if (!big.empty()) { if (VB2) launch(ss_local_big_kernel<512, 1, true>, 512, SS_LOCAL_MAX, ss_big_list.p + medium.size(), big.size()); else launch(ss_local_big_kernel<512, 0, true>, 512, SS_LOCAL_MAX, ss_big_list.p + medium.size(), big.size()); }
+				if (n_medium) { if (VB2) launch(ss_local_big_kernel<256, 1, true>, 256, 4096, d_medium, n_medium); else launch(ss_local_big_kernel<256, 0, true>, 256, 4096, d_medium, n_medium); }
+				if (n_big) { if (VB2) launch(ss_local_big_kernel<512, 1, true>, 512, SS_LOCAL_MAX, d_big, n_big); else launch(ss_local_big_kernel<512, 0, true>, 512, SS_LOCAL_MAX, d_big, n_big); }
 			} else {
-				if (!medium.empty()) { if (VB2) launch(ss_local_big_kernel<256, 1>, 256, 4096, ss_big_list.p, medium.size()); else launch(ss_local_big_kernel<256, 0>, 256, 4096, ss_big_list.p, medium.size()); }
-				if (!big.empty()) { if (VB2) launch(ss_local_big_kernel<512, 1>, 512, SS_LOCAL_MAX, ss_big_list.p + medium.size(), big.size()); else launch(ss_local_big_kernel<512, 0>, 512, SS_LOCAL_MAX, ss_big_list.p + medium.size(), big.size()); }
+				if (n_medium) { if (VB2) launch(ss_local_big_kernel<256, 1>, 256, 4096, d_medium, n_medium); else launch(ss_local_big_kernel<256, 0>, 256, 4096, d_medium, n_medium); }
+				if (n_big) { if (VB2) launch(ss_local_big_kernel<512, 1>, 512, SS_LOCAL_MAX, d_big, n_big); else launch(ss_local_big_kernel<512, 0>, 512, SS_LOCAL_MAX, d_big, n_big); }
 			}
 		});
-		HIP_CHECK(stream_wait(stream));
+		if (!device_lists) drain();
 	}
 	const u32 n_chunks = div_up(F2, 1024);
 	timed("ss_scan", double(F2) * 12, [&] {
@@ -1114,7 +1180,7 @@
 		}
 	});
 	u32 total_flag[4] = {0, 0, 0, 0};
-	fetch(total_flag, scalars.p + 1, 16);
+	take_scalars(post_scalars(scalars.p + 1, 16), total_flag);
 	if (total_flag[1]) {
 		if (atomic_rank) lds_atomics_mark_unordered(cfg.device);
 		stats["count:ss_order_violation"].launches += 1;
@@ -1220,7 +1286,7 @@
 		n_chr_rows = 0;
 		if (!cg_from_sort) reduce_molecules_to_cell_gene();
 		reduce_cell_gene_to_cells();
-		HIP_CHECK(stream_wait(stream));
+		if (mailbox_off()) drain();
 		return;
 	}
 	main_sort_passes = u32(plan_radix_passes(varying).size()); main_sort_kind = 0;
@@ -1259,7 +1325,7 @@
 	}
 	reduce_molecules_to_cell_gene();
 	reduce_cell_gene_to_cells();
-	HIP_CHECK(stream_wait(stream));
+	if (mailbox_off()) drain();
 }
 
 void dropest_ctx::reduce_molecules_to_cell_gene() {
@@ -1332,7 +1398,7 @@
 	});
 	tail_mark("fetch_real_cells: flag kernels enqueued", true);
 	u32 count = 0;
-	fetch(&count, scalars.p, 4);
+	take_scalars(post_scalars(scalars.p, 4), &count);
 	tail_mark("count fetched");
 	if (count == 0) return;
 	DevBuf<CellRowPod> &rows = real_rows_dev; rows.ensure(count);
@@ -1344,7 +1410,8 @@
 	h_stage.ensure(id_off + size_t(count) * 4);
 	HIP_CHECK(hipMemcpyAsync(h_stage.p, rows.p, row_bytes, hipMemcpyDeviceToHost, stream));
 	HIP_CHECK(hipMemcpyAsync(h_stage.p + id_off, list.p, size_t(count) * 4, hipMemcpyDeviceToHost, stream));
-	HIP_CHECK(stream_wait(stream));
+	++n_host_wait_copies;
+	drain();
 	tail_mark("rows on the host");
 	const CellRowPod *host_rows = reinterpret_cast<const CellRowPod *>(h_stage.p);
 	const u32 *ids = reinterpret_cast<const u32 *>(h_stage.p + id_off);
@@ -1618,6 +1685,7 @@
 		if (const char *e = getenv("DROPEST_CB_SAMPLE_MIN")) sample_min = uint64_t(std::max(1ll, atoll(e)));
 		lazy_stats = !ingested && n_reads >= sample_min && !getenv("DROPEST_EXACT_INGEST_STATS");
 	}
+	if (!ingested) n_host_waits = n_host_wait_copies = 0;
 	run_ingest();
 	HostStage hs_all(this, "set_initialized");
 	if (n_reads > 0) {
@@ -1644,6 +1712,11 @@
 		{ HostStage hs(this, "sort+reduce"); reduce_all(); }
 		accumulate_umi_qualities();
 		{ HostStage hs(this, "real_cells"); fetch_real_cells(true); }
+		if (profiling) {
+			stats["count:host_waits"].launches += n_host_waits;
+			stats["count:host_wait_copies"].launches += n_host_wait_copies;
+		}
+		n_host_waits = n_host_wait_copies = 0;
 	} else {
 		plan_key_layout();
 	}
@@ -2826,3 +2899,4 @@
 }
 
 #include "shard_run.h"
+#include "mailbox_test.h"
diff --git a/dropest_amd/csrc/k_ssort.h b/dropest_amd/csrc/k_ssort.h
--- a/dropest_amd/csrc/k_ssort.h
+++ b/dropest_amd/csrc/k_ssort.h
@@ -383,6 +383,25 @@
 	if (b < n_buckets) { c = cur2[b] < cap ? cur2[b] : cap; bucket_base[b] = b * cap; bucket_cnt[b] = c; }
 	const unsigned long long m = wave_reduce_max_u64(c);
 	if (lane_id() == 0 && m) atomicMax(max_cnt, uint32_t(m));
+}
+__global__ __launch_bounds__(256) void ss_list_buckets_kernel(const uint32_t *__restrict__ bucket_cnt, uint32_t n_buckets, uint32_t small_max,
+                                                              uint32_t *__restrict__ list, uint32_t *__restrict__ counts) {
+	const uint32_t b = blockIdx.x * 256 + threadIdx.x, lane = lane_id();
+	const uint32_t c = b < n_buckets ? bucket_cnt[b] : 0u;
+	const bool medium = c > small_max && c <= 4096u, big = c > 4096u;
+	for (int which = 0; which < 2; ++which) {
+		const bool mine = which ? big : medium;
+		const unsigned long long m = __ballot(mine);
+		if (!m) continue;
+		const int leader = __builtin_ctzll(m);
+		uint32_t base = 0;
+		if (lane == uint32_t(leader)) base = atomicAdd(counts + which, uint32_t(__popcll(m)));
+		base = uint32_t(__shfl(int(base), leader, 64));
+		if (mine) {
+			const uint32_t at = base + uint32_t(__popcll(m & ((1ull << lane) - 1ull)));
+			if (at < n_buckets) list[which ? n_buckets - 1u - at : at] = b;
+		}
+	}
 }
 
 struct SsLocalArgs {
diff --git a/dropest_amd/csrc/mailbox.h b/dropest_amd/csrc/mailbox.h
--- /dev/null
+++ b/dropest_amd/csrc/mailbox.h
@@ -0,0 +1,56 @@
+#pragma once
+
+#include "mailbox_host.h"
+#include "util.h"
+
+namespace dropest {
+
+__global__ __launch_bounds__(64) void mailbox_post_kernel(uint32_t *a, uint32_t wa, uint32_t *b, uint32_t wb, uint32_t *payload, uint32_t *flag,
+                                                          uint32_t epoch, uint32_t clear) {
+	for (uint32_t i = threadIdx.x; i < wa; i += 64) { payload[i] = a[i]; if (clear) a[i] = 0; }
+	for (uint32_t i = threadIdx.x; i < wb; i += 64) { payload[wa + i] = b[i]; if (clear) b[i] = 0; }
+	__threadfence_system();
+	__syncthreads();
+	if (threadIdx.x == 0) __hip_atomic_store(flag, epoch, __ATOMIC_RELEASE, __HIP_MEMORY_SCOPE_SYSTEM);
+}
+
+struct MailboxHipOps {
+	static hipStream_t st(void *s) { return static_cast<hipStream_t>(s); }
+	bool ready(void *s) {
+		const hipError_t e = hipStreamQuery(st(s));
+		if (e == hipErrorNotReady) return false;
+		HIP_CHECK(e);
+		return true;
+	}
+	void sync(void *s) { HIP_CHECK(hipStreamSynchronize(st(s))); }
+	void relax() { host_cpu_relax(); }
+	[[noreturn]] void lost(const char *what) { throw DeviceError(what); }
+	[[noreturn]] void misuse(const char *what) { throw InvalidError(what); }
+};
+
+struct Mailbox {
+	PinnedBuf<unsigned char> mem;
+	MailboxRing<MailboxHipOps> ring;
+	void ensure(uint32_t start_epoch = 0) {
+		if (ring.attached()) return;
+		mem.ensure_exact(size_t(MAILBOX_SLOTS) * MAILBOX_STRIDE, hipHostMallocDefault);
+		std::memset(mem.p, 0, size_t(MAILBOX_SLOTS) * MAILBOX_STRIDE);
+		ring.attach(mem.p, start_epoch);
+	}
+	void restart(uint32_t start_epoch) { ensure(); ring.attach(mem.p, start_epoch); }
+	MailboxTicket post(hipStream_t stream, const void *a, size_t bytes_a, const void *b, size_t bytes_b, bool clear) {
+		ensure();
+		if ((uintptr_t(a) | uintptr_t(b)) & 3u) throw InvalidError("mailbox: a post reads whole, aligned words");
+		if (bytes_a > MAILBOX_PAYLOAD || bytes_b > MAILBOX_PAYLOAD) throw InvalidError("mailbox: a post is 4 .. 240 bytes in whole words");
+		const MailboxTicket t = ring.reserve(stream, uint32_t(bytes_a), b ? uint32_t(bytes_b) : 0u);
+		hipLaunchKernelGGL(mailbox_post_kernel, dim3(1), dim3(64), 0, stream, static_cast<uint32_t *>(const_cast<void *>(a)), t.bytes[0] / 4,
+		                   static_cast<uint32_t *>(const_cast<void *>(b)), t.bytes[1] / 4, reinterpret_cast<uint32_t *>(ring.payload(t.slot)), ring.flag(t.slot), t.epoch,
+		                   clear ? 1u : 0u);
+		const hipError_t e = hipGetLastError();
+		if (e != hipSuccess) { ring.abandon(t); HIP_CHECK(e); }
+		return t;
+	}
+	void take(const MailboxTicket &t, void *dst_a, void *dst_b, bool spin) { ring.take(t, dst_a, dst_b, spin); }
+};
+
+}
diff --git a/dropest_amd/csrc/mailbox_host.h b/dropest_amd/csrc/mailbox_host.h
--- /dev/null
+++ b/dropest_amd/csrc/mailbox_host.h
@@ -0,0 +1,85 @@
+#pragma once
+
+#include <chrono>
+#include <cstdint>
+#include <cstring>
+
+namespace dropest {
+
+constexpr uint32_t MAILBOX_SLOTS = 16, MAILBOX_STRIDE = 256, MAILBOX_PAYLOAD = 240;
+
+struct MailboxTicket {
+	uint32_t slot = 0xFFFFFFFFu, epoch = 0;
+	uint32_t bytes[2] = {0, 0};
+	void *stream = nullptr;
+	const void *src[2] = {nullptr, nullptr};
+	bool clear = false;
+	bool valid() const { return slot != 0xFFFFFFFFu || src[0] != nullptr; }
+};
+
+template <class Ops>
+class MailboxRing {
+	unsigned char *mem_ = nullptr;
+	uint32_t epoch_ = 0, next_ = 0;
+	bool busy_[MAILBOX_SLOTS] = {};
+	uint32_t expect_[MAILBOX_SLOTS] = {};
+	std::chrono::microseconds patience_{50000};
+	static uint32_t load_flag(const uint32_t *f) { return __atomic_load_n(f, __ATOMIC_ACQUIRE); }
+
+public:
+	Ops ops;
+	bool attached() const { return mem_ != nullptr; }
+	uint32_t outstanding() const { uint32_t n = 0; for (bool b : busy_) n += b; return n; }
+	void set_patience(std::chrono::microseconds p) { patience_ = p; }
+	void attach(unsigned char *mem, uint32_t start_epoch) {
+		if (outstanding()) ops.misuse("mailbox: re-attached with tickets outstanding");
+		mem_ = mem; epoch_ = start_epoch; next_ = 0;
+		for (uint32_t s = 0; s < MAILBOX_SLOTS; ++s) __atomic_store_n(flag(s), start_epoch, __ATOMIC_RELEASE);
+	}
+	unsigned char *payload(uint32_t slot) const { return mem_ + size_t(slot) * MAILBOX_STRIDE; }
+	uint32_t *flag(uint32_t slot) const { return reinterpret_cast<uint32_t *>(mem_ + size_t(slot) * MAILBOX_STRIDE + MAILBOX_PAYLOAD); }
+
+	MailboxTicket reserve(void *stream, uint32_t bytes0, uint32_t bytes1) {
+		if (!mem_) ops.misuse("mailbox: not attached");
+		if ((bytes0 | bytes1) & 3u || bytes0 == 0 || uint64_t(bytes0) + bytes1 > MAILBOX_PAYLOAD) ops.misuse("mailbox: a post is 4 .. 240 bytes in whole words");
+		const uint32_t s = next_;
+		if (busy_[s]) ops.misuse("mailbox: the ring is full (a ticket was never taken)");
+		next_ = (next_ + 1) % MAILBOX_SLOTS;
+		busy_[s] = true; expect_[s] = ++epoch_;
+		MailboxTicket t;
+		t.slot = s; t.epoch = epoch_; t.bytes[0] = bytes0; t.bytes[1] = bytes1; t.stream = stream;
+		return t;
+	}
+	void abandon(const MailboxTicket &t) { if (t.slot < MAILBOX_SLOTS && expect_[t.slot] == t.epoch) busy_[t.slot] = false; }
+
+	void take(const MailboxTicket &t, void *dst0, void *dst1, bool spin) {
+		if (t.slot >= MAILBOX_SLOTS || !busy_[t.slot] || expect_[t.slot] != t.epoch) ops.misuse("mailbox: ticket taken twice or never posted");
+		busy_[t.slot] = false;
+		const uint32_t *f = flag(t.slot);
+		bool there = false;
+		if (spin) {
+			const auto t0 = std::chrono::steady_clock::now();
+			for (uint32_t it = 0;; ++it) {
+				if (load_flag(f) == t.epoch) { there = true; break; }
+				if ((it & 255u) == 255u) {
+					if (ops.ready(t.stream)) {
+						if (load_flag(f) != t.epoch) ops.lost("mailbox: the stream is complete and the post's flag is not there");
+						there = true;
+						break;
+					}
+					if (std::chrono::steady_clock::now() - t0 > patience_) break;
+				}
+				ops.relax();
+			}
+		}
+		if (!there) {
+			ops.sync(t.stream);
+			if (load_flag(f) != t.epoch) ops.lost("mailbox: the stream is complete and the post's flag is not there");
+		}
+		const unsigned char *p = payload(t.slot);
+		if (dst0) std::memcpy(dst0, p, t.bytes[0]);
+		if (dst1 && t.bytes[1]) std::memcpy(dst1, p + t.bytes[0], t.bytes[1]);
+	}
+};
+
+}
```

Result: no change. 11020, median of 2 (+0.2%).
